# simplew4y/VeritasFi

Hardware: AMD Instinct MI355X
Metric: queries/sec top-100 over 10Mx768 corpus (higher is better)
Workload: dtype f16

## Files before the change

### include/veritasfi_hip.h

```cpp
#ifndef VERITASFI_HIP_H
#define VERITASFI_HIP_H

#include <stdint.h>

#ifdef __cplusplus
extern "C" {
#endif

#define VF_VERSION 100

enum {
    VF_OK = 0,
    VF_EINVAL = -1,
    VF_ENOMEM = -2,
    VF_EHIP = -3,
    VF_EUNSUPPORTED = -4,
    VF_EINTERNAL = -5
};

enum { VF_DTYPE_F32 = 0, VF_DTYPE_F16 = 1, VF_DTYPE_FP8_E4M3 = 2, VF_DTYPE_INT8 = 3 };

typedef struct vf_index vf_index;

typedef struct vf_search_stats {
    int64_t path;
    int64_t n_queries;
    int64_t candidates;
    int64_t max_candidates;
    int64_t uncertified;
    int64_t overflowed;
    int64_t exact_reruns;
    int64_t wide_launches;
    int64_t wide_queries;
    int64_t aux_cus;
    int64_t scans_overlap;
    int64_t scan_kernel;
    int64_t scan_image;
    int64_t reserved[3];
} vf_search_stats;

int vf_version(void);
const char* vf_last_error(void);
int vf_device_count(int32_t* out);

int vf_index_create(vf_index** out, const void* rows, int64_t n, int32_t d, int32_t dtype,
                    int32_t device_id, int64_t id_offset);

int vf_index_create_device(vf_index** out, const void* d_rows, int64_t n, int32_t d, int32_t dtype,
                           int32_t device_id, int64_t id_offset);

int vf_index_create_sharded(vf_index** out, const void* rows, int64_t n, int32_t d, int32_t dtype,
                            const int32_t* device_ids, int32_t n_dev);
int vf_index_create_sharded_from_file(vf_index** out, const char* path, const int32_t* device_ids, int32_t n_dev);
int vf_index_group(vf_index** out, vf_index** shards, int32_t n_shards);
int vf_index_shards(vf_index* idx, int32_t* n_shards, int32_t* device_ids, int32_t cap);
int vf_index_peer_access(vf_index* idx, int32_t* ok, int32_t cap, int32_t* n_missing);

int vf_corpus_file_info(const char* path, int64_t* n, int32_t* d, int32_t* dtype, int32_t* has_ids);
int vf_index_create_from_file(vf_index** out, const char* path, int64_t row_lo, int64_t row_hi, int32_t device_id,
                              int64_t id_offset);

int vf_index_search(vf_index* idx, const float* queries, int32_t nq, int32_t k, int64_t* out_ids,
                    float* out_scores);

int vf_index_search_device(vf_index* idx, const float* d_queries, int32_t nq, int32_t k,
                           int64_t* d_ids, float* d_scores, void* stream);

int vf_index_slots(vf_index* idx, int32_t* out);
int vf_index_search_begin(vf_index* idx, int32_t slot, const float* d_queries, int32_t nq, int32_t k,
                          int64_t* d_ids, float* d_scores, void* stream);
int vf_index_search_end(vf_index* idx, int32_t slot);

int vf_index_info(vf_index* idx, int64_t* n, int32_t* d, int32_t* dtype, int32_t* device_id);
int vf_index_stats(vf_index* idx, vf_search_stats* out);
int vf_index_set_option(vf_index* idx, const char* name, int64_t value);
int vf_index_profile(vf_index* idx, double* scan_ms_total, int64_t* scan_launches, double* pipeline_ms_total,
                     int64_t* scan_bytes_per_launch);
int vf_index_profile_span(vf_index* idx, double* span_ms, int64_t* launches);
int vf_index_debug_read(vf_index* idx, int32_t slot, unsigned long long* out, int64_t n_words);
int vf_index_destroy(vf_index* idx);

int vf_cosine_matrix(const float* x, int32_t n, int32_t d, float* out, int32_t device_id);
int vf_cosine_matrix_rows(vf_index* idx, const int64_t* ids, int32_t n, float* out);
int vf_cosine_matrix_rows_mixed(vf_index* idx, const int64_t* ids, int32_t n, const float* extra, int32_t n_extra, float* out);

int vf_cosine_scores(const float* a, int32_t na, const float* b, int64_t nb, int32_t d, float* out,
                     int32_t device_id);

int vf_merge_topk_device(const int64_t* d_ids_parts, const float* d_score_parts, int32_t nparts,
                         int32_t nq, int32_t k, int64_t* d_ids, float* d_scores, int32_t device_id,
                         void* stream);

int vf_merge_topk_packed_device(const void* d_parts, int32_t nparts, int32_t nq, int32_t k, int64_t* d_ids,
                                float* d_scores, int32_t device_id, void* stream);

int vf_fuse_rank(const float* rerank_scores, const float* time_scores, int32_t n, float* out_scores,
                 int64_t* out_order, int32_t device_id);

typedef struct vf_encoder vf_encoder;
typedef struct vf_encoder_config {
    int32_t vocab, hidden, layers, heads, ffn, max_pos, type_vocab;
    int32_t roberta_pad_idx;
    int32_t pooling;
    int32_t normalize;
    int32_t head;
    float ln_eps;
} vf_encoder_config;

int vf_encoder_weight_sizes(const vf_encoder_config* cfg, int64_t* n_fp16, int64_t* n_fp32);
int vf_encoder_create(vf_encoder** out, const vf_encoder_config* cfg, const void* w_fp16, int64_t n_fp16,
                      const float* w_fp32, int64_t n_fp32, int32_t device_id);
int vf_encoder_forward(vf_encoder* enc, const int32_t* ids, const int32_t* mask, const int32_t* type_ids,
                       int32_t b, int32_t t, int32_t t_valid, float* out);
int vf_encoder_forward_pooled(vf_encoder* enc, const int32_t* ids, const int32_t* mask, const int32_t* type_ids,
                              int32_t b, int32_t t, int32_t t_valid, int32_t pooling, int32_t normalize, float* out);
int vf_encoder_forward_hidden(vf_encoder* enc, const int32_t* ids, const int32_t* mask, const int32_t* type_ids,
                              int32_t b, int32_t t, float* out_hidden);
int vf_encoder_info(vf_encoder* enc, vf_encoder_config* out);
int vf_encoder_destroy(vf_encoder* enc);
typedef struct vf_decoder vf_decoder;
typedef struct vf_decoder_config {
    int32_t vocab, hidden, layers, heads, kv_heads, head_dim, ffn;
    float rope_theta, rms_eps;
    int32_t qk_norm;
    int32_t pooling;
    int32_t normalize;
    int32_t head;
    int32_t act;
    int32_t norm_plus_one;
    float embed_scale;
} vf_decoder_config;
int vf_decoder_weight_sizes(const vf_decoder_config* cfg, int64_t* n_fp16, int64_t* n_fp32);
int vf_decoder_create(vf_decoder** out, const vf_decoder_config* cfg, const void* w_fp16, int64_t n_fp16,
                      const float* w_fp32, int64_t n_fp32, int32_t device_id);
int vf_decoder_forward(vf_decoder* dec, const int32_t* ids, const int32_t* mask, int32_t b, int32_t t, int32_t t_valid,
                       float* out);
int vf_decoder_forward_pooled(vf_decoder* dec, const int32_t* ids, const int32_t* mask, int32_t b, int32_t t, int32_t t_valid,
                              int32_t normalize, float* out);
int vf_decoder_forward_hidden(vf_decoder* dec, const int32_t* ids, const int32_t* mask, int32_t b, int32_t t,
                              float* out_hidden);
int vf_decoder_destroy(vf_decoder* dec);

int vf_reranker_create(vf_encoder** out, const vf_encoder_config* cfg, const void* w_fp16, int64_t n_fp16,
                       const float* w_fp32, int64_t n_fp32, int32_t device_id);
int vf_reranker_score(vf_encoder* rr, const int32_t* ids, const int32_t* mask, const int32_t* type_ids, int32_t b,
                      int32_t t, float* out_scores);
int vf_reranker_destroy(vf_encoder* rr);

typedef struct vf_vit vf_vit;
typedef struct vf_vit_config {
    int32_t image, patch, channels;
    int32_t hidden, layers, heads, ffn;
    int32_t proj_dim;
    int32_t act;
    int32_t normalize;
    float ln_eps;
} vf_vit_config;
int vf_vit_weight_sizes(const vf_vit_config* cfg, int64_t* n_fp16, int64_t* n_fp32);
int vf_vit_create(vf_vit** out, const vf_vit_config* cfg, const void* w_fp16, int64_t n_fp16, const float* w_fp32,
                  int64_t n_fp32, int32_t device_id);
int vf_vit_forward(vf_vit* vit, const float* pixels, int32_t b, float* out);
int vf_vit_forward_u8(vf_vit* vit, const unsigned char* pixels, const float* mean3, const float* std3, int32_t b, float* out);
int vf_vit_destroy(vf_vit* vit);

typedef struct vf_clip_text vf_clip_text;
typedef struct vf_clip_text_config {
    int32_t vocab, max_pos;
    int32_t hidden, layers, heads, ffn;
    int32_t proj_dim;
    int32_t act;
    int32_t eos_token_id;
    int32_t normalize;
    float ln_eps;
} vf_clip_text_config;
int vf_clip_text_weight_sizes(const vf_clip_text_config* cfg, int64_t* n_fp16, int64_t* n_fp32);
int vf_clip_text_create(vf_clip_text** out, const vf_clip_text_config* cfg, const void* w_fp16, int64_t n_fp16, const float* w_fp32,
                        int64_t n_fp32, int32_t device_id);
int vf_clip_text_forward(vf_clip_text* ct, const int32_t* ids, const int32_t* mask, int32_t b, int32_t t, float* out);
int vf_clip_text_destroy(vf_clip_text* ct);

typedef struct vf_bm25 vf_bm25;
int vf_bm25_create(const int64_t* indptr, int64_t vocab, const int32_t* indices, const float* data, int64_t nnz,
                   int64_t n_docs, int32_t device_id, vf_bm25** out, int32_t* slots);
int vf_bm25_search(vf_bm25* h, const int64_t* q_offsets, const int32_t* q_terms, int32_t nq, int32_t k, int64_t* out_ids,
                   float* out_scores);

#ifdef __cplusplus
}
#endif
#endif
```

### veritasfi_amd/_ffi.py

```python
from __future__ import annotations

import ctypes
import os
import threading

_HERE = os.path.dirname(os.path.abspath(__file__))
LIB_PATH = os.environ.get("VF_LIB_PATH") or os.path.join(_HERE, "lib", "libveritasfi_hip.so")

VF_OK = 0
VF_DTYPE_F32, VF_DTYPE_F16, VF_DTYPE_FP8_E4M3, VF_DTYPE_INT8 = 0, 1, 2, 3

c_i32, c_i64, c_f32 = ctypes.c_int32, ctypes.c_int64, ctypes.c_float
p_i32, p_i64, p_f32 = ctypes.POINTER(c_i32), ctypes.POINTER(c_i64), ctypes.POINTER(c_f32)
vp = ctypes.c_void_p


class EncoderConfig(ctypes.Structure):
    _fields_ = [
        ("vocab", c_i32), ("hidden", c_i32), ("layers", c_i32), ("heads", c_i32), ("ffn", c_i32), ("max_pos", c_i32),
        ("type_vocab", c_i32), ("roberta_pad_idx", c_i32), ("pooling", c_i32), ("normalize", c_i32), ("head", c_i32),
        ("ln_eps", c_f32),
    ]


class DecoderConfig(ctypes.Structure):
    _fields_ = [
        ("vocab", c_i32), ("hidden", c_i32), ("layers", c_i32), ("heads", c_i32), ("kv_heads", c_i32), ("head_dim", c_i32),
        ("ffn", c_i32), ("rope_theta", c_f32), ("rms_eps", c_f32), ("qk_norm", c_i32), ("pooling", c_i32),
        ("normalize", c_i32), ("head", c_i32), ("act", c_i32), ("norm_plus_one", c_i32), ("embed_scale", c_f32),
    ]


class VitConfig(ctypes.Structure):
    _fields_ = [
        ("image", c_i32), ("patch", c_i32), ("channels", c_i32), ("hidden", c_i32), ("layers", c_i32), ("heads", c_i32),
        ("ffn", c_i32), ("proj_dim", c_i32), ("act", c_i32), ("normalize", c_i32), ("ln_eps", c_f32),
    ]


class ClipTextConfig(ctypes.Structure):
    _fields_ = [
        ("vocab", c_i32), ("max_pos", c_i32), ("hidden", c_i32), ("layers", c_i32), ("heads", c_i32), ("ffn", c_i32),
        ("proj_dim", c_i32), ("act", c_i32), ("eos_token_id", c_i32), ("normalize", c_i32), ("ln_eps", c_f32),
    ]


class SearchStats(ctypes.Structure):
    _fields_ = [
        ("path", c_i64), ("n_queries", c_i64), ("candidates", c_i64), ("max_candidates", c_i64),
        ("uncertified", c_i64), ("overflowed", c_i64), ("exact_reruns", c_i64), ("wide_launches", c_i64), ("wide_queries", c_i64),
        ("aux_cus", c_i64), ("scans_overlap", c_i64), ("scan_kernel", c_i64), ("scan_image", c_i64), ("reserved", c_i64 * 3),
    ]

    def as_dict(self):
        return {k: int(getattr(self, k)) for k, _ in self._fields_ if k != "reserved"}


SIGNATURES = {
    "vf_version": (ctypes.c_int, []),
    "vf_last_error": (ctypes.c_char_p, []),
    "vf_device_count": (ctypes.c_int, [p_i32]),
    "vf_index_create": (ctypes.c_int, [ctypes.POINTER(vp), vp, c_i64, c_i32, c_i32, c_i32, c_i64]),
    "vf_index_create_device": (ctypes.c_int, [ctypes.POINTER(vp), vp, c_i64, c_i32, c_i32, c_i32, c_i64]),
    "vf_index_create_sharded": (ctypes.c_int, [ctypes.POINTER(vp), vp, c_i64, c_i32, c_i32, p_i32, c_i32]),
    "vf_index_create_sharded_from_file": (ctypes.c_int, [ctypes.POINTER(vp), ctypes.c_char_p, p_i32, c_i32]),
    "vf_index_group": (ctypes.c_int, [ctypes.POINTER(vp), ctypes.POINTER(vp), c_i32]),
    "vf_index_shards": (ctypes.c_int, [vp, p_i32, p_i32, c_i32]),
    "vf_index_peer_access": (ctypes.c_int, [vp, p_i32, c_i32, p_i32]),
    "vf_corpus_file_info": (ctypes.c_int, [ctypes.c_char_p, ctypes.POINTER(c_i64), ctypes.POINTER(c_i32), ctypes.POINTER(c_i32), ctypes.POINTER(c_i32)]),
    "vf_index_create_from_file": (ctypes.c_int, [ctypes.POINTER(vp), ctypes.c_char_p, c_i64, c_i64, c_i32, c_i64]),
    "vf_index_search": (ctypes.c_int, [vp, vp, c_i32, c_i32, vp, vp]),
    "vf_index_search_device": (ctypes.c_int, [vp, vp, c_i32, c_i32, vp, vp, vp]),
    "vf_index_slots": (ctypes.c_int, [vp, p_i32]),
    "vf_index_search_begin": (ctypes.c_int, [vp, c_i32, vp, c_i32, c_i32, vp, vp, vp]),
    "vf_index_search_end": (ctypes.c_int, [vp, c_i32]),
    "vf_index_info": (ctypes.c_int, [vp, p_i64, p_i32, p_i32, p_i32]),
    "vf_index_stats": (ctypes.c_int, [vp, ctypes.POINTER(SearchStats)]),
    "vf_index_set_option": (ctypes.c_int, [vp, ctypes.c_char_p, c_i64]),
    "vf_index_profile": (ctypes.c_int, [vp, ctypes.POINTER(ctypes.c_double), p_i64, ctypes.POINTER(ctypes.c_double), p_i64]),
    "vf_index_profile_span": (ctypes.c_int, [vp, ctypes.POINTER(ctypes.c_double), p_i64]),
    "vf_index_debug_read": (ctypes.c_int, [vp, c_i32, vp, c_i64]),
    "vf_index_destroy": (ctypes.c_int, [vp]),
    "vf_cosine_matrix": (ctypes.c_int, [vp, c_i32, c_i32, vp, c_i32]),
    "vf_cosine_matrix_rows": (ctypes.c_int, [vp, vp, c_i32, vp]),
    "vf_cosine_matrix_rows_mixed": (ctypes.c_int, [vp, vp, c_i32, vp, c_i32, vp]),
    "vf_cosine_scores": (ctypes.c_int, [vp, c_i32, vp, c_i64, c_i32, vp, c_i32]),
    "vf_merge_topk_device": (ctypes.c_int, [vp, vp, c_i32, c_i32, c_i32, vp, vp, c_i32, vp]),
    "vf_merge_topk_packed_device": (ctypes.c_int, [vp, c_i32, c_i32, c_i32, vp, vp, c_i32, vp]),
    "vf_fuse_rank": (ctypes.c_int, [vp, vp, c_i32, vp, vp, c_i32]),
    "vf_encoder_weight_sizes": (ctypes.c_int, [ctypes.POINTER(EncoderConfig), p_i64, p_i64]),
    "vf_encoder_create": (ctypes.c_int, [ctypes.POINTER(vp), ctypes.POINTER(EncoderConfig), vp, c_i64, vp, c_i64, c_i32]),
    "vf_encoder_forward": (ctypes.c_int, [vp, vp, vp, vp, c_i32, c_i32, c_i32, vp]),
    "vf_encoder_forward_pooled": (ctypes.c_int, [vp, vp, vp, vp, c_i32, c_i32, c_i32, c_i32, c_i32, vp]),
    "vf_encoder_forward_hidden": (ctypes.c_int, [vp, vp, vp, vp, c_i32, c_i32, vp]),
    "vf_encoder_info": (ctypes.c_int, [vp, ctypes.POINTER(EncoderConfig)]),
    "vf_encoder_destroy": (ctypes.c_int, [vp]),
    "vf_reranker_create": (ctypes.c_int, [ctypes.POINTER(vp), ctypes.POINTER(EncoderConfig), vp, c_i64, vp, c_i64, c_i32]),
    "vf_reranker_score": (ctypes.c_int, [vp, vp, vp, vp, c_i32, c_i32, vp]),
    "vf_reranker_destroy": (ctypes.c_int, [vp]),
    "vf_decoder_weight_sizes": (ctypes.c_int, [vp, p_i64, p_i64]),
    "vf_decoder_create": (ctypes.c_int, [ctypes.POINTER(vp), vp, vp, c_i64, vp, c_i64, c_i32]),
    "vf_decoder_forward": (ctypes.c_int, [vp, vp, vp, c_i32, c_i32, c_i32, vp]),
    "vf_decoder_forward_pooled": (ctypes.c_int, [vp, vp, vp, c_i32, c_i32, c_i32, c_i32, vp]),
    "vf_decoder_forward_hidden": (ctypes.c_int, [vp, vp, vp, c_i32, c_i32, vp]),
    "vf_decoder_destroy": (ctypes.c_int, [vp]),
    "vf_vit_weight_sizes": (ctypes.c_int, [ctypes.POINTER(VitConfig), p_i64, p_i64]),
    "vf_vit_create": (ctypes.c_int, [ctypes.POINTER(vp), ctypes.POINTER(VitConfig), vp, c_i64, vp, c_i64, c_i32]),
    "vf_vit_forward": (ctypes.c_int, [vp, vp, c_i32, vp]),
    "vf_vit_forward_u8": (ctypes.c_int, [vp, vp, vp, vp, c_i32, vp]),
    "vf_vit_destroy": (ctypes.c_int, [vp]),
    "vf_clip_text_weight_sizes": (ctypes.c_int, [ctypes.POINTER(ClipTextConfig), p_i64, p_i64]),
    "vf_clip_text_create": (ctypes.c_int, [ctypes.POINTER(vp), ctypes.POINTER(ClipTextConfig), vp, c_i64, vp, c_i64, c_i32]),
    "vf_clip_text_forward": (ctypes.c_int, [vp, vp, vp, c_i32, c_i32, vp]),
    "vf_clip_text_destroy": (ctypes.c_int, [vp]),
    "vf_bm25_create": (ctypes.c_int, [p_i64, c_i64, p_i32, p_f32, c_i64, c_i64, c_i32, ctypes.POINTER(vp), p_i32]),
    "vf_bm25_search": (ctypes.c_int, [vp, p_i64, p_i32, c_i32, c_i32, p_i64, p_f32]),
}

_lib = None
_lock = threading.Lock()


def lib():
    global _lib
    if _lib is None:
        with _lock:
            if _lib is None:
                if not os.path.exists(LIB_PATH):
                    raise RuntimeError(
                        f"{LIB_PATH} is missing: build it with `python -m veritasfi_amd.build` "
                        "(hipcc --offload-arch=gfx950). veritasfi_amd has no CPU fallback.")
                try:
                    import torch
                except ImportError:
                    pass
                L = ctypes.CDLL(LIB_PATH)
                for name, (res, args) in SIGNATURES.items():
                    fn = getattr(L, name)
                    fn.restype = res
                    fn.argtypes = args
                _lib = L
    return _lib


def loaded() -> bool:
    return _lib is not None


def last_error() -> str:
    msg = lib().vf_last_error()
    return msg.decode("utf-8", "replace") if msg else ""


def check(rc: int, what: str = "") -> None:
    if rc != VF_OK:
        raise RuntimeError(f"{what or 'veritasfi_hip'} failed (rc={rc}): {last_error()}")
```

### veritasfi_amd/csrc/vf_api.hip

```cpp
#include "../../include/veritasfi_hip.h"
#include "vf_internal.h"

#include <fcntl.h>
#include <float.h>
#include <sys/stat.h>
#include <unistd.h>
#include <math.h>
#include <string.h>

#include <algorithm>
#include <atomic>
#include <mutex>
#include <string>
#include <vector>

using namespace vf;

static thread_local std::string g_err;

static int fail(int code, const std::string& msg) {
    g_err = msg;
    return code;
}
int vf::set_error(int code, const std::string& msg) { return fail(code, msg); }

#define VF_HIP(expr)                                                                                   \
    do {                                                                                               \
        hipError_t _e = (expr);                                                                        \
        if (_e != hipSuccess)                                                                          \
            return fail(VF_EHIP, std::string(#expr) + ": " + hipGetErrorString(_e) + " (" + __FILE__ + \
                                     ":" + std::to_string(__LINE__) + ")");                            \
    } while (0)

#define VF_TRY(expr)             \
    do {                         \
        int _rc = (expr);        \
        if (_rc != VF_OK) return _rc; \
    } while (0)

extern "C" int vf_version(void) { return VF_VERSION; }
extern "C" const char* vf_last_error(void) { return g_err.c_str(); }

extern "C" int vf_device_count(int32_t* out) {
    if (!out) return fail(VF_EINVAL, "vf_device_count: null out");
    int n = 0;
    hipError_t e = hipGetDeviceCount(&n);
    if (e != hipSuccess) { *out = 0; return fail(VF_EHIP, std::string("hipGetDeviceCount: ") + hipGetErrorString(e)); }
    *out = n;
    return VF_OK;
}

namespace {

constexpr int kSlots = 4;

struct DevBuf {
    void* p = nullptr;
    size_t bytes = 0;
    int ensure(size_t need) {
        if (need <= bytes) return VF_OK;
        if (p) { (void)hipFree(p); p = nullptr; bytes = 0; }
        hipError_t e = hipMalloc(&p, need);
        if (e != hipSuccess) return fail(VF_ENOMEM, std::string("hipMalloc(") + std::to_string(need) + "): " + hipGetErrorString(e));
        bytes = need;
        return VF_OK;
    }
    void release() { if (p) (void)hipFree(p); p = nullptr; bytes = 0; }
    template <class T> T* as() const { return (T*)p; }
};

struct HostBuf {
    void* p = nullptr;
    size_t bytes = 0;
    int ensure(size_t need) {
        if (need <= bytes) return VF_OK;
        if (p) { (void)hipHostFree(p); p = nullptr; bytes = 0; }
        hipError_t e = hipHostMalloc(&p, need, hipHostMallocDefault);
        if (e != hipSuccess) return fail(VF_ENOMEM, std::string("hipHostMalloc(") + std::to_string(need) + "): " + hipGetErrorString(e));
        bytes = need;
        return VF_OK;
    }
    void release() { if (p) (void)hipHostFree(p); p = nullptr; bytes = 0; }
};

struct Slot {
    hipStream_t stream = nullptr;
    hipStream_t scan_stream = nullptr;
    hipEvent_t ev_pro = nullptr;
    hipEvent_t ev_in = nullptr, ev_done = nullptr, ev_scan = nullptr;
    hipEvent_t ev_t[4] = {nullptr, nullptr, nullptr, nullptr};
    bool timed = false;
    int wide_launches = 0, wide_queries = 0;
    int scan_kernel = 0;
    int scan_image = 0;
    DevBuf qn, qimg, s0, cnt, tau, hist, hist_coarse, cand, flags, counts;
    DevBuf dbg, wgbase, tilecnt, sib;
    DevBuf qimg8, epsq;
    DevBuf qscale, bandq;
    int image_i8 = 0;
    int64_t wgbase_n = -1; int wgbase_grid = -1;
    DevBuf dense_s, cn_tmp, parts_ids, parts_sc, run_ids, run_sc, qsel;
    int* h_flags = nullptr;
    u32* h_counts = nullptr;
    int* d_flags = nullptr;
    u32* d_counts = nullptr;
    size_t h_cap = 0;
    bool pending = false;
    const float* d_queries = nullptr;
    int nq = 0, k = 0, path = 0;
    int64_t* d_ids = nullptr;
    float* d_scores = nullptr;
    hipStream_t user_stream = nullptr;
};

struct GroupSlot {
    std::vector<hipStream_t> feed;
    std::vector<hipEvent_t> ev;
    std::vector<DevBuf> dq, blob;
    DevBuf all;
    hipEvent_t ev_in = nullptr;
    hipStream_t hq_stream = nullptr;
    hipEvent_t ev_hq = nullptr;
    HostBuf hq;
    std::vector<hipStream_t> hfeed;
    std::vector<hipEvent_t> ev_hb;
    std::vector<hipEvent_t> ev_home;
    std::vector<HostBuf> hb;
    std::vector<char> staged_last;
    bool pending = false;
    int nq = 0, k = 0;
    int64_t* d_ids = nullptr; float* d_scores = nullptr;
    hipStream_t user = nullptr;
};

}

struct vf_index {
    int device = 0;
    int64_t n = 0;
    int d = 0, dp = 0, dtype = 0;
    int64_t id_offset = 0;
    int n_cu = 256;
    int64_t aux_applied = -1;
    bool owns_rows = false;
    void* rows_orig = nullptr;
    void* rows_scan = nullptr;
    bool owns_scan = false;
    float* norm = nullptr;
    float* inv_scan = nullptr;
    float* cn_cache = nullptr;
    unsigned char* rows_img = nullptr;
    bool owns_img = false;
    float* inv_img = nullptr;
    float rho_max = 0.0f;
    float rho_mean = 0.0f;
    std::mutex mu;
    Slot slots[kSlots];
    int64_t force_path = -1, sample_rows = -1, margin = -1, cap_opt = 0, waves_opt = 0, scan_g = 0,
            refresh_every = 128, debug = 0, steal_opt = 0, wide_opt = 1, wide_sync = -1, wide_mfma = -1, wide8_waves = 8, wide8_stage = 0,
            aux_cus = -1, sample_grid = -1, overlap_scans = -1, scan_impl = 2, sample_impl = -1, scan_image = 1, wide_rows = 1, image_mfma = -1;
    vf_search_stats stats{};
    bool profile = false;
    double prof_scan_ms = 0.0, prof_pipe_ms = 0.0;
    int64_t prof_launches = 0, prof_bytes = 0;
    hipEvent_t ev_span = nullptr;
    bool span_started = false;
    bool span_slot[4] = {false, false, false, false};
    DevBuf st_q, st_ids, st_sc;
    std::vector<vf_index*> shards;
    std::vector<int> peer_ok;
    GroupSlot gslots[kSlots];
};

static int ensure_pinned(Slot& s, size_t nq_total) {
    if (nq_total <= s.h_cap) return VF_OK;
    if (s.h_flags) (void)hipHostFree(s.h_flags);
    if (s.h_counts) (void)hipHostFree(s.h_counts);
    s.h_flags = nullptr; s.h_counts = nullptr; s.h_cap = 0;
    size_t cap = std::max<size_t>(nq_total, 256);
    VF_HIP(hipHostMalloc((void**)&s.h_flags, cap * sizeof(int), hipHostMallocMapped));
    VF_HIP(hipHostMalloc((void**)&s.h_counts, cap * sizeof(u32), hipHostMallocMapped));
    VF_HIP(hipHostGetDevicePointer((void**)&s.d_flags, s.h_flags, 0));
    VF_HIP(hipHostGetDevicePointer((void**)&s.d_counts, s.h_counts, 0));
    s.h_cap = cap;
    return VF_OK;
}

static int build_image(vf_index* ix, int64_t mode);

static bool byte_rows(int dtype) { return dtype == VF_DTYPE_FP8_E4M3 || dtype == VF_DTYPE_INT8; }
static bool known_dtype(int64_t dtype) { return dtype >= VF_DTYPE_F32 && dtype <= VF_DTYPE_INT8; }
static size_t dtype_bytes(int dtype) { return dtype == VF_DTYPE_F32 ? 4 : (dtype == VF_DTYPE_F16 ? 2 : 1); }
static int scan_f8(int dtype) { return dtype == VF_DTYPE_INT8 ? 2 : (dtype == VF_DTYPE_FP8_E4M3 ? 1 : 0); }

static int build_common(vf_index* ix) {
    hipDeviceProp_t prop;
    VF_HIP(hipGetDeviceProperties(&prop, ix->device));
    ix->n_cu = prop.multiProcessorCount > 0 ? prop.multiProcessorCount : 256;
    VF_HIP(scan_configure());
    const int dt = ix->dtype;
    const size_t scan_esz = byte_rows(dt) ? 1 : 2;
    ix->dp = (ix->d + 127) / 128 * 128;
    const size_t npad = (size_t)ix->n + 64;
    VF_HIP(hipMalloc((void**)&ix->norm, npad * sizeof(float)));
    VF_HIP(hipMalloc((void**)&ix->inv_scan, npad * sizeof(float)));
    VF_HIP(hipMemset(ix->norm, 0, npad * sizeof(float)));
    VF_HIP(hipMemset(ix->inv_scan, 0, npad * sizeof(float)));
    const bool need_scan = ix->n > kSmallN;
    void* scan_out = nullptr;
    if (need_scan) {
        if (dt != VF_DTYPE_F32 && ix->dp == ix->d && ((uintptr_t)ix->rows_orig % 16) == 0) {
            ix->rows_scan = ix->rows_orig;
            ix->owns_scan = false;
        } else {
            VF_HIP(hipMalloc((void**)&ix->rows_scan, (size_t)ix->n * ix->dp * scan_esz));
            ix->owns_scan = true;
            scan_out = ix->rows_scan;
        }
    }
    VF_HIP(launch_prep_rows(ix->rows_orig, dt, ix->n, ix->d, ix->dp, scan_out, ix->norm, ix->inv_scan, nullptr));
    VF_TRY(build_image(ix, ix->scan_image));
    if (ix->n > 0 && ix->n <= kSmallN) {
        VF_HIP(hipMalloc((void**)&ix->cn_cache, (size_t)ix->n * ix->d * sizeof(float)));
        VF_HIP(launch_normalize_rows(ix->rows_orig, dt, 0, ix->n, ix->d, ix->norm, ix->cn_cache, nullptr));
    }
    VF_HIP(hipDeviceSynchronize());
    return VF_OK;
}

constexpr int64_t kSplitMaxRows = 6'000'000;
constexpr int64_t kScan2rMinRows = 1'100'000;
static bool scan2r_auto_width(int dp, bool f8) { return f8 ? (dp == 768 || dp == 1024) : (dp == 768 || dp == 1024 || dp == 512 || dp == 384); }
static int64_t split_limit(const vf_index* ix) {
    const bool r_rows = !byte_rows(ix->dtype) && ix->scan_impl != 4 && ix->scan_impl != 1 && ix->scan_impl != 3 && !ix->steal_opt &&
                        scan2r_auto_width(ix->dp, false) && scan2r_stage_cap(ix->dp, kMaxBatch, 0) >= 256;
    return r_rows ? INT64_MAX : kSplitMaxRows;
}
static int64_t resolved_aux(const vf_index* ix) {
    if (ix->aux_applied >= 0) return ix->aux_applied;
    int64_t a = ix->aux_cus >= 0 ? ix->aux_cus : (ix->n <= split_limit(ix) ? 32 : 0);
    if (a <= 0 || ix->n_cu < 64 || a * 2 > ix->n_cu) return 0;
    return a;
}
static bool resolved_overlap(const vf_index* ix) {
    return ix->overlap_scans >= 0 ? ix->overlap_scans != 0 : resolved_aux(ix) > 0;
}

constexpr int kImageMaxK = 128;
constexpr int64_t kImageMinRows = 4'000'000;
constexpr double kImageMaxRho = 1.0 / 64;
constexpr size_t kImageHeadroom = (size_t)8 << 30;
constexpr int kImageMfmaAuto = 1;
static bool image_eligible(const vf_index* ix, int64_t mode) {
    if (!ix->shards.empty() || ix->n >= (int64_t)0xFFFFFFFFll || ix->dp != 768 || scan2r_stage_cap(ix->dp, kMaxBatch, 2) < 256) return false;
    if (ix->dtype == VF_DTYPE_INT8) return ix->rows_scan && (mode == 2 ? ix->n > kSmallN : ix->n >= kImageMinRows);
    return (ix->dtype == VF_DTYPE_F16 || ix->dtype == VF_DTYPE_F32) && ix->n >= kImageMinRows;
}
static float* image_offsets(const vf_index* ix) { return ix->inv_img ? ix->inv_img + ix->n + 64 : nullptr; }
static void free_image(vf_index* ix) {
    if (ix->rows_img && ix->owns_img) (void)hipFree(ix->rows_img);
    if (ix->inv_img) (void)hipFree(ix->inv_img);
    ix->rows_img = nullptr; ix->inv_img = nullptr; ix->owns_img = false; ix->rho_max = ix->rho_mean = 0.0f;
}
static int build_image(vf_index* ix, int64_t mode) {
    if (mode == 0 || ix->rows_img || !image_eligible(ix, mode)) return VF_OK;
    const size_t ibytes = 2 * ((size_t)ix->n + 64) * sizeof(float);
    if (ix->dtype == VF_DTYPE_INT8) {
        if (hipMalloc((void**)&ix->inv_img, ibytes) != hipSuccess) {
            (void)hipGetLastError();
            ix->inv_img = nullptr;
            return mode == 2 ? fail(VF_ENOMEM, "scan_image = 2: the row inverses and offsets do not fit in device memory") : VF_OK;
        }
        VF_HIP(hipMemset(ix->inv_img, 0, ibytes));
        VF_HIP(hipMemcpy(ix->inv_img, ix->inv_scan, (size_t)ix->n * sizeof(float), hipMemcpyDeviceToDevice));
        ix->rows_img = (unsigned char*)ix->rows_scan; ix->owns_img = false;
        return VF_OK;
    }
    const size_t bytes = (size_t)ix->n * ix->dp;
    if (mode == 1) {
        size_t free_b = 0, total_b = 0;
        if (hipMemGetInfo(&free_b, &total_b) != hipSuccess) { (void)hipGetLastError(); return VF_OK; }
        if (free_b < bytes + ibytes + kImageHeadroom) return VF_OK;
    }
    ix->owns_img = true;
    if (hipMalloc((void**)&ix->rows_img, bytes) != hipSuccess || hipMalloc((void**)&ix->inv_img, ibytes) != hipSuccess) {
        (void)hipGetLastError();
        free_image(ix);
        return mode == 2 ? fail(VF_ENOMEM, "scan_image = 2: the int8 row image does not fit in device memory") : VF_OK;
    }
    u32* d_rho = nullptr;
    VF_HIP(hipMalloc((void**)&d_rho, 2 * sizeof(u32)));
    VF_HIP(hipMemset(d_rho, 0, 2 * sizeof(u32)));
    VF_HIP(hipMemset(ix->inv_img, 0, ibytes));
    VF_HIP(launch_prep_image(ix->rows_orig, ix->dtype, ix->n, ix->d, ix->dp, ix->norm, ix->rows_img, ix->inv_img, image_offsets(ix), d_rho,
                             (float*)(d_rho + 1), nullptr));
    u32 bits[2] = {0u, 0u};
    VF_HIP(hipMemcpy(bits, d_rho, sizeof(bits), hipMemcpyDeviceToHost));
    (void)hipFree(d_rho);
    float rho, sum;
    memcpy(&rho, &bits[0], sizeof(rho));
    memcpy(&sum, &bits[1], sizeof(sum));
    if (!(rho <= kImageMaxRho)) { free_image(ix); return VF_OK; }
    ix->rho_max = rho;
    ix->rho_mean = sum / (float)ix->n;
    return VF_OK;
}

static int ensure_slot(vf_index* ix, Slot& s) {
    if (s.stream) return VF_OK;
    VF_HIP(hipStreamCreateWithFlags(&s.stream, hipStreamNonBlocking));
    s.scan_stream = s.stream;
    int64_t aux = resolved_aux(ix);
    if (aux) {
        const int words = (ix->n_cu + 31) / 32;
        std::vector<uint32_t> mask(words, 0u);
        for (int b = 0; b < ix->n_cu - (int)aux; ++b) mask[b / 32] |= 1u << (b % 32);
        hipStream_t ms = nullptr;
        if (hipExtStreamCreateWithCUMask(&ms, (uint32_t)words, mask.data()) == hipSuccess && ms) s.scan_stream = ms;
        else { (void)hipGetLastError(); if (ix->aux_applied < 0) aux = 0; }
    }
    if (ix->aux_applied < 0) ix->aux_applied = aux;
    VF_HIP(hipEventCreateWithFlags(&s.ev_in, hipEventDisableTiming));
    VF_HIP(hipEventCreateWithFlags(&s.ev_done, hipEventDisableTiming));
    VF_HIP(hipEventCreateWithFlags(&s.ev_scan, hipEventDisableTiming));
    VF_HIP(hipEventCreateWithFlags(&s.ev_pro, hipEventDisableTiming));
    for (int e = 0; e < 4; ++e) VF_HIP(hipEventCreate(&s.ev_t[e]));
    return VF_OK;
}

static void destroy_index(vf_index* ix) {
    if (!ix) return;
    if (!ix->shards.empty()) {
        for (int i = 0; i < kSlots; ++i) {
            GroupSlot& gs = ix->gslots[i];
            for (size_t g = 0; g < ix->shards.size(); ++g) {
                (void)hipSetDevice(ix->shards[g]->device);
                (void)hipDeviceSynchronize();
                if (g < gs.dq.size()) gs.dq[g].release();
                if (g < gs.blob.size()) gs.blob[g].release();
                if (g < gs.feed.size() && gs.feed[g]) (void)hipStreamDestroy(gs.feed[g]);
                if (g < gs.ev.size() && gs.ev[g]) (void)hipEventDestroy(gs.ev[g]);
                if (g < gs.ev_hb.size() && gs.ev_hb[g]) (void)hipEventDestroy(gs.ev_hb[g]);
                if (g < gs.hb.size()) gs.hb[g].release();
            }
            (void)hipSetDevice(ix->device);
            gs.all.release();
            gs.hq.release();
            for (hipStream_t st : gs.hfeed) if (st) (void)hipStreamDestroy(st);
            for (hipEvent_t ev : gs.ev_home) if (ev) (void)hipEventDestroy(ev);
            if (gs.hq_stream) (void)hipStreamDestroy(gs.hq_stream);
            if (gs.ev_hq) (void)hipEventDestroy(gs.ev_hq);
            if (gs.ev_in) (void)hipEventDestroy(gs.ev_in);
        }
        for (vf_index* sh : ix->shards) destroy_index(sh);
        ix->shards.clear();
    }
    (void)hipSetDevice(ix->device);
    (void)hipDeviceSynchronize();
    ix->st_q.release(); ix->st_ids.release(); ix->st_sc.release();
    for (int i = 0; i < kSlots; ++i) {
        Slot& s = ix->slots[i];
        DevBuf* bufs[] = {&s.qn, &s.qimg, &s.s0, &s.cnt, &s.tau, &s.hist, &s.hist_coarse, &s.cand, &s.flags, &s.counts, &s.dense_s,
                          &s.cn_tmp, &s.parts_ids, &s.parts_sc, &s.run_ids, &s.run_sc, &s.qsel, &s.dbg, &s.wgbase, &s.tilecnt, &s.sib};
        for (DevBuf* b : bufs) b->release();
        if (s.h_flags) (void)hipHostFree(s.h_flags);
        if (s.h_counts) (void)hipHostFree(s.h_counts);
        if (s.scan_stream && s.scan_stream != s.stream) (void)hipStreamDestroy(s.scan_stream);
        if (s.stream) (void)hipStreamDestroy(s.stream);
        if (s.ev_pro) (void)hipEventDestroy(s.ev_pro);
        if (s.ev_in) (void)hipEventDestroy(s.ev_in);
        if (s.ev_done) (void)hipEventDestroy(s.ev_done);
        if (s.ev_scan) (void)hipEventDestroy(s.ev_scan);
        for (int e = 0; e < 4; ++e) if (s.ev_t[e]) (void)hipEventDestroy(s.ev_t[e]);
    }
    if (ix->owns_scan && ix->rows_scan) (void)hipFree(ix->rows_scan);
    if (ix->owns_rows && ix->rows_orig) (void)hipFree(ix->rows_orig);
    if (ix->norm) (void)hipFree(ix->norm);
    if (ix->inv_scan) (void)hipFree(ix->inv_scan);
    if (ix->cn_cache) (void)hipFree(ix->cn_cache);
    if (ix->rows_img && ix->owns_img) (void)hipFree(ix->rows_img);
    if (ix->inv_img) (void)hipFree(ix->inv_img);
    if (ix->ev_span) (void)hipEventDestroy(ix->ev_span);
    delete ix;
}

static int create_impl(vf_index** out, const void* rows, bool rows_on_device, int64_t n, int32_t d, int32_t dtype,
                       int32_t device_id, int64_t id_offset, bool adopt = false) {
    if (!out) return fail(VF_EINVAL, "vf_index_create: null out");
    *out = nullptr;
    if (n < 0 || d <= 0 || (n > 0 && !rows)) return fail(VF_EINVAL, "vf_index_create: bad rows/n/d");
    if (!known_dtype(dtype)) return fail(VF_EINVAL, "vf_index_create: unknown dtype");
    if (n >= (int64_t)0xFFFFFFFFll) return fail(VF_EUNSUPPORTED, "vf_index_create: more than 2^32-1 rows per shard");
    int ndev = 0;
    VF_HIP(hipGetDeviceCount(&ndev));
    if (device_id < 0 || device_id >= ndev) return fail(VF_EINVAL, "vf_index_create: bad device_id");
    VF_HIP(hipSetDevice(device_id));
    vf_index* ix = new (std::nothrow) vf_index();
    if (!ix) return fail(VF_ENOMEM, "vf_index_create: host allocation failed");
    ix->device = device_id; ix->n = n; ix->d = d; ix->id_offset = id_offset;
    ix->dtype = dtype;
    const size_t esz = dtype_bytes(dtype);
    int rc = VF_OK;
    if (rows_on_device && dtype == VF_DTYPE_INT8 && !adopt && n > 0) {
        hipError_t e = hipMalloc(&ix->rows_orig, (size_t)n * d);
        if (e != hipSuccess) rc = fail(VF_ENOMEM, std::string("hipMalloc(corpus): ") + hipGetErrorString(e));
        else {
            ix->owns_rows = true;
            e = launch_rebias_i8(rows, ix->rows_orig, (long long)n * d, nullptr);
            if (e != hipSuccess) rc = fail(VF_EHIP, std::string("re-biasing the int8 rows: ") + hipGetErrorString(e));
        }
    } else if (rows_on_device) {
        ix->rows_orig = const_cast<void*>(rows);
        ix->owns_rows = false;
        if (dtype == VF_DTYPE_INT8 && n > 0) {
            const hipError_t e = launch_rebias_i8(ix->rows_orig, ix->rows_orig, (long long)n * d, nullptr);
            if (e != hipSuccess) rc = fail(VF_EHIP, std::string("re-biasing the int8 rows: ") + hipGetErrorString(e));
        }
    } else if (n > 0) {
        hipError_t e = hipMalloc(&ix->rows_orig, (size_t)n * d * esz);
        if (e != hipSuccess) rc = fail(VF_ENOMEM, std::string("hipMalloc(corpus): ") + hipGetErrorString(e));
        else {
            ix->owns_rows = true;
            e = hipMemcpy(ix->rows_orig, rows, (size_t)n * d * esz, hipMemcpyHostToDevice);
            if (e != hipSuccess) rc = fail(VF_EHIP, std::string("hipMemcpy(corpus): ") + hipGetErrorString(e));
            else if (dtype == VF_DTYPE_INT8) {
                e = launch_rebias_i8(ix->rows_orig, ix->rows_orig, (long long)n * d, nullptr);
                if (e != hipSuccess) rc = fail(VF_EHIP, std::string("re-biasing the int8 rows: ") + hipGetErrorString(e));
            }
        }
    }
    if (rc == VF_OK) rc = build_common(ix);
    if (rc != VF_OK) { std::string keep = g_err; destroy_index(ix); g_err = keep; return rc; }
    *out = ix;
    return VF_OK;
}

extern "C" int vf_index_create(vf_index** out, const void* rows, int64_t n, int32_t d, int32_t dtype,
                               int32_t device_id, int64_t id_offset) {
    DeviceGuard restore_callers_device;
    return create_impl(out, rows, false, n, d, dtype, device_id, id_offset);
}

extern "C" int vf_index_create_device(vf_index** out, const void* d_rows, int64_t n, int32_t d, int32_t dtype,
                                      int32_t device_id, int64_t id_offset) {
    DeviceGuard restore_callers_device;
    return create_impl(out, d_rows, true, n, d, dtype, device_id, id_offset);
}

struct VfcHeader {
    char magic[8];
    uint32_t version, dtype;
    uint64_t n;
    uint32_t d, flags;
    uint8_t reserved[32];
};
static_assert(sizeof(VfcHeader) == 64, "corpus file header is 64 bytes");

static int read_vfc_header(int fd, const char* path, VfcHeader* h, size_t* esz) {
    if (pread(fd, h, sizeof(*h), 0) != (ssize_t)sizeof(*h)) return fail(VF_EINVAL, std::string("corpus file too short: ") + path);
    if (memcmp(h->magic, "VFCORPUS", 8) != 0) return fail(VF_EINVAL, std::string("not a corpus file (bad magic): ") + path);
    if (h->version != 1) return fail(VF_EUNSUPPORTED, std::string("corpus file version not supported: ") + path);
    if (!known_dtype(h->dtype) || h->d == 0) return fail(VF_EINVAL, std::string("corpus file header is corrupt: ") + path);
    *esz = dtype_bytes((int)h->dtype);
    struct stat st;
    if (fstat(fd, &st) != 0) return fail(VF_EINVAL, std::string("cannot stat corpus file: ") + path);
    unsigned long long payload = 0, ids = 0, need = 0;
    if (__builtin_mul_overflow((unsigned long long)h->n, (unsigned long long)h->d * (unsigned long long)*esz, &payload) ||
        __builtin_mul_overflow((unsigned long long)h->n, (h->flags & 1u) ? 8ull : 0ull, &ids) ||
        __builtin_add_overflow(payload, ids, &need) || __builtin_add_overflow(need, 64ull, &need))
        return fail(VF_EINVAL, std::string("corpus file header is corrupt (n x d overflows): ") + path);
    if ((unsigned long long)st.st_size < need) return fail(VF_EINVAL, std::string("corpus file is truncated: ") + path);
    if (h->n >= 0x7fffffffffffffffull / 2) return fail(VF_EINVAL, std::string("corpus file header is corrupt: ") + path);
    return VF_OK;
}

extern "C" int vf_corpus_file_info(const char* path, int64_t* n, int32_t* d, int32_t* dtype, int32_t* has_ids) {
    if (!path) return fail(VF_EINVAL, "vf_corpus_file_info: null path");
    const int fd = open(path, O_RDONLY);
    if (fd < 0) return fail(VF_EINVAL, std::string("cannot open corpus file: ") + path);
    VfcHeader h; size_t esz = 0;
    const int rc = read_vfc_header(fd, path, &h, &esz);
    close(fd);
    if (rc != VF_OK) return rc;
    if (n) *n = (int64_t)h.n;
    if (d) *d = (int32_t)h.d;
    if (dtype) *dtype = (int32_t)h.dtype;
    if (has_ids) *has_ids = (int32_t)(h.flags & 1u);
    return VF_OK;
}

extern "C" int vf_index_create_from_file(vf_index** out, const char* path, int64_t row_lo, int64_t row_hi,
                                         int32_t device_id, int64_t id_offset) {
    DeviceGuard restore_callers_device;
    if (!out || !path) return fail(VF_EINVAL, "vf_index_create_from_file: null argument");
    *out = nullptr;
    const int fd = open(path, O_RDONLY);
    if (fd < 0) return fail(VF_EINVAL, std::string("cannot open corpus file: ") + path);
    VfcHeader h; size_t esz = 0;
    int rc = read_vfc_header(fd, path, &h, &esz);
    if (rc == VF_OK && (row_lo < 0 || row_hi < row_lo || (uint64_t)row_hi > h.n))
        rc = fail(VF_EINVAL, "vf_index_create_from_file: row range outside the file");
    int ndev = 0;
    if (rc == VF_OK && (hipGetDeviceCount(&ndev) != hipSuccess || device_id < 0 || device_id >= ndev))
        rc = fail(VF_EINVAL, "vf_index_create_from_file: bad device_id");
    if (rc != VF_OK) { close(fd); return rc; }
    const int64_t n = row_hi - row_lo;
    const size_t row_bytes = (size_t)h.d * esz, total = (size_t)n * row_bytes;
    void* d_rows = nullptr;
    char* stage[2] = {nullptr, nullptr};
    hipEvent_t ev[2] = {nullptr, nullptr};
    const size_t chunk = 64u << 20;
    hipError_t e = hipSetDevice(device_id);
    if (e == hipSuccess && total) e = hipMalloc(&d_rows, total);
    for (int i = 0; i < 2 && e == hipSuccess && total; ++i) {
        e = hipHostMalloc((void**)&stage[i], chunk, hipHostMallocDefault);
        if (e == hipSuccess) e = hipEventCreateWithFlags(&ev[i], hipEventDisableTiming);
    }
    if (e != hipSuccess) rc = fail(VF_ENOMEM, std::string("vf_index_create_from_file: ") + hipGetErrorString(e));
    size_t done = 0;
    for (int i = 0; rc == VF_OK && done < total; i ^= 1) {
        const size_t len = std::min(chunk, total - done);
        if (hipEventSynchronize(ev[i]) != hipSuccess) { rc = fail(VF_EHIP, "vf_index_create_from_file: event wait failed"); break; }
        size_t got = 0;
        while (got < len) {
            const ssize_t r = pread(fd, stage[i] + got, len - got, (off_t)(64 + (size_t)row_lo * row_bytes + done + got));
            if (r <= 0) { rc = fail(VF_EINVAL, std::string("read error in corpus file: ") + path); break; }
            got += (size_t)r;
        }
        if (rc != VF_OK) break;
        e = hipMemcpyAsync((char*)d_rows + done, stage[i], len, hipMemcpyHostToDevice, nullptr);
        if (e == hipSuccess) e = hipEventRecord(ev[i], nullptr);
        if (e != hipSuccess) { rc = fail(VF_EHIP, std::string("vf_index_create_from_file: ") + hipGetErrorString(e)); break; }
        done += len;
    }
    close(fd);
    if (rc == VF_OK && hipDeviceSynchronize() != hipSuccess) rc = fail(VF_EHIP, "vf_index_create_from_file: copy failed");
    for (int i = 0; i < 2; ++i) {
        if (stage[i]) (void)hipHostFree(stage[i]);
        if (ev[i]) (void)hipEventDestroy(ev[i]);
    }
    if (rc == VF_OK) {
        rc = create_impl(out, d_rows, true, n, (int32_t)h.d, (int32_t)h.dtype, device_id, id_offset, true);
        if (rc == VF_OK) { (*out)->owns_rows = true; d_rows = nullptr; }
    }
    if (d_rows) (void)hipFree(d_rows);
    return rc;
}

extern "C" int vf_index_destroy(vf_index* ix) {
    DeviceGuard restore_callers_device;
    if (!ix) return VF_OK;
    destroy_index(ix);
    return VF_OK;
}

extern "C" int vf_index_info(vf_index* ix, int64_t* n, int32_t* d, int32_t* dtype, int32_t* device_id) {
    if (!ix) return fail(VF_EINVAL, "vf_index_info: null handle");
    if (n) *n = ix->n;
    if (d) *d = ix->d;
    if (dtype) *dtype = ix->dtype;
    if (device_id) *device_id = ix->device;
    return VF_OK;
}

extern "C" int vf_index_stats(vf_index* ix, vf_search_stats* out) {
    if (!ix || !out) return fail(VF_EINVAL, "vf_index_stats: null argument");
    std::lock_guard<std::mutex> g(ix->mu);
    *out = ix->stats;
    return VF_OK;
}

extern "C" int vf_index_profile(vf_index* ix, double* scan_ms_total, int64_t* scan_launches, double* pipeline_ms_total,
                                int64_t* scan_bytes_per_launch) {
    if (!ix) return fail(VF_EINVAL, "vf_index_profile: null handle");
    std::lock_guard<std::mutex> g(ix->mu);
    double sm = ix->prof_scan_ms, pm = ix->prof_pipe_ms;
    int64_t nl = ix->prof_launches, nb = ix->prof_bytes;
    for (vf_index* sh : ix->shards) {
        std::lock_guard<std::mutex> lk(sh->mu);
        sm += sh->prof_scan_ms; pm += sh->prof_pipe_ms; nl += sh->prof_launches;
        if (nb == 0) nb = sh->prof_bytes;
    }
    if (scan_ms_total) *scan_ms_total = sm;
    if (scan_launches) *scan_launches = nl;
    if (pipeline_ms_total) *pipeline_ms_total = pm;
    if (scan_bytes_per_launch) *scan_bytes_per_launch = nb;
    return VF_OK;
}

extern "C" int vf_index_profile_span(vf_index* ix, double* span_ms, int64_t* launches) {
    if (!ix || !span_ms || !launches) return fail(VF_EINVAL, "vf_index_profile_span: null argument");
    DeviceGuard restore_callers_device;
    vf_index* t = ix->shards.empty() ? ix : ix->shards[0];
    std::lock_guard<std::mutex> g(t->mu);
    *span_ms = 0.0; *launches = t->prof_launches;
    if (!t->span_started || !t->ev_span) return VF_OK;
    VF_HIP(hipSetDevice(t->device));
    for (int i = 0; i < kSlots; ++i) {
        if (!t->span_slot[i] || !t->slots[i].ev_t[1] || t->slots[i].pending) continue;
        float ms = 0.f;
        if (hipEventElapsedTime(&ms, t->ev_span, t->slots[i].ev_t[1]) == hipSuccess && ms > *span_ms) *span_ms = ms;
        else (void)hipGetLastError();
    }
    return VF_OK;
}

extern "C" int vf_index_debug_read(vf_index* ix, int32_t slot, unsigned long long* out, int64_t n_words) {
    DeviceGuard restore_callers_device;
    if (!ix || !out || slot < 0 || slot >= kSlots) return fail(VF_EINVAL, "vf_index_debug_read: bad argument");
    if (!ix->shards.empty()) return vf_index_debug_read(ix->shards[0], slot, out, n_words);
    std::lock_guard<std::mutex> g(ix->mu);
    Slot& s = ix->slots[slot];
    const size_t bytes = std::min<size_t>(s.dbg.bytes, (size_t)n_words * 8);
    VF_HIP(hipSetDevice(ix->device));
    VF_HIP(hipDeviceSynchronize());
    if (bytes) VF_HIP(hipMemcpy(out, s.dbg.p, bytes, hipMemcpyDeviceToHost));
    return (int)(bytes / 8);
}

extern "C" int vf_index_slots(vf_index* ix, int32_t* out) {
    if (!ix || !out) return fail(VF_EINVAL, "vf_index_slots: null argument");
    *out = kSlots;
    return VF_OK;
}

extern "C" int vf_index_set_option(vf_index* ix, const char* name, int64_t value) {
    if (!ix || !name) return fail(VF_EINVAL, "vf_index_set_option: null argument");
    for (vf_index* sh : ix->shards) VF_TRY(vf_index_set_option(sh, name, value));
    std::lock_guard<std::mutex> g(ix->mu);
    const std::string s(name);
    auto in_range = [&](int64_t lo, int64_t hi) { return value >= lo && value <= hi; };
    if (s == "force_path") { if (!in_range(-1, 2)) return fail(VF_EINVAL, "force_path must be -1 (auto), 0, 1 or 2"); ix->force_path = value; }
    else if (s == "sample_rows") { if (!in_range(-1, 64) || value == 0) return fail(VF_EINVAL, "sample_rows must be -1 (auto) or in [1, 64]"); ix->sample_rows = value; }
    else if (s == "margin") { if (!in_range(-1, 2048)) return fail(VF_EINVAL, "margin must be -1 (auto) or in [0, 2048]"); ix->margin = value; }
    else if (s == "cap") { if (!in_range(0, 16384)) return fail(VF_EINVAL, "cap must be in [0, 16384]"); ix->cap_opt = value; }
    else if (s == "waves") { if (!in_range(0, 8 * 1024)) return fail(VF_EINVAL, "waves must be in [0, 8192]"); ix->waves_opt = value; }
    else if (s == "scan_g") { if (!in_range(0, 4)) return fail(VF_EINVAL, "scan_g must be in [0, 4]"); ix->scan_g = value; }
    else if (s == "refresh_every") { if (!in_range(1, 256)) return fail(VF_EINVAL, "refresh_every must be in [1, 256]"); ix->refresh_every = value; }
    else if (s == "steal") { if (!in_range(0, 1)) return fail(VF_EINVAL, "steal must be 0 or 1"); ix->steal_opt = value; }
    else if (s == "wide") { if (!in_range(0, 4096)) return fail(VF_EINVAL, "wide must be 0 (off), 1 (auto) or a query count"); ix->wide_opt = value; }
    else if (s == "wide8_stage") { if (value != 0 && !in_range(64, 3584)) return fail(VF_EINVAL, "wide8_stage must be 0 (auto) or 64..3584 candidate-stage entries"); ix->wide8_stage = value; }
    else if (s == "wide8_waves") {
#ifdef VF_EXPERIMENTS
        if (value != 4 && value != 8) return fail(VF_EINVAL, "wide8_waves must be 8 (one 512-thread workgroup per CU, 256-query tiles: the default) or 4 (two 256-thread workgroups, 128-query tiles: measured slower, DESIGN.md 4)");
#else
        if (value != 8) return fail(VF_EINVAL, "wide8_waves must be 8 (the 4-wave form was measured slower and is built with -DVF_EXPERIMENTS only: DESIGN.md 4)");
#endif
        ix->wide8_waves = value;
    }
    else if (s == "wide_mfma") { if (!in_range(-1, 1)) return fail(VF_EINVAL, "wide_mfma must be -1 (auto: the fp8 instruction for e4m3 rows), 0 (fp16 matrix instruction on converted rows) or 1 (the fp8 instruction on the e4m3 row bytes: k_scan_wide8)"); ix->wide_mfma = value; }
    else if (s == "wide_sync") { if (!in_range(-1, 8)) return fail(VF_EINVAL, "wide_sync must be -1 (off) or a slack of 0..8 super-tiles"); ix->wide_sync = value; }
    else if (s == "aux_cus") {
        if (!in_range(-1, 128)) return fail(VF_EINVAL, "aux_cus must be -1 (auto) or in [0, 128]");
        if (ix->aux_applied >= 0 && value != ix->aux_cus)
            return fail(VF_EINVAL, "aux_cus is fixed once the first search has created the scan streams: set it before searching");
        ix->aux_cus = value;
    }
    else if (s == "sample_grid") { if (!in_range(-1, 1024)) return fail(VF_EINVAL, "sample_grid must be -1 (auto), 0 (one workgroup per range) or a workgroup count"); ix->sample_grid = value; }
    else if (s == "scan_impl") { if (!in_range(1, 5)) return fail(VF_EINVAL, "scan_impl must be 1 (k_scan), 2 (auto: k_scan2 for fp16 rows, k_scan2r where it measured faster), 3 (k_scan2 wherever it fits, e4m3 rows converted), 4 (k_scan2 for fp16 rows, never k_scan2r) or 5 (k_scan2r wherever a shape of it exists: fp16 rows of 384 / 512 / 768 / 1024 elements, e4m3 rows of 768 / 1024)"); ix->scan_impl = value; }
    else if (s == "sample_impl") { if (!in_range(-1, 1)) return fail(VF_EINVAL, "sample_impl must be -1 (auto: k_scan2r's operand path for the sample pass where it exists and the CU split is on), 0 (k_scan) or 1 (k_scan2r wherever it fits)"); ix->sample_impl = value; }
    else if (s == "overlap_scans") { if (!in_range(-1, 1)) return fail(VF_EINVAL, "overlap_scans must be -1 (auto), 0 or 1"); ix->overlap_scans = value; }
    else if (s == "scan_image") {
        if (!in_range(0, 2)) return fail(VF_EINVAL, "scan_image must be 0 (off), 1 (auto: when it fits with headroom) or 2 (force)");
        if (!ix->shards.empty()) { ix->scan_image = value; return VF_OK; }
        for (const Slot& sl : ix->slots) if (sl.pending) return fail(VF_EINVAL, "scan_image cannot change while a search is pending");
        DeviceGuard restore_callers_device;
        VF_HIP(hipSetDevice(ix->device));
        VF_HIP(hipDeviceSynchronize());
        if (value == 0) free_image(ix);
        else VF_TRY(build_image(ix, value));
        ix->scan_image = value;
    }
    else if (s == "image_mfma") { if (!in_range(-1, 2)) return fail(VF_EINVAL, "image_mfma must be -1 (auto), 0 (the int8 row image on the fp16 matrix instruction, fp16 queries), 1 (on the int8 matrix instruction, the queries as one int8 plane) or 2 (as two planes, hi + lo: the band of 0)"); ix->image_mfma = value; }
    else if (s == "wide_rows") { if (!in_range(0, 2)) return fail(VF_EINVAL, "wide_rows must be 0 (rows of more than 2432 padded elements never take the fused path), 1 (auto: from 131 072 rows, e4m3 rows from 32 768) or 2 (wherever k_scan_ksplit / k_scan_ksplit8 serve them)"); ix->wide_rows = value; }
    else if (s == "debug") ix->debug = value;
    else if (s == "profile") {
        ix->profile = value != 0; ix->prof_scan_ms = ix->prof_pipe_ms = 0.0; ix->prof_launches = 0;
        ix->span_started = false;
        for (bool& b : ix->span_slot) b = false;
    }
    else return fail(VF_EINVAL, "vf_index_set_option: unknown option " + s);
    return VF_OK;
}

static int exact_search(vf_index* ix, Slot& s, const float* qn_dev, int nq, int k, int64_t* out_ids,
                        float* out_scores, hipStream_t st) {
    const int dt = ix->dtype;
    const int64_t chunk = kSmallN;
    const int64_t nchunks = ix->n == 0 ? 1 : (ix->n + chunk - 1) / chunk;
    if (nchunks > 1) {
        int64_t P = 1;
        while (P < 2 * (int64_t)k) P <<= 1;
        if (P * 8 > 160 * 1024) return fail(VF_EUNSUPPORTED, "exact chunked search supports k <= 8192 when n > 16384");
    }
    VF_TRY(s.dense_s.ensure((size_t)nq * chunk * sizeof(float)));
    if (nchunks == 1) {
        const float* cn = ix->cn_cache;
        if (!cn && ix->n > 0) {
            VF_TRY(s.cn_tmp.ensure((size_t)chunk * ix->d * sizeof(float)));
            VF_HIP(launch_normalize_rows(ix->rows_orig, dt, 0, ix->n, ix->d, ix->norm, s.cn_tmp.as<float>(), st));
            cn = s.cn_tmp.as<float>();
        }
        VF_HIP(launch_dense_dot16(qn_dev, nq, cn, ix->n, ix->d, s.dense_s.as<float>(), chunk, st));
        VF_HIP(launch_sort_rows(s.dense_s.as<float>(), chunk, nq, (int)ix->n, k, ix->id_offset, (long long*)out_ids,
                                out_scores, k, st));
        return VF_OK;
    }
    VF_TRY(s.cn_tmp.ensure((size_t)chunk * ix->d * sizeof(float)));
    const size_t part = (size_t)nq * k;
    VF_TRY(s.parts_ids.ensure(2 * part * sizeof(long long)));
    VF_TRY(s.parts_sc.ensure(2 * part * sizeof(float)));
    VF_TRY(s.run_ids.ensure(part * sizeof(long long)));
    VF_TRY(s.run_sc.ensure(part * sizeof(float)));
    long long* pid = s.parts_ids.as<long long>();
    float* psc = s.parts_sc.as<float>();
    VF_HIP(hipMemsetAsync(pid, 0xFF, part * sizeof(long long), st));
    VF_HIP(hipMemsetAsync(psc, 0, part * sizeof(float), st));
    for (int64_t c = 0; c < nchunks; ++c) {
        const int64_t r0 = c * chunk, nr = std::min(chunk, ix->n - r0);
        VF_HIP(launch_normalize_rows(ix->rows_orig, dt, r0, nr, ix->d, ix->norm, s.cn_tmp.as<float>(), st));
        VF_HIP(launch_dense_dot16(qn_dev, nq, s.cn_tmp.as<float>(), nr, ix->d, s.dense_s.as<float>(), chunk, st));
        VF_HIP(launch_sort_rows(s.dense_s.as<float>(), chunk, nq, (int)nr, k, ix->id_offset + r0, pid + part, psc + part,
                                k, st));
        VF_HIP(launch_merge_topk(pid, psc, 2, nq, k, s.run_ids.as<long long>(), s.run_sc.as<float>(), st));
        VF_HIP(hipMemcpyAsync(pid, s.run_ids.p, part * sizeof(long long), hipMemcpyDeviceToDevice, st));
        VF_HIP(hipMemcpyAsync(psc, s.run_sc.p, part * sizeof(float), hipMemcpyDeviceToDevice, st));
    }
    VF_HIP(hipMemcpyAsync(out_ids, s.run_ids.p, part * sizeof(long long), hipMemcpyDeviceToDevice, st));
    VF_HIP(hipMemcpyAsync(out_scores, s.run_sc.p, part * sizeof(float), hipMemcpyDeviceToDevice, st));
    return VF_OK;
}

struct FusedPlan {
    int kprime, cap, total_waves, grid, samp;
    float eps;
    bool image;
    int tau_band, fine_band;
};

static int qn_tile_for(int nq_batch) { return nq_batch <= kQueryTile ? kQueryTile : kMaxBatch; }

constexpr int64_t kWideRowsMinRows = 131072;
static bool ksplit_width(const vf_index* ix) { return scan_lds_bytes(ix->dp, kQueryTile) > 160 * 1024; }
constexpr int64_t kWideRowsMinRows8 = 32768;
static bool rows_e4m3(const vf_index* ix) { return ix->dtype == VF_DTYPE_FP8_E4M3; }
static int ksplit_stage_cap(const vf_index* ix) { return rows_e4m3(ix) ? scan_ksplit8_stage_cap(ix->dp) : scan_ksplit_stage_cap(ix->dp); }
static bool ksplit_serves(const vf_index* ix, bool forced) {
    if (ix->dtype == VF_DTYPE_INT8) return false;
    if (ix->wide_rows == 0 || ksplit_stage_cap(ix) < 256) return false;
    return forced || ix->wide_rows == 2 || ix->n >= (rows_e4m3(ix) ? kWideRowsMinRows8 : kWideRowsMinRows);
}

static bool fused_possible(const vf_index* ix, int k, bool forced = false) {
    if (ix->n <= 1024 || k > kMaxKFused || k <= 0) return false;
    if (!ix->rows_scan || !ix->inv_scan) return false;
    if (ksplit_width(ix)) return ix->n > kSmallN && ksplit_serves(ix, forced);
    return true;
}

static int batch_limit(const vf_index* ix) {
    return scan_lds_bytes(ix->dp, kMaxBatch) <= 160 * 1024 ? kMaxBatch : kQueryTile;
}

static void image_bound(int d, int dtype, float rho_mean, float* eps, int* tau_band, int* fine_band) {
    const double u16 = 1.0 / 2048.0;
    const double base = u16 * (dtype == VF_DTYPE_F32 ? 2.0 : 1.0) + sqrt((double)d) * ldexp(1.0, -24) + 2.0 * d * ldexp(1.0, -24) + 1e-6;
    const float e = (float)(base + 1e-7);
    const double band = (double)e + 1.5 * rho_mean * (1.0 + u16) * (1.0 + ldexp(1.0, -20)) + ldexp(1.0, -9);
    *eps = e;
    *tau_band = (int)ceil(band * (kHistBins / 2)) + 1;
    *fine_band = (int)ceil(band * (kHistBins / 2) * 16) + 1;
}

extern "C" int vf_debug_image_bound(int32_t d, int32_t dtype, float rho_mean, float* eps, int32_t* tau_band, int32_t* fine_band) {
    if (!eps || !tau_band || !fine_band || d <= 0) return fail(VF_EINVAL, "vf_debug_image_bound: bad argument");
    int tb = 0, fb = 0;
    image_bound(d, dtype, rho_mean, eps, &tb, &fb);
    *tau_band = tb; *fine_band = fb;
    return VF_OK;
}

extern "C" int vf_debug_image_q8_bound(float rho_q, float eps_img, int32_t tau_band, int32_t fine_band, float* eps_q, int32_t* tau_band_q,
                                       int32_t* fine_band_q) {
    if (!eps_q || !tau_band_q || !fine_band_q) return fail(VF_EINVAL, "vf_debug_image_q8_bound: bad argument");
    const Q8Bound b = image_q8_bound(rho_q);
    *eps_q = image_q8_eps(eps_img, b.eps_add);
    *tau_band_q = tau_band + b.tau_bins; *fine_band_q = fine_band + b.fine_bins;
    return VF_OK;
}

static int image_planes(const vf_index* ix, int qt) {
    const int m = ix->image_mfma < 0 ? kImageMfmaAuto : (int)ix->image_mfma;
    return (m >= 1 && scan2r_stage_cap(ix->dp, qt, 2 + m) >= 256) ? m : 0;
}

static bool image_serves(const vf_index* ix, int k, int qt) {
    return ix->rows_img && k <= kImageMaxK && (ix->scan_impl == 2 || ix->scan_impl == 5) && !ix->steal_opt && ix->sample_impl != 0 &&
           scan2r_stage_cap(ix->dp, qt, 2) >= 256;
}

static FusedPlan make_plan(const vf_index* ix, int k, bool image = false) {
    FusedPlan p;
    p.image = image; p.tau_band = 0; p.fine_band = 0;
    int margin = ix->margin >= 0 ? (int)ix->margin : std::max(24, k / 4);
    const double u16 = 1.0 / 2048.0;
    const float eps_plan = (float)(u16 * (ix->dtype == VF_DTYPE_F32 ? 2.0 : 1.0) + sqrt((double)ix->d) * ldexp(1.0, -24) +
                                   2.0 * ix->d * ldexp(1.0, -24) + 1e-6);
    if (ix->margin < 0 && ksplit_width(ix)) {
        const double z = sqrt(2.0 * log(std::max(3.0, (double)ix->n / k)));
        margin = std::max(margin, (int)ceil(2.5 * eps_plan * k * z * sqrt((double)ix->d)));
    }
    p.kprime = ix->margin >= 0 ? k + margin : (k + margin + 31) / 32 * 32;
    p.kprime = std::min(p.kprime, 4096);
    int cap = kMaxCap;
    while (cap < 4 * p.kprime && cap < 16384) cap <<= 1;
    if (ix->cap_opt > 0) { cap = 1; while (cap < ix->cap_opt) cap <<= 1; cap = std::min(cap, 16384); }
    while (cap < 2 * p.kprime) cap <<= 1;
    p.cap = cap;
    const int64_t scan_cus = ix->n_cu - resolved_aux(ix);
    int64_t wgs = std::min<int64_t>(scan_cus, std::max<int64_t>(1, ix->n / 512));
    if (ix->waves_opt > 0) wgs = std::max<int64_t>(1, ix->waves_opt / (kScanThreads / 64));
    p.grid = (int)wgs;
    p.total_waves = p.grid * (kScanThreads / 64);
    p.samp = ix->sample_rows > 0 ? (int)ix->sample_rows : ((ix->n <= 1500000 && 8ll * p.total_waves >= 16ll * p.kprime) ? 8 : 16);
    if (ix->cap_opt <= 0) {
        const double sample_rows = (double)p.total_waves * p.samp;
        const double expect = p.kprime * (1.0 + log(std::max(1.0, (double)ix->n / std::max(1.0, sample_rows))));
        while (p.cap < (int)(1.6 * expect) && p.cap < 32768) p.cap <<= 1;
    }
    p.eps = eps_plan;
    if (image) {
        image_bound(ix->d, ix->dtype, ix->rho_mean, &p.eps, &p.tau_band, &p.fine_band);
        p.kprime = k;
        p.cap = 32768;
    }
    return p;
}

static int select_path(const vf_index* ix, int k) {
    if (ix->force_path >= 0) {
        if (ix->force_path == 1 && !fused_possible(ix, k, true)) return -1;
        return (int)ix->force_path;
    }
    if (ix->n <= kSmallN) return 0;
    return fused_possible(ix, k) ? 1 : 2;
}

constexpr int kWideMinQueries = 129;
constexpr int kWideMinQueries16 = 65;
constexpr int kWideMinQueriesKsplit = 33;
constexpr int kWideMinQueriesKsplit8 = 65;
constexpr int kWideMaxQueries = 1024;
constexpr int kWideTile = 256;

static bool wide_possible(const vf_index* ix, int nq) {
    const bool ks = ksplit_width(ix);
    if (ix->wide_opt == 0 || nq < (ix->wide_opt > 1 ? (int)ix->wide_opt : ks ? (rows_e4m3(ix) ? kWideMinQueriesKsplit8 : kWideMinQueriesKsplit) : (byte_rows(ix->dtype) ? kWideMinQueries : kWideMinQueries16))) return false;
    return ix->dp % (byte_rows(ix->dtype) ? 256 : 128) == 0;
}

static int wide_pass(vf_index* ix, Slot& s, const FusedPlan& p0, const float* d_queries, int nb, int k, int64_t* d_ids,
                     float* d_scores, int flag_off, float* qn_b, bool timed, hipStream_t st, int slot_id) {
    const int qtot = (nb + kWideTile - 1) / kWideTile * kWideTile;
    const int J = qtot / kWideTile;
    const int RG = std::max(1, ix->n_cu / J);
    FusedPlan p = p0;
    if (p.kprime > 256) p.cap = std::max(p.cap, 16384);
    const bool w8 = (ix->wide_mfma > 0 || (ix->wide_mfma < 0 && !ksplit_width(ix))) && ix->dtype == VF_DTYPE_FP8_E4M3 && ix->dp % 64 == 0 &&
                    (ix->n / RG + 2 * 256) * (int64_t)ix->dp < (int64_t)0xFFFFFFFFll;
    if (w8) {
        if (p.kprime > 256) p.cap = std::max(p.cap, 32768);
    }
    const int samp = J >= 2 ? 64 : 32;
    const size_t slen = (size_t)RG * samp * 8;
    VF_TRY(s.qimg.ensure((size_t)ix->dp * qtot * 2));
    VF_TRY(s.s0.ensure((size_t)qtot * slen * sizeof(float)));
    VF_TRY(s.cnt.ensure((size_t)qtot * kCntStride * sizeof(u32)));
    VF_TRY(s.tau.ensure((size_t)qtot * sizeof(int)));
    VF_TRY(s.hist.ensure((size_t)qtot * kHistBins * sizeof(u32)));
    VF_TRY(s.hist_coarse.ensure((size_t)qtot * 64 * sizeof(u32)));
    VF_TRY(s.cand.ensure((size_t)qtot * p.cap * sizeof(u64)));
    if (s.wgbase_n != ix->n || s.wgbase_grid != -RG) {
        std::vector<long long> base(RG);
        for (int w = 0; w < RG; ++w) base[w] = ix->n * (long long)w / RG;
        VF_TRY(s.wgbase.ensure((size_t)RG * sizeof(long long)));
        VF_HIP(hipMemcpyAsync(s.wgbase.p, base.data(), (size_t)RG * sizeof(long long), hipMemcpyHostToDevice, st));
        VF_HIP(hipStreamSynchronize(st));
        s.wgbase_n = ix->n; s.wgbase_grid = -RG;
    }
    VF_HIP(launch_prep_queries(d_queries, nb, ix->d, ix->dp, qtot, qn_b, s.qimg.as<_Float16>(), st));
    if (w8) {
        VF_TRY(s.qimg8.ensure((size_t)ix->dp * qtot * 2));
        VF_TRY(s.epsq.ensure((size_t)qtot * sizeof(float)));
        VF_HIP(launch_prep_wide8(qn_b, nb, ix->d, ix->dp, qtot, (unsigned char*)s.qimg8.p, s.epsq.as<float>(), st));
    }
    const int f8 = scan_f8(ix->dtype);
    ScanArgs a{};
    a.rows = (const char*)ix->rows_scan; a.inv_scan = ix->inv_scan; a.qimg = s.qimg.as<_Float16>();
    a.n = ix->n; a.dp = ix->dp; a.row_bytes = (long long)ix->dp * (f8 ? 1 : 2);
    a.total_waves = RG * 8; a.samp = samp;
    a.s0 = s.s0.as<float>(); a.wg_base = s.wgbase.as<long long>(); a.cnt = s.cnt.as<u32>(); a.tau_bin = s.tau.as<int>();
    a.hist = s.hist.as<u32>(); a.hist_coarse = s.hist_coarse.as<u32>(); a.cand = s.cand.as<u64>(); a.cap = p.cap; a.kprime = p.kprime;
    a.stage_cap = 3584; a.dbg = nullptr; a.debug = (int)ix->debug;
    a.refresh_every = 1;
    while (a.refresh_every * 2 <= (int)std::min<int64_t>(256, std::max<int64_t>(1, ix->refresh_every))) a.refresh_every *= 2;
    a.nq = nb; a.qn_total = qtot; a.jtiles = J; a.rgroups = RG;
    if (ix->n / RG < (int64_t)samp * 8)
        VF_HIP(hipMemsetAsync(a.s0, 0xFF, (size_t)qtot * slen * sizeof(float), st));
    VF_HIP(launch_scan_wide(a, kModeSample, f8, st));
    VF_HIP(launch_sel0(a, qtot, st));
    for (int o = 0; o < kSlots; ++o)
        if (o != slot_id && ix->slots[o].ev_scan) VF_HIP(hipStreamWaitEvent(st, ix->slots[o].ev_scan, 0));
    const int w8_waves = ix->wide8_waves == 4 ? 4 : 8;
    const int J8 = w8 && w8_waves == 4 ? (nb + 127) / 128 : J;
    if (J8 > 1 && ix->wide_sync >= 0) {
        VF_TRY(s.sib.ensure((size_t)RG * 8 * sizeof(u32)));
        VF_HIP(hipMemsetAsync(s.sib.p, 0, (size_t)RG * 8 * sizeof(u32), st));
        a.sib = s.sib.as<u32>(); a.sib_slack = (int)ix->wide_sync;
    }
    if (timed) VF_HIP(hipEventRecord(s.ev_t[0], st));
    if (w8) {
        ScanArgs a8 = a;
        a8.qimg = (const _Float16*)s.qimg8.p;
        a8.jtiles = J8;
        a8.stage_cap = ix->wide8_stage > 0 ? (int)std::min<int64_t>(ix->wide8_stage, scan_wide8_stage_cap(w8_waves)) : scan_wide8_stage_cap(w8_waves);
        if (ix->debug & 128) {
            VF_TRY(s.dbg.ensure((size_t)8 * J8 * ((RG + 7) / 8) * w8_waves * 16 * sizeof(u64)));
            VF_HIP(hipMemsetAsync(s.dbg.p, 0, s.dbg.bytes, st));
            a8.dbg = s.dbg.as<u64>();
        }
        VF_HIP(launch_scan_wide8(a8, w8_waves, st));
    } else
        VF_HIP(launch_scan_wide(a, kModeMain, f8, st));
    VF_HIP(hipEventRecord(s.ev_scan, st));
    if (timed) {
        VF_HIP(hipEventRecord(s.ev_t[1], st));
        const int64_t sampled = std::min<int64_t>(ix->n, (int64_t)RG * std::min<int64_t>((int64_t)samp * 8, ix->n / RG));
        ix->prof_bytes = (ix->n - sampled) * ((int64_t)ix->d * (f8 ? 1 : 2) + 4);
    }
    FinalArgs f{};
    f.cnt = a.cnt; f.cand = a.cand; f.cap = p.cap; f.tau_bin = a.tau_bin; f.rows_orig = ix->rows_orig;
    f.orig_dtype = ix->dtype; f.orig_row_elems = ix->d; f.norm = ix->norm; f.qn = qn_b;
    f.d = ix->d; f.k = k; f.kprime = p.kprime; f.eps = p.eps; f.n_rows = ix->n; f.id_offset = ix->id_offset;
    f.eps_q = w8 ? s.epsq.as<float>() : nullptr;
    f.out_ids = (long long*)d_ids; f.out_scores = d_scores;
    f.flags = s.d_flags + flag_off; f.cand_count_out = s.d_counts + flag_off;
    f.dbg = nullptr;
    if (ix->debug & 256) { VF_TRY(s.dbg.ensure((size_t)qtot * 8 * sizeof(u64))); f.dbg = s.dbg.as<u64>(); }
    VF_HIP(launch_final(f, nb, st));
    s.scan_kernel = w8 ? 4 : 3;
    return VF_OK;
}

static int begin_impl(vf_index* ix, int slot_id, const float* d_queries, int nq, int k, int64_t* d_ids,
                      float* d_scores, hipStream_t user) {
    Slot& s = ix->slots[slot_id];
    if (s.pending) return fail(VF_EINVAL, "vf_index_search_begin: slot already has a pending search");
    const int path = select_path(ix, k);
    if (path < 0) return fail(VF_EUNSUPPORTED, "forced fused path is not possible for this n / k / d");
    if (path != 1 && ix->n > kSmallN && k > 8192)
        return fail(VF_EUNSUPPORTED, "exact chunked search supports k <= 8192 when n > 16384");
    VF_TRY(ensure_slot(ix, s));
    VF_HIP(hipEventRecord(s.ev_in, user));
    VF_HIP(hipStreamWaitEvent(s.stream, s.ev_in, 0));
    hipStream_t st = s.stream;
    const int bl = batch_limit(ix);
    VF_TRY(s.qn.ensure((size_t)std::max(nq, 1) * ix->d * sizeof(float)));
    VF_TRY(s.qimg.ensure(scan_lds_bytes(ix->dp, kMaxBatch)));
    VF_TRY(ensure_pinned(s, (size_t)nq));
    s.pending = true; s.d_queries = d_queries; s.nq = nq; s.k = k; s.d_ids = d_ids; s.d_scores = d_scores;
    s.path = path; s.user_stream = user; s.wide_launches = 0; s.wide_queries = 0; s.scan_kernel = 0;
    if (nq == 0 || k == 0) { VF_HIP(hipEventRecord(s.ev_done, st)); return VF_OK; }

    if (path != 1) {
        for (int b0 = 0; b0 < nq; b0 += bl) {
            const int nb = std::min(bl, nq - b0);
            VF_HIP(launch_prep_queries(d_queries + (size_t)b0 * ix->d, nb, ix->d, ix->dp, qn_tile_for(nb),
                                       s.qn.as<float>() + (size_t)b0 * ix->d, s.qimg.as<_Float16>(), st));
            VF_TRY(exact_search(ix, s, s.qn.as<float>() + (size_t)b0 * ix->d, nb, k, d_ids + (size_t)b0 * k,
                                d_scores + (size_t)b0 * k, st));
        }
        VF_HIP(hipEventRecord(s.ev_done, st));
        return VF_OK;
    }

    const bool ks = ksplit_width(ix);
    const bool img = !ks && !wide_possible(ix, nq) && image_serves(ix, k, qn_tile_for(std::min(bl, nq)));
    FusedPlan p = make_plan(ix, k, img);
    s.scan_image = img ? 1 : 0;
    s.image_i8 = img ? image_planes(ix, qn_tile_for(std::min(bl, nq))) : 0;
    const int img_f8 = 2 + s.image_i8;
    if (wide_possible(ix, nq)) {
        s.timed = ix->profile;
        if (s.timed) VF_HIP(hipEventRecord(s.ev_t[2], st));
        for (int b0 = 0; b0 < nq; b0 += kWideMaxQueries) {
            const int nb = std::min(kWideMaxQueries, nq - b0);
            VF_TRY(wide_pass(ix, s, p, d_queries + (size_t)b0 * ix->d, nb, k, d_ids + (size_t)b0 * k, d_scores + (size_t)b0 * k,
                             b0, s.qn.as<float>() + (size_t)b0 * ix->d, s.timed && b0 == 0, st, slot_id));
            ++s.wide_launches; s.wide_queries += nb;
        }
        if (s.timed) VF_HIP(hipEventRecord(s.ev_t[3], st));
        VF_HIP(hipEventRecord(s.ev_done, st));
        return VF_OK;
    }
    VF_TRY(s.s0.ensure((size_t)kMaxBatch * p.total_waves * p.samp * sizeof(float)));
    VF_TRY(s.cnt.ensure((size_t)kMaxBatch * kCntStride * sizeof(u32)));
    VF_TRY(s.tau.ensure(kMaxBatch * sizeof(int)));
    VF_TRY(s.hist.ensure((size_t)kMaxBatch * kHistBins * sizeof(u32)));
    VF_TRY(s.hist_coarse.ensure((size_t)kMaxBatch * 64 * sizeof(u32)));
    VF_TRY(s.cand.ensure((size_t)kMaxBatch * p.cap * sizeof(u64)));
    VF_TRY(s.tilecnt.ensure((size_t)p.grid * sizeof(u32)));
    s.timed = ix->profile;
    if (s.timed) VF_HIP(hipEventRecord(s.ev_t[2], st));
    if (s.wgbase_n != ix->n || s.wgbase_grid != p.grid) {
        std::vector<long long> base(p.grid);
        for (int w = 0; w < p.grid; ++w) base[w] = ix->n * (long long)w / p.grid;
        VF_TRY(s.wgbase.ensure((size_t)p.grid * sizeof(long long)));
        VF_HIP(hipMemcpy(s.wgbase.p, base.data(), (size_t)p.grid * sizeof(long long), hipMemcpyHostToDevice));
        s.wgbase_n = ix->n; s.wgbase_grid = p.grid;
    }
    for (int b0 = 0; b0 < nq; b0 += bl) {
        const int nb = std::min(bl, nq - b0);
        const int qt = qn_tile_for(nb);
        float* qn_b = s.qn.as<float>() + (size_t)b0 * ix->d;
        VF_HIP(launch_prep_queries(d_queries + (size_t)b0 * ix->d, nb, ix->d, ix->dp, qt, qn_b, s.image_i8 ? nullptr : s.qimg.as<_Float16>(), st));
        ScanArgs a{};
        a.rows = (const char*)ix->rows_scan; a.inv_scan = ix->inv_scan; a.qimg = s.qimg.as<_Float16>();
        if (s.image_i8) {
            VF_TRY(s.qimg8.ensure((size_t)ix->dp * kMaxBatch * 2));
            VF_TRY(s.epsq.ensure(kMaxBatch * sizeof(float)));
            VF_TRY(s.qscale.ensure(kMaxBatch * sizeof(float)));
            VF_TRY(s.bandq.ensure(2 * kMaxBatch * sizeof(int)));
            VF_HIP(launch_prep_q8(qn_b, nb, ix->d, ix->dp, qt, s.image_i8, (signed char*)s.qimg8.p, s.qscale.as<float>(), s.epsq.as<float>(), s.bandq.as<int>(),
                                  p.eps, p.tau_band, p.fine_band, st));
            a.qimg = (const _Float16*)s.qimg8.p; a.q_scale = s.qscale.as<float>(); a.band_q = s.bandq.as<int>();
        }
        a.n = ix->n; a.dp = ix->dp; a.row_bytes = (long long)ix->dp * (byte_rows(ix->dtype) ? 1 : 2); a.total_waves = p.total_waves; a.samp = p.samp;
        if (p.image) { a.rows = (const char*)ix->rows_img; a.inv_scan = ix->inv_img; a.off_scan = image_offsets(ix); a.row_bytes = ix->dp; }
        a.s0 = s.s0.as<float>(); a.wg_base = s.wgbase.as<long long>(); a.cnt = s.cnt.as<u32>(); a.tau_bin = s.tau.as<int>(); a.hist = s.hist.as<u32>();
        a.cand = s.cand.as<u64>(); a.cap = p.cap; a.kprime = p.kprime; a.tau_band = p.tau_band;
        a.hist_coarse = s.hist_coarse.as<u32>(); a.stage_cap = ks ? ksplit_stage_cap(ix) : scan_stage_cap(ix->dp, qt);
        a.tile_cnt = ix->steal_opt ? s.tilecnt.as<u32>() : nullptr; a.scan_grid = p.grid;
        a.dbg = nullptr;
        if (ix->debug & 128) { VF_TRY(s.dbg.ensure((size_t)p.total_waves * ((ix->debug & 512) ? 72 : 4) * sizeof(u64))); a.dbg = s.dbg.as<u64>(); if (ix->debug & 512) VF_HIP(hipMemsetAsync(s.dbg.p, 0, s.dbg.bytes, st)); }
        a.refresh_every = (int)std::min<int64_t>(256, std::max<int64_t>(4, std::max<int64_t>(1, ix->refresh_every) * nb / kMaxBatch));
        while (a.refresh_every & (a.refresh_every - 1)) a.refresh_every &= a.refresh_every - 1;
        a.nq = nb; a.debug = (int)ix->debug;
        if (ix->n / p.total_waves < p.samp)
            VF_HIP(hipMemsetAsync(a.s0, 0xFF, (size_t)qt * p.total_waves * p.samp * sizeof(float), st));
        const bool f8rows = ix->dtype == VF_DTYPE_FP8_E4M3 || p.image;
        const bool i8conv = ix->dtype == VF_DTYPE_INT8 && !p.image;
        const bool r_f8_auto = f8rows && ix->scan_impl == 2 && ix->n > kScan2rMinRows && !ix->steal_opt && scan2r_auto_width(ix->dp, true);
        const bool sample_r = p.image || (!i8conv && ix->sample_impl != 0 && ix->scan_impl != 1 && scan2r_stage_cap(ix->dp, qt, f8rows) >= 256 &&
                              (ix->sample_impl == 1 || (!f8rows && s.scan_stream != s.stream && scan2r_auto_width(ix->dp, false)) || r_f8_auto));
        if (ks) {
            VF_HIP(rows_e4m3(ix) ? launch_scan_ksplit8(a, kModeSample, p.grid, st) : launch_scan_ksplit(a, kModeSample, p.grid, st));
        } else if (sample_r) {
            const int64_t sg_r = ix->sample_grid > 0 ? ix->sample_grid : (s.scan_stream != s.stream ? resolved_aux(ix) : p.grid);
            ScanArgs as = a;
            as.stage_cap = 0;
            VF_HIP(launch_scan2r_sample(as, qt, (int)std::min<int64_t>(std::max<int64_t>(sg_r, 1), p.grid), p.image ? img_f8 : (int)f8rows, st));
        } else {
        const int64_t sg_opt = ix->sample_grid >= 0 ? ix->sample_grid : (s.scan_stream != s.stream ? 4 * resolved_aux(ix) : 0);
        const int sgrid = sg_opt > 0 ? (int)std::min<int64_t>(sg_opt, p.grid) : p.grid;
        VF_HIP(launch_scan(a, kModeSample, qt, sgrid, (int)ix->scan_g, scan_f8(ix->dtype), st));
        }
        VF_HIP(launch_sel0(a, qt, st));
        hipStream_t sst = s.scan_stream;
        if (sst != st) {
            VF_HIP(hipEventRecord(s.ev_pro, st));
            VF_HIP(hipStreamWaitEvent(sst, s.ev_pro, 0));
        }
        if (!resolved_overlap(ix))
            for (int o = 0; o < kSlots; ++o)
                if (o != slot_id && ix->slots[o].ev_scan) VF_HIP(hipStreamWaitEvent(sst, ix->slots[o].ev_scan, 0));
        if (s.timed && b0 == 0) {
            if (!ix->span_started) {
                if (!ix->ev_span) VF_HIP(hipEventCreate(&ix->ev_span));
                VF_HIP(hipEventRecord(ix->ev_span, sst));
                ix->span_started = true;
            }
            ix->span_slot[slot_id] = true;
            VF_HIP(hipEventRecord(s.ev_t[0], sst));
        }
        const int f8 = ix->dtype == VF_DTYPE_FP8_E4M3 ? 1 : 0;
        const int cap2 = i8conv ? 0 : (((ix->scan_impl == 3 || ((ix->scan_impl == 2 || ix->scan_impl == 4 || ix->scan_impl == 5) && !f8)) && !ix->steal_opt) ? scan2_stage_cap(ix->dp, qt, f8) : 0);
        const bool r_auto = ix->scan_impl == 2 && ix->n > kScan2rMinRows && scan2r_auto_width(ix->dp, f8 != 0) && (f8 || (s.scan_stream != s.stream && resolved_overlap(ix)));
#ifdef VF_EXPERIMENTS
        const bool dbg_r = f8 || !(ix->debug & (32 | 64));
#else
        const bool dbg_r = true;
#endif
        const int capr = ((ix->scan_impl == 5 || r_auto) && !ix->steal_opt && dbg_r && !i8conv) ? scan2r_stage_cap(ix->dp, qt, f8) : 0;
        if (ks && f8) {
            VF_HIP(launch_scan_ksplit8(a, kModeMain, p.grid, sst));
            s.scan_kernel = 7;
        } else if (ks) {
            VF_HIP(launch_scan_ksplit(a, kModeMain, p.grid, sst));
            s.scan_kernel = 6;
        } else if (p.image) {
            ScanArgs a2 = a;
            a2.stage_cap = scan2r_stage_cap(ix->dp, qt, img_f8);
            VF_HIP(launch_scan2r(a2, qt, p.grid, img_f8, sst));
            s.scan_kernel = 5;
        } else if (capr >= 256) {
            ScanArgs a2 = a;
            a2.stage_cap = capr;
            VF_HIP(launch_scan2r(a2, qt, p.grid, f8, sst));
            s.scan_kernel = 5;
        } else if (cap2 >= 256) {
            ScanArgs a2 = a;
            a2.stage_cap = cap2;
#ifdef VF_EXPERIMENTS
            if (ix->debug & 32) {
                const bool fresh = s.sib.bytes < 4096;
                VF_TRY(s.sib.ensure(4096));
                if (fresh) VF_HIP(hipMemsetAsync(s.sib.p, 0xFF, 4096, st));
                a2.sib = s.sib.as<u32>();
            }
#endif
            VF_HIP(launch_scan2(a2, qt, p.grid, f8, sst));
            s.scan_kernel = 2;
        } else {
            VF_HIP(launch_scan(a, kModeMain, qt, p.grid, (int)ix->scan_g, scan_f8(ix->dtype), sst));
            s.scan_kernel = 1;
        }
        VF_HIP(hipEventRecord(s.ev_scan, sst));
        if (s.timed && b0 == 0) {
            VF_HIP(hipEventRecord(s.ev_t[1], sst));
            const int64_t per_wave = ix->n / p.total_waves;
            const int64_t sampled = std::min<int64_t>(ix->n, (int64_t)p.total_waves * std::min<int64_t>(p.samp, per_wave));
            ix->prof_bytes = (ix->n - sampled) * (p.image ? (int64_t)ix->dp + 8 : (int64_t)ix->d * (byte_rows(ix->dtype) ? 1 : 2) + 4);
        }
        if (sst != st) VF_HIP(hipStreamWaitEvent(st, s.ev_scan, 0));
        FinalArgs f{};
        f.cnt = a.cnt; f.cand = a.cand; f.cap = p.cap; f.tau_bin = a.tau_bin; f.rows_orig = ix->rows_orig;
        f.orig_dtype = ix->dtype; f.orig_row_elems = ix->d; f.norm = ix->norm; f.qn = qn_b;
        f.d = ix->d; f.k = k; f.kprime = p.kprime; f.eps = p.eps; f.n_rows = ix->n; f.id_offset = ix->id_offset;
        f.band = p.fine_band;
        if (s.image_i8) { f.eps_q = s.epsq.as<float>(); f.band_q = s.bandq.as<int>() + qt; }
        f.out_ids = (long long*)(d_ids + (size_t)b0 * k); f.out_scores = d_scores + (size_t)b0 * k;
        f.flags = s.d_flags + b0; f.cand_count_out = s.d_counts + b0;
        f.dbg = nullptr;
        if (ix->debug & 256) { VF_TRY(s.dbg.ensure((size_t)std::max(p.total_waves * 4, 64 * 8) * sizeof(u64))); f.dbg = s.dbg.as<u64>(); }
        VF_HIP(launch_final(f, nb, st));
    }
    if (s.timed) VF_HIP(hipEventRecord(s.ev_t[3], st));
    VF_HIP(hipEventRecord(s.ev_done, st));
    return VF_OK;
}

static int end_impl(vf_index* ix, int slot_id) {
    Slot& s = ix->slots[slot_id];
    if (!s.pending) return fail(VF_EINVAL, "vf_index_search_end: slot has no pending search");
    s.pending = false;
    VF_HIP(hipEventSynchronize(s.ev_done));
    vf_search_stats stt{};
    stt.path = s.path; stt.n_queries = s.nq; stt.wide_launches = s.wide_launches; stt.wide_queries = s.wide_queries;
    stt.aux_cus = (s.path == 1 && s.scan_stream && s.scan_stream != s.stream) ? resolved_aux(ix) : 0;
    stt.scans_overlap = (s.path == 1 && resolved_overlap(ix)) ? 1 : 0;
    stt.scan_kernel = s.scan_kernel;
    stt.scan_image = (s.path == 1) ? s.scan_image : 0;
    if (s.path == 1 && s.nq > 0 && s.k > 0) {
        if (s.timed) {
            float ms = 0.f;
            if (hipEventElapsedTime(&ms, s.ev_t[0], s.ev_t[1]) == hipSuccess) { ix->prof_scan_ms += ms; ++ix->prof_launches; }
            if (hipEventElapsedTime(&ms, s.ev_t[2], s.ev_t[3]) == hipSuccess) ix->prof_pipe_ms += ms;
            s.timed = false;
        }
        std::vector<int> redo;
        for (int q = 0; q < s.nq; ++q) {
            stt.candidates += s.h_counts[q];
            stt.max_candidates = std::max<int64_t>(stt.max_candidates, s.h_counts[q]);
            if (s.h_flags[q] == 1) ++stt.uncertified;
            if (s.h_flags[q] == 2) ++stt.overflowed;
            if (s.h_flags[q] != 0) redo.push_back(q);
        }
        if (!redo.empty()) {
            const int m = (int)redo.size();
            hipStream_t st = s.stream;
            VF_TRY(s.qsel.ensure((size_t)m * ix->d * sizeof(float) + (size_t)m * s.k * (sizeof(long long) + sizeof(float))));
            float* qsel = s.qsel.as<float>();
            long long* rid = (long long*)(qsel + (size_t)m * ix->d);
            float* rsc = (float*)(rid + (size_t)m * s.k);
            for (int i = 0; i < m; ++i)
                VF_HIP(hipMemcpyAsync(qsel + (size_t)i * ix->d, s.qn.as<float>() + (size_t)redo[i] * ix->d,
                                      (size_t)ix->d * sizeof(float), hipMemcpyDeviceToDevice, st));
            for (int i0 = 0; i0 < m; i0 += kMaxBatch) {
                const int nb = std::min(kMaxBatch, m - i0);
                VF_TRY(exact_search(ix, s, qsel + (size_t)i0 * ix->d, nb, s.k, (int64_t*)(rid + (size_t)i0 * s.k),
                                    rsc + (size_t)i0 * s.k, st));
            }
            for (int i = 0; i < m; ++i) {
                VF_HIP(hipMemcpyAsync(s.d_ids + (size_t)redo[i] * s.k, rid + (size_t)i * s.k, (size_t)s.k * sizeof(long long),
                                      hipMemcpyDeviceToDevice, st));
                VF_HIP(hipMemcpyAsync(s.d_scores + (size_t)redo[i] * s.k, rsc + (size_t)i * s.k, (size_t)s.k * sizeof(float),
                                      hipMemcpyDeviceToDevice, st));
            }
            VF_HIP(hipEventRecord(s.ev_done, st));
            VF_HIP(hipEventSynchronize(s.ev_done));
            stt.exact_reruns = m;
        }
    }
    VF_HIP(hipStreamWaitEvent(s.user_stream, s.ev_done, 0));
    ix->stats = stt;
    return VF_OK;
}

static int check_search_args(vf_index* ix, const void* q, int nq, int k, const void* ids, const void* sc) {
    if (!ix) return fail(VF_EINVAL, "search: null handle");
    if (nq < 0 || k < 0) return fail(VF_EINVAL, "search: negative nq / k");
    if (nq > 0 && k > 0 && (!q || !ids || !sc)) return fail(VF_EINVAL, "search: null buffer");
    return VF_OK;
}

static int group_ensure_slot(vf_index* ix, GroupSlot& gs) {
    const size_t G = ix->shards.size();
    if (gs.feed.size() == G) return VF_OK;
    gs.feed.assign(G, nullptr); gs.ev.assign(G, nullptr);
    gs.dq.resize(G); gs.blob.resize(G);
    for (size_t g = 0; g < G; ++g) {
        VF_HIP(hipSetDevice(ix->shards[g]->device));
        VF_HIP(hipStreamCreateWithFlags(&gs.feed[g], hipStreamNonBlocking));
        VF_HIP(hipEventCreateWithFlags(&gs.ev[g], hipEventDisableTiming));
    }
    VF_HIP(hipSetDevice(ix->device));
    VF_HIP(hipEventCreateWithFlags(&gs.ev_in, hipEventDisableTiming));
    gs.hfeed.assign(G, nullptr); gs.ev_hb.assign(G, nullptr); gs.ev_home.assign(G, nullptr); gs.hb.resize(G); gs.staged_last.assign(G, 0);
    return VF_OK;
}

static bool shard_is_staged(const vf_index* ix, size_t g) { return g < ix->peer_ok.size() && !ix->peer_ok[g]; }

static int group_ensure_staged(vf_index* ix, GroupSlot& gs, size_t g) {
    if (!gs.hq_stream) {
        VF_HIP(hipSetDevice(ix->device));
        VF_HIP(hipStreamCreateWithFlags(&gs.hq_stream, hipStreamNonBlocking));
        VF_HIP(hipEventCreateWithFlags(&gs.ev_hq, hipEventDisableTiming));
    }
    if (!gs.hfeed[g]) {
        VF_HIP(hipSetDevice(ix->device));
        VF_HIP(hipStreamCreateWithFlags(&gs.hfeed[g], hipStreamNonBlocking));
        VF_HIP(hipEventCreateWithFlags(&gs.ev_home[g], hipEventDisableTiming));
        VF_HIP(hipSetDevice(ix->shards[g]->device));
        VF_HIP(hipEventCreateWithFlags(&gs.ev_hb[g], hipEventDisableTiming));
    }
    return VF_OK;
}

static int group_begin(vf_index* ix, int slot_id, const float* d_queries, int nq, int k, int64_t* d_ids, float* d_scores,
                       hipStream_t user) {
    GroupSlot& gs = ix->gslots[slot_id];
    if (gs.pending) return fail(VF_EINVAL, "vf_index_search_begin: slot already has a pending search");
    const size_t G = ix->shards.size();
    if ((size_t)G * k > 16384) return fail(VF_EUNSUPPORTED, "sharded search: shards * k > 16384");
    VF_TRY(group_ensure_slot(ix, gs));
    gs.nq = nq; gs.k = k; gs.d_ids = d_ids; gs.d_scores = d_scores; gs.user = user;
    if (nq == 0 || k == 0) { gs.pending = true; return VF_OK; }
    const size_t qbytes = (size_t)nq * ix->d * sizeof(float);
    const size_t part = (size_t)packed_part_bytes(nq, k);
    VF_HIP(hipSetDevice(ix->device));
    VF_TRY(gs.all.ensure(G * part));
    VF_HIP(hipEventRecord(gs.ev_in, user));
    size_t started = 0;
    int rc = VF_OK;
    bool host_copy_issued = false;
    for (size_t g = 0; g < G && rc == VF_OK; ++g) {
        vf_index* sh = ix->shards[g];
        const bool staged = shard_is_staged(ix, g);
        hipError_t e = hipSuccess;
        if (staged) {
            if ((rc = group_ensure_staged(ix, gs, g)) != VF_OK) break;
            if (!host_copy_issued) {
                if ((rc = gs.hq.ensure(qbytes)) != VF_OK) break;
                e = hipSetDevice(ix->device);
                if (e == hipSuccess) e = hipStreamWaitEvent(gs.hq_stream, gs.ev_in, 0);
                if (e == hipSuccess) e = hipMemcpyAsync(gs.hq.p, d_queries, qbytes, hipMemcpyDeviceToHost, gs.hq_stream);
                if (e == hipSuccess) e = hipEventRecord(gs.ev_hq, gs.hq_stream);
                if (e != hipSuccess) { rc = fail(VF_EHIP, std::string("sharded search: staged query copy (home -> host): ") + hipGetErrorString(e)); break; }
                host_copy_issued = true;
            }
        }
        e = hipSetDevice(sh->device);
        if (e == hipSuccess) e = hipStreamWaitEvent(gs.feed[g], staged ? gs.ev_hq : gs.ev_in, 0);
        if (e != hipSuccess) { rc = fail(VF_EHIP, std::string("sharded search: ") + hipGetErrorString(e)); break; }
        if ((rc = gs.dq[g].ensure(qbytes)) != VF_OK || (rc = gs.blob[g].ensure(part)) != VF_OK) break;
        if (staged) e = hipMemcpyAsync(gs.dq[g].p, gs.hq.p, qbytes, hipMemcpyHostToDevice, gs.feed[g]);
        else e = hipMemcpyPeerAsync(gs.dq[g].p, sh->device, d_queries, ix->device, qbytes, gs.feed[g]);
        if (e != hipSuccess) { rc = fail(VF_EHIP, std::string("sharded search: query ") + (staged ? "staged" : "peer") + " copy: " + hipGetErrorString(e)); break; }
        std::lock_guard<std::mutex> lk(sh->mu);
        rc = begin_impl(sh, slot_id, gs.dq[g].as<float>(), nq, k, (int64_t*)gs.blob[g].p,
                        (float*)((char*)gs.blob[g].p + (size_t)nq * k * 8), gs.feed[g]);
        if (rc == VF_OK) ++started; else sh->slots[slot_id].pending = false;
    }
    if (rc != VF_OK) {
        const std::string keep = g_err;
        for (size_t g = 0; g < started; ++g) {
            (void)hipSetDevice(ix->shards[g]->device);
            std::lock_guard<std::mutex> lk(ix->shards[g]->mu);
            (void)end_impl(ix->shards[g], slot_id);
        }
        g_err = keep;
        return rc;
    }
    gs.pending = true;
    return VF_OK;
}

static int group_end(vf_index* ix, int slot_id) {
    GroupSlot& gs = ix->gslots[slot_id];
    if (!gs.pending) return fail(VF_EINVAL, "vf_index_search_end: slot has no pending search");
    gs.pending = false;
    vf_search_stats tot{};
    tot.n_queries = gs.nq;
    if (gs.nq == 0 || gs.k == 0) { ix->stats = tot; return VF_OK; }
    const size_t G = ix->shards.size();
    const size_t part = (size_t)packed_part_bytes(gs.nq, gs.k);
    int rc = VF_OK;
    for (size_t g = 0; g < G; ++g) {
        vf_index* sh = ix->shards[g];
        (void)hipSetDevice(sh->device);
        int r;
// ... 562 lines not shown
```

### veritasfi_amd/csrc/vf_internal.h

```cpp
#pragma once
#include <hip/hip_runtime.h>
#include <math.h>
#include <stdint.h>

#include "../../include/veritasfi_hip.h"

#include <string>

#include "vf_ksplit_geom.h"

namespace vf {

int set_error(int code, const std::string& msg);

typedef unsigned long long u64;
typedef unsigned int u32;

struct DeviceGuard {
    int prev = -1;
    DeviceGuard() { if (hipGetDevice(&prev) != hipSuccess) prev = -1; }
    ~DeviceGuard() { if (prev >= 0) (void)hipSetDevice(prev); }
    DeviceGuard(const DeviceGuard&) = delete;
    DeviceGuard& operator=(const DeviceGuard&) = delete;
};

__device__ __forceinline__ u32 orderkey(float f) {
    f = f + 0.0f;
    const u32 b = __float_as_uint(f);
    return b ^ ((b >> 31) ? 0xFFFFFFFFu : 0x80000000u);
}
__device__ __forceinline__ float unorderkey(u32 k) {
    return __uint_as_float((k & 0x80000000u) ? (k ^ 0x80000000u) : ~k);
}

__device__ __forceinline__ void bitonic_sort_desc(u64* s, int n, int tid, int nthreads) {
    for (int k = 2; k <= n; k <<= 1) {
        for (int j = k >> 1; j > 0; j >>= 1) {
            for (int i = tid; i < (n >> 1); i += nthreads) {
                const int lo = ((i & ~(j - 1)) << 1) | (i & (j - 1));
                const int hi = lo | j;
                const bool desc = (lo & k) == 0;
                const u64 a = s[lo], b = s[hi];
                if ((a < b) == desc) { s[lo] = b; s[hi] = a; }
            }
            __syncthreads();
        }
    }
}

constexpr int kQueryTile = 32;
constexpr int kMaxBatch = 64;
constexpr int kRowTile = 32;
constexpr int kScanThreads = 512;
constexpr int kHistBins = 2048;
constexpr int kSmallN = 16384;
constexpr int kMaxCap = 8192;
constexpr int kCntStride = 32;
constexpr int kMaxKFused = 2048;

enum ScanMode { kModeSample = 0, kModeMain = 1 };

struct Q8Bound { float eps_add; int tau_bins, fine_bins; };
__host__ __device__ inline Q8Bound image_q8_bound(float rho_q) {
    Q8Bound b;
    if (!(rho_q < 1.0f)) { b.eps_add = INFINITY; b.tau_bins = kHistBins; b.fine_bins = 16 * kHistBins; return b; }
    const double c = (double)rho_q * (65.0 / 64.0);
    b.eps_add = (float)c;
    if ((double)b.eps_add < c) b.eps_add = nextafterf(b.eps_add, INFINITY);
    b.tau_bins = (int)ceil(c * (kHistBins / 2));
    b.fine_bins = (int)ceil(c * (kHistBins / 2) * 16);
    return b;
}
__host__ __device__ inline float image_q8_eps(float eps_img, float eps_add) {
    const float e = nextafterf(eps_img + eps_add, INFINITY) + 0x1p-20f;
    return nextafterf(e, INFINITY);
}

struct ScanArgs {
    const char* rows;
    const float* inv_scan;
    const float* off_scan;
    const float* q_scale;
    const _Float16* qimg;
    long long n;
    int dp;
    long long row_bytes;
    int total_waves;
    int samp;
    float* s0;
    const long long* wg_base;
    u32* cnt;
    int* tau_bin;
    u32* hist;
    u32* hist_coarse;
    int stage_cap;
    u64* cand;
    int cap;
    int kprime;
    int tau_band;
    const int* band_q;
    int refresh_every;
    int nq;
    u32* tile_cnt;
    int scan_grid;
    int qn_total, jtiles, rgroups;
    u32* sib;
    int sib_slack;
    unsigned long long* dbg;
    int debug;
};

struct FinalArgs {
    const u32* cnt; const u64* cand; int cap;
    int top_cap, sel_cap;
    const int* tau_bin;
    const void* rows_orig; int orig_dtype; long long orig_row_elems;
    const float* norm;
    const float* qn;
    int d; int k; int kprime; float eps;
    const float* eps_q;
    int band;
    const int* band_q;
    long long n_rows;
    long long id_offset;
    long long* out_ids; float* out_scores;
    int* flags;
    u32* cand_count_out;
    unsigned long long* dbg;
};

hipError_t launch_prep_rows(const void* rows, int dt , long long n, int d, int dp,
                            void* scan ,
                            float* norm, float* inv_scan, hipStream_t s);
hipError_t launch_prep_image(const void* rows, int dt, long long n, int d, int dp, const float* norm, unsigned char* img,
                             float* inv_img, float* off_img, u32* rho_max_bits, float* rho_sum, hipStream_t s);
hipError_t launch_prep_queries(const float* q, int nq, int d, int dp, int qn_tile ,
                               float* qn, _Float16* qimg, hipStream_t s);
hipError_t launch_normalize_rows(const void* rows, int dt , long long row0, long long nrows, int d,
                                 const float* norm, float* out, hipStream_t s);
hipError_t launch_normalize_rows_gather(const void* rows, int dt, const long long* sel , int nsel, int d,
                                        const float* norm, float* out, hipStream_t s);
hipError_t launch_dense_dot16(const float* qn, int nq, const float* cn, long long nrows, int d,
                              float* out, long long out_stride, hipStream_t s);
hipError_t launch_sort_rows(const float* scores, long long score_stride, int nq, int n, int k,
                            long long id_base, long long* out_ids, float* out_scores, int out_stride,
                            hipStream_t s);
hipError_t launch_scan(const ScanArgs& a, int mode, int qn_tile, int grid, int want_g ,
                       int f8 , hipStream_t s);
hipError_t launch_rebias_i8(const void* in, void* out, long long bytes, hipStream_t s);
hipError_t launch_debug_cvt_e4m3(const unsigned char* in, float* out, int count, hipStream_t s);
hipError_t launch_debug_mfma_i8(const signed char* A, const signed char* B, int* C, hipStream_t s);
hipError_t launch_scan2(const ScanArgs& a, int qn_tile, int grid, int rows_are_fp8, hipStream_t s);
size_t scan2_lds_bytes(int dp, int qn_tile, int stage_cap);
int scan2_stage_cap(int dp, int qn_tile, int rows_are_fp8);
size_t scan2r_lds_bytes(int dp, int qn_tile, int stage_cap, int f8);
int scan2r_stage_cap(int dp, int qn_tile, int f8);
hipError_t launch_scan2r(const ScanArgs& a, int qn_tile, int grid, int f8, hipStream_t s);
hipError_t launch_scan2r_sample(const ScanArgs& a, int qn_tile, int grid, int f8, hipStream_t s);
hipError_t launch_scan_ksplit(const ScanArgs& a, int mode, int grid, hipStream_t s);
size_t scan_ksplit_lds_bytes(int dp, int stage_cap);
int scan_ksplit_stage_cap(int dp);
hipError_t launch_scan_ksplit8(const ScanArgs& a, int mode, int grid, hipStream_t s);
size_t scan_ksplit8_lds_bytes(int dp, int stage_cap);
int scan_ksplit8_stage_cap(int dp);
hipError_t launch_scan_wide(const ScanArgs& a, int mode, int f8 , hipStream_t s);
size_t scan_wide_lds_bytes(int stage_cap);
hipError_t launch_prep_wide8(const float* qn, int nq, int d, int dp, int qtot, unsigned char* img8, float* eps_q, hipStream_t s);
hipError_t launch_scan_wide8(const ScanArgs& a, int waves , hipStream_t s);
int scan_wide8_stage_cap(int waves);
int scan_wide8_occupancy(int waves, int stage_cap);
hipError_t launch_prep_q8(const float* qn, int nq, int d, int dp, int qn_tile, int planes , signed char* img8, float* q_scale, float* eps_q, int* band_q,
                          float eps_img, int tau_band, int fine_band, hipStream_t s);
hipError_t launch_sel0(const ScanArgs& a, int qn_tile, hipStream_t s);
hipError_t launch_final(FinalArgs a, int nq, hipStream_t s);
hipError_t launch_merge_topk(const long long* ids_parts, const float* score_parts, int nparts, int nq,
                             int k, long long* ids, float* scores, hipStream_t s);
hipError_t launch_merge_topk_packed(const void* parts, int nparts, int nq, int k, long long* ids, float* scores,
                                    hipStream_t s);
hipError_t launch_fuse_rank(const float* a, const float* b, int n, float* out, long long* order,
                            hipStream_t s);
inline long long packed_part_bytes(int nq, int k) { return ((long long)nq * k * 12 + 15) / 16 * 16; }
size_t scan_lds_bytes(int dp, int qn_tile);
int scan_stage_cap(int dp, int qn_tile);
hipError_t scan_configure();

}
```

### veritasfi_amd/csrc/vf_kernels.hip

```cpp
#include "vf_internal.h"

#include <float.h>
#include <algorithm>
#include <type_traits>

#include <mutex>

namespace vf {

typedef _Float16 h8 __attribute__((ext_vector_type(8)));
typedef _Float16 h4 __attribute__((ext_vector_type(4)));
typedef float f16v __attribute__((ext_vector_type(16)));
typedef int i4v __attribute__((ext_vector_type(4)));
typedef int i16v __attribute__((ext_vector_type(16)));
typedef int i8v __attribute__((ext_vector_type(8)));

__device__ __forceinline__ float group16_tree(float acc) {
    acc = acc + __shfl_down(acc, 8, 16);
    acc = acc + __shfl_down(acc, 4, 16);
    acc = acc + __shfl_down(acc, 2, 16);
    acc = acc + __shfl_down(acc, 1, 16);
    return acc;
}

// ... 579 lines not shown
#if VF_SCAN_NT
    return __builtin_nontemporal_load(p);
#else
    return *p;
#endif
}

template <int G>
__device__ __forceinline__ void issue_loads(h8 (&buf)[4 * G], const char* rows, long long row_bytes, long long myrow,
                                            int ss , int h) {
    const char* p = rows + myrow * row_bytes + (long long)(ss * G) * 128 + h * 64;
#pragma unroll
    for (int g = 0; g < G; ++g)
#pragma unroll
        for (int i = 0; i < 4; ++i) buf[g * 4 + i] = stream_load((const h8*)(p + g * 128 + i * 16));
}

template <int NT, int G>
__device__ __forceinline__ void compute_superstep(f16v (&acc)[NT], const h8 (&buf)[4 * G], const char* lds_lane,
                                                  int ss) {
    constexpr int QN = NT * kQueryTile;
    const char* base = lds_lane + (long long)(ss * G) * (8 * QN * 16);
#pragma unroll
    for (int g = 0; g < G; ++g)
#pragma unroll
        for (int i = 0; i < 4; ++i)
#pragma unroll
            for (int nt = 0; nt < NT; ++nt) {
                const h8 b = *(const h8*)(base + (g * 8 + i) * (QN * 16) + nt * (kQueryTile * 16));
                acc[nt] = __builtin_amdgcn_mfma_f32_32x32x16_f16(buf[g * 4 + i], b, acc[nt], 0, 0, 0);
            }
}

typedef _Float16 h2v __attribute__((ext_vector_type(2)));

__device__ __forceinline__ h8 cvt8_e4m3(u32 w0, u32 w1) {
    const h2v a = __builtin_amdgcn_cvt_scalef32_pk_f16_fp8(w0, 1.0f, false);
    const h2v b = __builtin_amdgcn_cvt_scalef32_pk_f16_fp8(w0, 1.0f, true);
    const h2v c = __builtin_amdgcn_cvt_scalef32_pk_f16_fp8(w1, 1.0f, false);
    const h2v d = __builtin_amdgcn_cvt_scalef32_pk_f16_fp8(w1, 1.0f, true);
    h8 r;
    r[0] = a[0]; r[1] = a[1]; r[2] = b[0]; r[3] = b[1]; r[4] = c[0]; r[5] = c[1]; r[6] = d[0]; r[7] = d[1];
    return r;
}

__device__ __forceinline__ h8 cvt8_i8b(u32 w0, u32 w1) {
    const h2v off = {(_Float16)-1152.0f, (_Float16)-1152.0f};
    const h2v a = __builtin_bit_cast(h2v, __builtin_amdgcn_perm(0x64646464u, w0, 0x04010400u)) + off;
    const h2v b = __builtin_bit_cast(h2v, __builtin_amdgcn_perm(0x64646464u, w0, 0x04030402u)) + off;
    const h2v c = __builtin_bit_cast(h2v, __builtin_amdgcn_perm(0x64646464u, w1, 0x04010400u)) + off;
    const h2v d = __builtin_bit_cast(h2v, __builtin_amdgcn_perm(0x64646464u, w1, 0x04030402u)) + off;
    h8 r;
    r[0] = a[0]; r[1] = a[1]; r[2] = b[0]; r[3] = b[1]; r[4] = c[0]; r[5] = c[1]; r[6] = d[0]; r[7] = d[1];
    return r;
}

template <int G>
__device__ __forceinline__ void issue_loads_f8(uint4 (&buf)[2 * G], const char* rows, long long row_bytes, long long myrow,
                                               int ss, int h) {
    const char* p = rows + myrow * row_bytes + (long long)(ss * G) * 64 + h * 32;
#pragma unroll
    for (int g = 0; g < G; ++g)
#pragma unroll
        for (int i = 0; i < 2; ++i) {
            typedef unsigned int u4v __attribute__((ext_vector_type(4)));
            const u4v w = stream_load((const u4v*)(p + g * 64 + i * 16));
            buf[g * 2 + i] = make_uint4(w[0], w[1], w[2], w[3]);
        }
}

template <int NT, int G, int F8 = 1>
__device__ __forceinline__ void compute_superstep_f8(f16v (&acc)[NT], const uint4 (&buf)[2 * G], const char* lds_lane,
                                                     int ss) {
    constexpr int QN = NT * kQueryTile;
    const char* base = lds_lane + (long long)(ss * G) * (8 * QN * 16);
#pragma unroll
    for (int g = 0; g < G; ++g)
#pragma unroll
        for (int i = 0; i < 4; ++i) {
            const uint4 w = buf[g * 2 + (i >> 1)];
            h8 afrag;
            if constexpr (F8 == 2) afrag = (i & 1) ? cvt8_i8b(w.z, w.w) : cvt8_i8b(w.x, w.y);
            else afrag = (i & 1) ? cvt8_e4m3(w.z, w.w) : cvt8_e4m3(w.x, w.y);
#pragma unroll
            for (int nt = 0; nt < NT; ++nt) {
                const h8 b = *(const h8*)(base + (g * 8 + i) * (QN * 16) + nt * (kQueryTile * 16));
                acc[nt] = __builtin_amdgcn_mfma_f32_32x32x16_f16(afrag, b, acc[nt], 0, 0, 0);
            }
        }
}

__global__ void k_debug_cvt_e4m3(const unsigned char* in, float* out, int count) {
    const int i = blockIdx.x * blockDim.x + threadIdx.x;
    if (i * 8 >= count) return;
    u32 w0 = 0, w1 = 0;
    for (int j = 0; j < 4; ++j) {
        w0 |= (u32)(i * 8 + j < count ? in[i * 8 + j] : 0) << (8 * j);
        w1 |= (u32)(i * 8 + 4 + j < count ? in[i * 8 + 4 + j] : 0) << (8 * j);
    }
    const h8 r = cvt8_e4m3(w0, w1);
    for (int j = 0; j < 8; ++j) if (i * 8 + j < count) out[i * 8 + j] = (float)r[j];
}

hipError_t launch_debug_cvt_e4m3(const unsigned char* in, float* out, int count, hipStream_t s) {
    if (count <= 0) return hipSuccess;
    const int groups = (count + 7) / 8;
    hipLaunchKernelGGL(k_debug_cvt_e4m3, dim3((groups + 63) / 64), dim3(64), 0, s, in, out, count);
    return hipGetLastError();
}

__global__ __launch_bounds__(64) void k_debug_mfma_i8(const signed char* A, const signed char* B, int* C) {
    const int lane = threadIdx.x, r = lane & 31, h = lane >> 5;
    const i4v a = *(const i4v*)(A + r * 32 + 16 * h), b = *(const i4v*)(B + r * 32 + 16 * h);
    i16v acc;
#pragma unroll
    for (int e = 0; e < 16; ++e) acc[e] = 0;
    acc = __builtin_amdgcn_mfma_i32_32x32x32_i8(a, b, acc, 0, 0, 0);
#pragma unroll
    for (int e = 0; e < 16; ++e) C[((e & 3) + 8 * (e >> 2) + 4 * h) * 32 + r] = acc[e];
}

hipError_t launch_debug_mfma_i8(const signed char* A, const signed char* B, int* C, hipStream_t s) {
    hipLaunchKernelGGL(k_debug_mfma_i8, dim3(1), dim3(64), 0, s, A, B, C);
    return hipGetLastError();
}

__device__ __forceinline__ int wave_tau_two_level(const u32* coarse_q, const u32* fine_q, int kprime,
                                                            int lane) {
    const u32 c = __hip_atomic_load(coarse_q + lane, __ATOMIC_RELAXED, __HIP_MEMORY_SCOPE_AGENT);
    u32 suf = c;
#pragma unroll
    for (int off = 1; off < 64; off <<= 1) {
        const u32 v = __shfl_down(suf, off);
        if (lane + off < 64) suf += v;
    }
    const u32 above = suf - c;
    const unsigned long long cross = __ballot(above < (u32)kprime && suf >= (u32)kprime);
    if (cross == 0ull) return -1;
    const int L = __ffsll((long long)cross) - 1;
    const u32 aboveL = (u32)__shfl((int)above, L);
    const u32 f = lane < 32 ? __hip_atomic_load(fine_q + L * 32 + lane, __ATOMIC_RELAXED, __HIP_MEMORY_SCOPE_AGENT) : 0u;
    u32 sf = f;
#pragma unroll
    for (int off = 1; off < 32; off <<= 1) {
        const u32 v = __shfl_down(sf, off);
        if (lane + off < 32) sf += v;
    }
    const unsigned long long ok = __ballot(lane < 32 && aboveL + sf >= (u32)kprime);
    if (ok == 0ull) return -1;
    return L * 32 + (63 - __clzll((long long)ok));
}

constexpr int kCtlBytes = 272;

template <int NT>
__device__ __forceinline__ constexpr int QN_of() { return NT * kQueryTile; }

template <int NT>
struct EpiRegs {
    float inv_lane;
    int tau_g[NT];
    bool sync_tau;
    const char* inv_lds = nullptr;
    float off_lane = 0.0f;
};

#define VF_DPP_ROR(v, n) (u32) __builtin_amdgcn_update_dpp(0, (int)(v), 0x120 + (n), 0xF, 0xF, false)
__device__ __forceinline__ u32 wave_or_u32(u32 v) {
    v |= VF_DPP_ROR(v, 1);
    v |= VF_DPP_ROR(v, 2);
    v |= VF_DPP_ROR(v, 4);
    v |= VF_DPP_ROR(v, 8);
    return (u32)(__builtin_amdgcn_readlane((int)v, 0) | __builtin_amdgcn_readlane((int)v, 16) |
                 __builtin_amdgcn_readlane((int)v, 32) | __builtin_amdgcn_readlane((int)v, 48));
}
__device__ __forceinline__ u32 wave_sum_u32(u32 v) {
    v += VF_DPP_ROR(v, 1);
    v += VF_DPP_ROR(v, 2);
    v += VF_DPP_ROR(v, 4);
    v += VF_DPP_ROR(v, 8);
    return (u32)(__builtin_amdgcn_readlane((int)v, 0) + __builtin_amdgcn_readlane((int)v, 16) +
                 __builtin_amdgcn_readlane((int)v, 32) + __builtin_amdgcn_readlane((int)v, 48));
}

template <int NT, int MODE>
__device__ __forceinline__ void epi_prefetch(EpiRegs<NT>& e, const ScanArgs& a, long long t0, int lane, bool sync_tau) {
    e.inv_lane = a.inv_scan[t0 + (lane & 31)];
    e.sync_tau = sync_tau;
    if (MODE == kModeMain && sync_tau) {
#pragma unroll
        for (int nt = 0; nt < NT; ++nt)
            e.tau_g[nt] = __hip_atomic_load(a.tau_bin + nt * kQueryTile + (lane & 31), __ATOMIC_RELAXED,
                                            __HIP_MEMORY_SCOPE_AGENT);
    }
}

template <int NT, int MODE, bool PUBLISH = true, bool INV_LDS = false, bool OFF = false>
__device__ __forceinline__ void tile_epilogue(const ScanArgs& a, const f16v (&acc)[NT], const EpiRegs<NT>& e,
                                              long long t0, long long hi, long long s0_slot, int lane, char* ctl) {
    const int r31 = lane & 31, h = lane >> 5;
    auto inv_of = [&](int reg) {
        const int r0 = (reg & 3) + 8 * (reg >> 2);
        const float lo_half = __builtin_bit_cast(float, __builtin_amdgcn_readlane(__builtin_bit_cast(int, e.inv_lane), r0));
        const float hi_half = __builtin_bit_cast(float, __builtin_amdgcn_readlane(__builtin_bit_cast(int, e.inv_lane), r0 + 4));
        return h ? hi_half : lo_half;
    };
    auto off_of = [&](int reg) {
        const int r0 = (reg & 3) + 8 * (reg >> 2);
        const float lo_half = __builtin_bit_cast(float, __builtin_amdgcn_readlane(__builtin_bit_cast(int, e.off_lane), r0));
        const float hi_half = __builtin_bit_cast(float, __builtin_amdgcn_readlane(__builtin_bit_cast(int, e.off_lane), r0 + 4));
        return h ? hi_half : lo_half;
    };
    if (MODE == kModeSample) {
        const long long s0_stride = (long long)a.total_waves * a.samp;
#pragma unroll
        for (int nt = 0; nt < NT; ++nt) {
            const int q = nt * kQueryTile + r31;
#pragma unroll
            for (int reg = 0; reg < 16; ++reg) {
                const int rr = (reg & 3) + 8 * (reg >> 2) + 4 * h;
                if constexpr (OFF) {
                    if (t0 + rr < hi) a.s0[(long long)q * s0_stride + s0_slot + rr] = acc[nt][reg] * inv_of(reg) + off_of(reg);
                } else {
                    if (t0 + rr < hi) a.s0[(long long)q * s0_stride + s0_slot + rr] = acc[nt][reg] * inv_of(reg);
                }
            }
        }
        return;
    }
    int* tau_lds = (int*)(ctl + 16);
    if (e.sync_tau && lane < 32) {
#pragma unroll
        for (int nt = 0; nt < NT; ++nt) atomicMax(tau_lds + nt * kQueryTile + lane, e.tau_g[nt]);
    }
    float inv16[16];
    if constexpr (INV_LDS) {
#pragma unroll
        for (int g = 0; g < 4; ++g) {
            const float4 v = *(const float4*)(e.inv_lds + (8 * g + 4 * h) * 4);
            inv16[4 * g] = v.x; inv16[4 * g + 1] = v.y; inv16[4 * g + 2] = v.z; inv16[4 * g + 3] = v.w;
        }
    } else {
#pragma unroll
        for (int reg = 0; reg < 16; ++reg) inv16[reg] = inv_of(reg);
    }
    float off16[16];
    if constexpr (OFF) {
        static_assert(INV_LDS, "the offsets ride in the scratch half the inverse norms' DMA fills");
#pragma unroll
        for (int g = 0; g < 4; ++g) {
            const float4 v = *(const float4*)(e.inv_lds + 128 + (8 * g + 4 * h) * 4);
            off16[4 * g] = v.x; off16[4 * g + 1] = v.y; off16[4 * g + 2] = v.z; off16[4 * g + 3] = v.w;
        }
    }
    const long long left = hi - t0;
    const int lf = __builtin_amdgcn_readfirstlane((int)(left < kRowTile ? left : kRowTile));
    if (lf < kRowTile) {
#pragma unroll
        for (int reg = 0; reg < 16; ++reg) inv16[reg] = ((reg & 3) + 8 * (reg >> 2) + 4 * h) < lf ? inv16[reg] : __builtin_nanf("");
    }
    typedef float mvec __attribute__((ext_vector_type(NT * 16)));
    mvec m;
    float tb[NT];
    bool any = false;
#pragma unroll
    for (int nt = 0; nt < NT; ++nt) {
        const int q = nt * kQueryTile + r31;
        const int t = tau_lds[q];
        tb[nt] = q < a.nq ? (t <= 0 ? -INFINITY : (float)t) : INFINITY;
        float top = -INFINITY;
#pragma unroll
        for (int reg = 0; reg < 16; ++reg) {
            if constexpr (OFF) m[nt * 16 + reg] = acc[nt][reg] * inv16[reg] + off16[reg];
            else m[nt * 16 + reg] = acc[nt][reg] * inv16[reg];
            top = fmaxf(top, m[nt * 16 + reg]);
        }
        any |= bin_x(top) >= tb[nt];
    }
    if (__ballot(any) == 0ull) return;
    u32 mask = 0;
#pragma unroll
    for (int nt = 0; nt < NT; ++nt)
#pragma unroll
        for (int reg = 0; reg < 16; ++reg) mask |= (bin_x(m[nt * 16 + reg]) >= tb[nt]) ? (1u << (nt * 16 + reg)) : 0u;
    const unsigned long long hot = __ballot(mask != 0u);
    if (hot == 0ull) return;
    if (a.debug & 4) return;
    u32 umask = 0u, total = 0u;
    if (__popcll(hot) <= 8) {
        for (unsigned long long hb = hot; hb != 0ull; hb &= hb - 1ull) {
            const u32 m = (u32)__builtin_amdgcn_readlane((int)mask, __builtin_ctzll(hb));
            umask |= m;
            total += (u32)__popc(m);
        }
    } else {
        umask = wave_or_u32(mask);
        total = wave_sum_u32((u32)__popc(mask));
    }
    u32* stage_cnt = (u32*)ctl;
    uint4* stage_ent = (uint4*)(ctl + kCtlBytes);
    const u32 rs = 31u - (u32)__builtin_clz((u32)a.refresh_every | 1u);
    const u32 R = 1u << rs;
    u32 base = 0;
    if (lane == 0) base = atomicAdd(stage_cnt, total);
    base = (u32)__builtin_amdgcn_readfirstlane((int)base);
    const bool need = (base >> rs) != ((base + total) >> rs);
    if (a.debug & 8) return;
    u32 run = base;
    const u32 edge = (((base + total) >> rs) << rs) - 1u;
    int qq = 0;
    for (u32 um = umask; um != 0u; um &= um - 1u) {
        const int pair = __builtin_ctz(um);
        const int nt = pair >> 4, reg = pair & 15;
        const int q = nt * kQueryTile + r31;
        const bool mine = ((mask >> pair) & 1u) != 0u;
        const unsigned long long bal = __ballot(mine);
        if (mine) {
            const u32 slot = run + __builtin_amdgcn_mbcnt_hi((u32)(bal >> 32), __builtin_amdgcn_mbcnt_lo((u32)bal, 0u));
            const int rr = (reg & 3) + 8 * (reg >> 2) + 4 * h;
            const float sc = m[pair];
            const u32 bin = (u32)bin_of_x(bin_x(sc));
            const u32 key = orderkey(sc), row = (u32)(t0 + rr);
            if (slot < (u32)a.stage_cap) {
                stage_ent[slot] = make_uint4(row, key, (u32)q | (bin << 8), 1u);
            } else {
                const u32 gs = atomicAdd(a.cnt + q * kCntStride, 1u);
                if (gs < (u32)a.cap) a.cand[(long long)q * a.cap + gs] = ((u64)key << 32) | (u64)row;
                atomicAdd(a.hist + (long long)q * kHistBins + bin, 1u);
                atomicAdd(a.hist_coarse + q * 64 + (bin >> 5), 1u);
            }
        }
        const u32 nxt = run + (u32)__popcll(bal);
        if (run <= edge && edge < nxt) qq = nt * kQueryTile + ((__ffsll((long long)bal) - 1) & 31);
        run = nxt;
    }
    if (a.debug & 2) return;
    if constexpr (!PUBLISH) return;
    if (need) {
        const int nb = wave_tau_two_level(a.hist_coarse + qq * 64, a.hist + (long long)qq * kHistBins, a.kprime, lane) - (a.band_q ? a.band_q[qq] : a.tau_band);
        if (lane == 0 && nb > 0) {
            atomicMax(a.tau_bin + qq, nb);
            atomicMax(tau_lds + qq, nb);
        }
        for (u32 blk = base >> rs; blk < (base + total) >> rs; ++blk)
        for (u32 j = (u32)lane; j < R; j += 64u) {
            const u32 idx = (blk << rs) + j;
            if (idx >= (u32)a.stage_cap) break;
            const uint4 en = stage_ent[idx];
            if (en.w == 1u) {
                const u32 q = en.z & 0xFFu, bin = en.z >> 8;
                if (q < (u32)QN_of<NT>() && bin < (u32)kHistBins) {
                    atomicAdd(a.hist + (long long)q * kHistBins + bin, 1u);
                    atomicAdd(a.hist_coarse + q * 64 + (bin >> 5), 1u);
                }
            }
        }
    }
}

#define VF_ISSUE(BUF, ...)                                                        \
    do {                                                                          \
        if constexpr (F8 != 0) issue_loads_f8<G>(BUF, __VA_ARGS__);               \
        else issue_loads<G>(BUF, __VA_ARGS__);                                    \
    } while (0)
#define VF_COMPUTE(ACC, BUF, ...)                                                 \
    do {                                                                          \
        if constexpr (F8 != 0) compute_superstep_f8<NT, G, F8>(ACC, BUF, __VA_ARGS__); \
        else compute_superstep<NT, G>(ACC, BUF, __VA_ARGS__);                      \
    } while (0)

template <int NT, int G, int MODE, int F8>
__global__ __launch_bounds__(kScanThreads) void k_scan(ScanArgs a) {
    extern __shared__ __attribute__((aligned(16))) char smem[];
    constexpr int QN = NT * kQueryTile;
    constexpr int WAVES = kScanThreads / 64;
    const int tid = threadIdx.x;
    const int lane = tid & 63, wid = tid >> 6;
    const int r31 = lane & 31, h = lane >> 5;
    const long long grid = (MODE == kModeSample && a.scan_grid > 0) ? a.scan_grid : gridDim.x;
    const long long swg = (long long)a.samp * WAVES;
    long long lo, hi;
    int ntiles;
    auto part_of = [&](long long v, long long& plo, long long& phi) {
        const long long Ra = a.n * v / grid, Rb = a.n * (v + 1) / grid;
        const long long Rs = (Ra + swg < Rb) ? Ra + swg : Rb;
        plo = MODE == kModeSample ? Ra : Rs;
        phi = MODE == kModeSample ? Rs : Rb;
    };
    part_of(blockIdx.x, lo, hi);
    ntiles = (int)((hi - lo + kRowTile - 1) / kRowTile);
    const int tps = (int)((swg + kRowTile - 1) / kRowTile);
    if (MODE == kModeSample) {
        const long long mine = ((long long)grid - blockIdx.x + gridDim.x - 1) / gridDim.x;
        ntiles = (int)(mine > 0 ? mine : 0) * tps;
    }
    auto sample_tile = [&](int tile, long long& t0, long long& thi, long long& sbase) {
        const int m = tile / tps, j = tile - m * tps;
        const long long v = blockIdx.x + (long long)m * gridDim.x;
        long long plo, phi;
        part_of(v < grid ? v : grid - 1, plo, phi);
        t0 = plo + (long long)j * kRowTile;
        thi = phi;
        sbase = v * swg + (long long)j * kRowTile;
    };
    constexpr int kPoolDiv = 12;
    const bool pooled = MODE == kModeMain && a.tile_cnt != nullptr;
    auto pool_of = [&](long long v, long long& plo, long long& phi) {
        part_of(v, plo, phi);
        const int nt_v = (int)((phi - plo + kRowTile - 1) / kRowTile);
        plo += (long long)(nt_v - nt_v / kPoolDiv) * kRowTile;
        if (plo > phi) plo = phi;
    };
    if (pooled) {
        const int nloc = ntiles - ntiles / kPoolDiv;
        hi = lo + (long long)nloc * kRowTile < hi ? lo + (long long)nloc * kRowTile : hi;
        ntiles = nloc;
    }
    const int SS = (a.dp >> 6) / G;
    char* ctl = smem + (size_t)a.dp * QN * 2;
    u32* next_tile = (u32*)(ctl + 4);
    u32* const own_cnt = next_tile;

    typedef typename std::conditional<F8 != 0, uint4, h8>::type stage_t;
    stage_t A0[F8 ? 2 * G : 4 * G], A1[F8 ? 2 * G : 4 * G];
    EpiRegs<NT> epi;
    int cur_tile = wid, claimed = 0x7fffffff, tiles_done = 0;
    bool active = cur_tile < ntiles;
    u32 lo32 = (u32)lo + (u32)r31, hi32m1 = (u32)(hi - 1);
    auto rowof = [&](int tile) {
        if (MODE == kModeSample) {
            long long t0s, this_, sb;
            sample_tile(tile < ntiles ? tile : (ntiles > 0 ? ntiles - 1 : 0), t0s, this_, sb);
            const long long r = t0s + r31;
            return r < this_ - 1 ? r : this_ - 1;
        }
        const u32 r = lo32 + (u32)tile * kRowTile;
        return (long long)(r < hi32m1 ? r : hi32m1);
    };
    if (active) VF_ISSUE(A0, a.rows, a.row_bytes, rowof(cur_tile), 0, h);
    {
        const uint4* src = (const uint4*)a.qimg;
        uint4* dst = (uint4*)smem;
        const int nvec = (a.dp >> 3) * QN;
#pragma unroll 4
        for (int i = tid; i < nvec; i += kScanThreads) dst[i] = src[i];
        uint4* z = (uint4*)ctl;
        const int nz = (MODE == kModeMain) ? (kCtlBytes / 16 + a.stage_cap) : 1;
        for (int i = tid; i < nz; i += kScanThreads) z[i] = make_uint4(0u, (i == 0) ? (u32)WAVES : 0u, 0u, 0u);
    }
    __syncthreads();
    if (MODE == kModeMain && tid < QN) ((int*)(ctl + 16))[tid] = a.tau_bin[tid];
    __syncthreads();
    const char* lds_lane = smem + ((4 * h) * QN + r31) * 16;
    unsigned long long* dbg = (MODE == kModeMain && (a.debug & 128) && a.dbg && lane == 0)
                                  ? a.dbg + ((long long)blockIdx.x * WAVES + wid) * 4 : nullptr;
    if (dbg) dbg[0] = wall_clock64();

    u32* seg_cnt = own_cnt;
    long long s0_base = (long long)blockIdx.x * swg;
    for (;;) {
    if (active) {
        f16v acc[NT];
#pragma unroll
        for (int nt = 0; nt < NT; ++nt)
#pragma unroll
            for (int e = 0; e < 16; ++e) acc[nt][e] = 0.0f;
        const int pairs = SS >> 1;
        while (true) {
            long long t0 = lo + (long long)cur_tile * kRowTile, t_hi = hi, t_s0 = s0_base + (t0 - lo);
            if (MODE == kModeSample) sample_tile(cur_tile, t0, t_hi, t_s0);
            {
                int v_ = 0;
                if (lane == 0) v_ = (int)atomicAdd(seg_cnt, 1u);
                claimed = __builtin_amdgcn_readfirstlane(v_);
            }
            const long long myrow = rowof(cur_tile);
            for (int p = 0; p + 1 < pairs; ++p) {
                VF_ISSUE(A1, a.rows, a.row_bytes, myrow, 2 * p + 1, h);
                __builtin_amdgcn_sched_barrier(0);
                VF_COMPUTE(acc, A0, lds_lane, 2 * p);
// ... 550 lines not shown
    constexpr int passes = 1;
#endif
    int tiles_done = 0;
    for (int pass = 0; pass < passes; ++pass) {
    if (pass > 0) {
        asm volatile("s_waitcnt vmcnt(0)" ::: "memory");
        __syncthreads();
        if (tid == 0) *next_tile = (u32)kScan2Waves;
        __syncthreads();
        cur_tile = wid;
        if (active) {
            src_cur = src_of(cur_tile);
            issue_epi(lo + (long long)cur_tile * kRowTile, !kScan2Service, tiles_done & 1);
#pragma unroll
            for (int sg = 0; sg < kRing; ++sg) issue_seg(src_cur, sg, sg);
        }
    }
    if (active) {
        f16v acc[NT];
#pragma unroll
        for (int nt = 0; nt < NT; ++nt)
#pragma unroll
            for (int e = 0; e < 16; ++e) acc[nt][e] = 0.0f;
        int buf = 0;
        while (true) {
            const long long t0 = lo + (long long)cur_tile * kRowTile;
            int claimed;
            {
                int v_ = 0;
                if (lane == 0) v_ = (int)atomicAdd(next_tile, 1u);
                claimed = __builtin_amdgcn_readfirstlane(v_);
            }
            const bool more = claimed < ntiles;
            const int nxt = more ? claimed : cur_tile;
            src_nxt = src_of(nxt);
            const bool sync_now = !kScan2Service && (tiles_done & (kScan2Waves - 1)) == wid;
            const bool sync_next = !kScan2Service && ((tiles_done + 1) & (kScan2Waves - 1)) == wid;
            if (dbg && dbg_rec > 4 && tiles_done < 64) dbg[4 + tiles_done] = wall_clock64();
            for (int sg = 0; sg < S; ++sg) {
                asm volatile("s_waitcnt vmcnt(8)" ::: "memory");
                const char* ab = a_lane + buf * kSegBytes;
                if constexpr (F8 == 0) {
                    const char* bb = lds_lane + (long long)sg * (8 * QN * 16);
#pragma unroll
                    for (int i = 0; i < 4; ++i) {
                        const h8 af = *(const h8*)(ab + (((4 * h + i) ^ asw) << 4));
#pragma unroll
                        for (int nt = 0; nt < NT; ++nt) {
                            const h8 bf = *(const h8*)(bb + i * (QN * 16) + nt * (kQueryTile * 16));
                            acc[nt] = __builtin_amdgcn_mfma_f32_32x32x16_f16(af, bf, acc[nt], 0, 0, 0);
                        }
                    }
                } else {
#pragma unroll
                    for (int c = 0; c < 2; ++c) {
                        const uint4 w0 = *(const uint4*)(ab + (((4 * c + 2 * h) ^ asw) << 4));
                        const uint4 w1 = *(const uint4*)(ab + (((4 * c + 2 * h + 1) ^ asw) << 4));
                        const char* bb = lds_lane + (long long)(sg * 16 + c * 8) * (QN * 16);
#pragma unroll
                        for (int i = 0; i < 4; ++i) {
                            const uint4 w = i < 2 ? w0 : w1;
                            const h8 af = (i & 1) ? cvt8_e4m3(w.z, w.w) : cvt8_e4m3(w.x, w.y);
#pragma unroll
                            for (int nt = 0; nt < NT; ++nt) {
                                const h8 bf = *(const h8*)(bb + i * (QN * 16) + nt * (kQueryTile * 16));
                                acc[nt] = __builtin_amdgcn_mfma_f32_32x32x16_f16(af, bf, acc[nt], 0, 0, 0);
                            }
                        }
                    }
                }
                asm volatile("s_waitcnt lgkmcnt(0)" ::: "memory");
                const int s3 = sg + kRing;
                if (s3 < S) issue_seg(src_cur, s3, buf);
                else {
                    if (s3 == S) issue_epi(lo + (long long)nxt * kRowTile, sync_next, (tiles_done + 1) & 1);
                    issue_seg(src_nxt, s3 - S, buf);
                }
                buf = buf + 1 == kRing ? 0 : buf + 1;
            }
            const char* sc = scratch + (tiles_done & 1) * 512;
            EpiRegs<NT> epi;
            epi.inv_lane = *(const float*)(sc + 256 + r31 * 4);
            epi.inv_lds = sc + 256;
            epi.sync_tau = sync_now;
            if (sync_now) {
#pragma unroll
                for (int nt = 0; nt < NT; ++nt) epi.tau_g[nt] = *(const int*)(sc + (nt * kQueryTile + r31) * 4);
            }
            tile_epilogue<NT, MODE, !kScan2Service, true>(a, acc, epi, t0, hi, 0, lane, ctl);
#pragma unroll
            for (int nt = 0; nt < NT; ++nt)
#pragma unroll
                for (int e = 0; e < 16; ++e) acc[nt][e] = 0.0f;
            ++tiles_done;
            if (!more) break;
            cur_tile = nxt;
            src_cur = src_nxt;
        }
    }
    }
    if (dbg && dbg_rec > 4) dbg[69] = (unsigned long long)tiles_done;
    asm volatile("s_waitcnt vmcnt(0)" ::: "memory");
    if (!service && lane == 0) atomicAdd((u32*)(ctl + 8), 1u);
    if (dbg) dbg[1] = wall_clock64();
    __syncthreads();
    if (dbg) dbg[2] = wall_clock64();
    {
        const u32 staged = *(const u32*)ctl;
        const u32 nst = staged < (u32)a.stage_cap ? staged : (u32)a.stage_cap;
        uint4* ent = (uint4*)(ctl + kCtlBytes);
        u32* qcnt = (u32*)img;
        u32* qbase = qcnt + QN;
        if (tid < QN) qcnt[tid] = 0u;
        __syncthreads();
        for (u32 i = tid; i < nst; i += kScan2Threads) {
            const uint4 e = ent[i];
            const u32 q = e.z & 0xFFu;
            if (e.w != 1u || q >= (u32)QN) continue;
            ent[i].w = 2u + atomicAdd(qcnt + q, 1u);
        }
        __syncthreads();
        if (tid < QN) {
            const u32 c = qcnt[tid];
            qbase[tid] = c ? atomicAdd(a.cnt + tid * kCntStride, c) : 0u;
        }
        __syncthreads();
        for (u32 i = tid; i < nst; i += kScan2Threads) {
            const uint4 e = ent[i];
            if (e.w < 2u) continue;
            const u32 q = e.z & 0xFFu;
            const u32 gs = qbase[q] + (e.w - 2u);
            if (gs < (u32)a.cap) a.cand[(long long)q * a.cap + gs] = ((u64)e.y << 32) | (u64)e.x;
        }
    }
    if (dbg) dbg[3] = wall_clock64();
}

struct Scan2rShape { int S, RB, RING; };
static Scan2rShape scan2r_shape(int dp, int f8) {
    if (!f8 && dp == 768) return {12, 6, 6};
    if (!f8 && dp == 1024) return {16, 6, 4};
    if (!f8 && dp == 512) return {8, 4, 6};
    if (!f8 && dp == 384) return {6, 3, 6};
    if (f8 == 3) return dp == 768 ? Scan2rShape{6, 6, 6} : Scan2rShape{0, 0, 0};
    if (f8 == 4) return dp == 768 ? Scan2rShape{6, 3, 6} : Scan2rShape{0, 0, 0};
    if (f8 && dp == 768) return {6, 3, 6};
    if (f8 && dp == 1024) return {8, 3, 4};
    return {0, 0, 0};
}

size_t scan2r_lds_bytes(int dp, int qn_tile, int stage_cap, int f8) {
    const Scan2rShape sh = scan2r_shape(dp, f8);
    const size_t seg_img = (size_t)(f8 ? 128 : 64) * qn_tile * 2;
    return (size_t)(sh.S - sh.RB) * seg_img + (size_t)kScan2Waves * (sh.RING * kSegBytes + kScratchBytes) + kCtlBytes + (size_t)stage_cap * 16;
}
int scan2r_stage_cap(int dp, int qn_tile, int f8) {
    if (scan2r_shape(dp, f8).S == 0) return 0;
    const size_t fixed = scan2r_lds_bytes(dp, qn_tile, 0, f8);
    if (fixed + 256 * 16 > 160 * 1024) return 0;
    const size_t area = std::min<size_t>(160 * 1024 - fixed, 32 * 1024);
    return (int)(area / 16);
}

template <int NT, int MODE, int F8 = 0, int S = 12, int RB = 6, int RING = 6, int AR = 1>
__global__ __launch_bounds__(kScan2Waves * 64) void k_scan2r(ScanArgs a) {
    const unsigned long long t_entry = (a.debug & 512) ? wall_clock64() : 0ull;
    const unsigned long long c_entry = (a.debug & 512) ? __builtin_amdgcn_s_memtime() : 0ull;
    extern __shared__ __attribute__((aligned(1024))) char smem[];
    constexpr int QN = NT * kQueryTile, THREADS = kScan2Waves * 64;
    constexpr bool I8 = F8 >= 3;
    constexpr int PLANES = F8 == 4 ? 2 : 1;
    constexpr int J = I8 ? 4 * PLANES : F8 ? 8 : 4;
    constexpr int SEGIMG = J * 2 * QN * 16;
    auto frag_off = [](int j) { return I8 ? (2 * (j & 3) * PLANES + (j >> 2)) * (QN * 16) : F8 ? ((j >> 2) * 8 + (j & 3)) * (QN * 16) : j * (QN * 16); };
    static_assert(F8 != 3 || RB == S, "the single int8 plane lives in registers whole: no LDS part");
    static_assert(S >= RING && RB <= S && RB <= 6, "ring fill and the spelled-out register segments");
    const int tid = threadIdx.x, lane = tid & 63, wid = tid >> 6;
    const int r31 = lane & 31, h = lane >> 5;
    const long long grid = (MODE == kModeSample && a.scan_grid > 0) ? a.scan_grid : gridDim.x;
    const long long swg = (long long)a.samp * (kScanThreads / 64);
    const int tps = (int)((swg + kRowTile - 1) / kRowTile);
    long long lo = 0, hi = 0;
    int ntiles;
    if (MODE == kModeSample) {
        const long long mine = (grid - (long long)blockIdx.x + gridDim.x - 1) / gridDim.x;
        ntiles = (int)(mine > 0 ? mine : 0) * tps;
    } else {
        const long long Ra = a.n * blockIdx.x / grid, Rb = a.n * (blockIdx.x + 1) / grid;
        lo = (Ra + swg < Rb) ? Ra + swg : Rb; hi = Rb;
        ntiles = (int)((hi - lo + kRowTile - 1) / kRowTile);
    }
    auto tile_rows = [&](int tile, long long& t0, long long& thi, long long& sbase) {
        if (MODE == kModeSample) {
            const int m = tile / tps, j = tile - m * tps;
            long long v = (long long)blockIdx.x + (long long)m * gridDim.x;
            v = v < grid ? v : grid - 1;
            const long long Ra = a.n * v / grid, Rb = a.n * (v + 1) / grid;
            thi = (Ra + swg < Rb) ? Ra + swg : Rb;
            t0 = Ra + (long long)j * kRowTile;
            sbase = v * swg + (long long)j * kRowTile;
        } else {
            t0 = lo + (long long)tile * kRowTile; thi = hi; sbase = 0;
        }
    };
    h8 breg[RB][J][NT];
    {
        const char* qb = (const char*)a.qimg + ((long long)((I8 ? PLANES : 4) * h) * QN + r31) * 16;
#pragma unroll
        for (int sg = 0; sg < RB; ++sg)
#pragma unroll
            for (int j = 0; j < J; ++j)
#pragma unroll
                for (int nt = 0; nt < NT; ++nt)
                    breg[sg][j][nt] = *(const h8*)(qb + (long long)sg * SEGIMG + frag_off(j) + nt * (kQueryTile * 16));
    }
    float sq[NT];
#pragma unroll
    for (int nt = 0; nt < NT; ++nt) sq[nt] = I8 ? a.q_scale[nt * kQueryTile + r31] : 1.0f;
    char* ring = smem + (size_t)wid * (RING * kSegBytes);
    char* img = smem + kScan2Waves * RING * kSegBytes;
    constexpr size_t kImgBytes = (size_t)(S - RB) * SEGIMG;
    char* scratch = img + kImgBytes + (size_t)wid * kScratchBytes;
    char* ctl = img + kImgBytes + kScan2Waves * kScratchBytes;
    u32* next_tile = (u32*)(ctl + 4);
    const unsigned ring_l = (unsigned)__builtin_amdgcn_readfirstlane((int)lds_addr(ring)), scratch_l = (unsigned)__builtin_amdgcn_readfirstlane((int)lds_addr(scratch));
    const int drow = lane >> 3;
    struct TileSrc { unsigned long long ua; unsigned v[4]; };
    auto src_of = [&](int tile) -> TileSrc {
        long long t0_, thi_, sb_;
        tile_rows(tile, t0_, thi_, sb_);
        TileSrc ts;
        const long long last_row = thi_ - 1 > 0 ? thi_ - 1 : 0;
        long long base_row = t0_ > 0 ? t0_ : 0;
        base_row = base_row < last_row ? base_row : last_row;
        ts.ua = (unsigned long long)(a.rows + base_row * a.row_bytes);
        ts.ua = ((unsigned long long)(unsigned)__builtin_amdgcn_readfirstlane((int)(ts.ua >> 32)) << 32) | (unsigned)__builtin_amdgcn_readfirstlane((int)ts.ua);
#pragma unroll
        for (int m = 0; m < 4; ++m) {
            const int row = 8 * m + drow;
            long long r = t0_ + row;
            r = r < last_row ? r : last_row;
            r = r > base_row ? r : base_row;
            ts.v[m] = (unsigned)((r - base_row) * a.row_bytes) + ((((lane & 7) ^ ((row >> 1) & 7))) << 4);
        }
        return ts;
    };
    auto first_row = [&](int tile) {
        long long t0_, thi_, sb_;
        tile_rows(tile, t0_, thi_, sb_);
        const long long last_row = thi_ - 1 > 0 ? thi_ - 1 : 0;
        return t0_ < last_row ? t0_ : last_row;
    };
    auto issue_seg = [&](const TileSrc& src, int seg, int buf) {
        dma16x4(src.ua + (unsigned long long)seg * 128ull, src.v[0], src.v[1], src.v[2], src.v[3], ring_l + buf * kSegBytes);
    };
    auto issue_epi = [&](long long t0, bool sync_tau, int par) {
        par = __builtin_amdgcn_readfirstlane(par);
        dma4((F8 >= 2 && h) ? a.off_scan + t0 + r31 : a.inv_scan + t0 + r31, scratch_l + par * 512 + 256);
        if (sync_tau) dma4(a.tau_bin + (lane < QN ? lane : QN - 1), scratch_l + par * 512);
    };
    int cur_tile = __builtin_amdgcn_readfirstlane(wid);
    const bool active = cur_tile < ntiles;
    TileSrc src_cur{}, src_nxt{};
    if (active) {
        src_cur = src_of(cur_tile);
        issue_epi(first_row(cur_tile), MODE == kModeMain, 0);
#pragma unroll
        for (int sg = 0; sg < RING; ++sg) issue_seg(src_cur, sg, sg);
    }
    typedef unsigned int u4r __attribute__((ext_vector_type(4)));
    {
        const char* srcq = (const char*)a.qimg + (long long)RB * SEGIMG;
        constexpr int nkb = (int)(kImgBytes >> 10);
        const unsigned img_l = (unsigned)__builtin_amdgcn_readfirstlane((int)lds_addr(img));
        const int wu = __builtin_amdgcn_readfirstlane(wid);
        for (int c = wu; c < nkb; c += kScan2Waves) dma16(srcq + ((long long)c << 10) + (lane << 4), img_l + ((unsigned)c << 10));
        __builtin_amdgcn_s_waitcnt(0x0F70);
        if constexpr (AR) {
#pragma unroll
            for (int sg = 0; sg < RB; ++sg)
#pragma unroll
                for (int j = 0; j < J; ++j)
#pragma unroll
                    for (int nt = 0; nt < NT; ++nt) asm volatile("" : "+a"(breg[sg][j][nt]));
        }
        uint4* z = (uint4*)ctl;
        const int nz = kCtlBytes / 16 + (MODE == kModeMain ? a.stage_cap : 0);
        for (int i = tid; i < nz; i += THREADS) z[i] = make_uint4(0u, (i == 0) ? (u32)kScan2Waves : 0u, 0u, 0u);
    }
    __syncthreads();
    if (MODE == kModeMain) {
        if (tid < QN) ((int*)(ctl + 16))[tid] = a.tau_bin[tid];
        __syncthreads();
    }

    const char* lds_lane = img + (((I8 ? PLANES : 4) * h) * QN + r31) * 16;
    const int asw = (r31 >> 1) & 7;
    const char* a_lane = ring + r31 * 128;
    const int dbg_rec = (a.debug & 512) ? 72 : 4;
    unsigned long long* dbg = (MODE == kModeMain && (a.debug & 128) && a.dbg && lane == 0) ? a.dbg + ((long long)blockIdx.x * kScan2Waves + wid) * dbg_rec : nullptr;
    if (dbg) dbg[0] = wall_clock64();
    if (dbg && dbg_rec > 4) {
        dbg[68] = t_entry;
        unsigned hw_id, xcc_id;
        asm volatile("s_getreg_b32 %0, hwreg(HW_REG_HW_ID)\n\ts_getreg_b32 %1, hwreg(HW_REG_XCC_ID)" : "=s"(hw_id), "=s"(xcc_id));
        dbg[70] = ((unsigned long long)xcc_id << 32) | hw_id;
    }
#ifdef VF_EXPERIMENTS
    const bool prof = (a.debug & 4096) != 0;
    unsigned long long pc_wait = 0, pc_use = 0, pc_fill = 0, pc_head = 0, pc_epi = 0, pc_n = 0, pt0 = 0, pt1 = 0;
    auto cyc = [&]() { unsigned long long t; asm volatile("s_memtime %0\n\ts_waitcnt lgkmcnt(0)" : "=s"(t) :: "memory"); return t; };
#define VF_PC(stmt) if (prof) { stmt; }
#else
#define VF_PC(stmt)
#endif
    int tiles_done = 0;
    if (active) {
        f16v acc[NT];
        i16v acci[PLANES][NT];
#pragma unroll
        for (int nt = 0; nt < NT; ++nt)
#pragma unroll
            for (int e = 0; e < 16; ++e) {
                acc[nt][e] = 0.0f;
#pragma unroll
                for (int pl = 0; pl < PLANES; ++pl) acci[pl][nt][e] = 0;
            }
        int buf = 0;
        while (true) {
            VF_PC(pt0 = cyc())
            long long t0, t_hi, t_s0;
            tile_rows(cur_tile, t0, t_hi, t_s0);
            int claimed;
            {
                int v_ = 0;
                if (lane == 0) v_ = (int)atomicAdd(next_tile, 1u);
                claimed = __builtin_amdgcn_readfirstlane(v_);
            }
            const bool more = claimed < ntiles;
            const int nxt = more ? claimed : cur_tile;
            src_nxt = src_of(nxt);
            const bool sync_now = MODE == kModeMain && (tiles_done & (kScan2Waves - 1)) == wid;
            const bool sync_next = MODE == kModeMain && ((tiles_done + 1) & (kScan2Waves - 1)) == wid;
            if (dbg && dbg_rec > 4 && tiles_done < 64) dbg[4 + tiles_done] = wall_clock64();
            VF_PC(pt1 = cyc(); pc_head += pt1 - pt0)
            auto consume = [&](auto sg_c, const char* bb) {
                constexpr int sgc = decltype(sg_c)::value;
                VF_PC(pt0 = cyc())
                if constexpr (RING == 6) asm volatile("s_waitcnt vmcnt(20)" ::: "memory");
                else if constexpr (RING == 5) asm volatile("s_waitcnt vmcnt(16)" ::: "memory");
                else asm volatile("s_waitcnt vmcnt(12)" ::: "memory");
                static_assert(RING >= 4 && RING <= 6, "the counted waits above");
                VF_PC(pt1 = cyc(); pc_wait += pt1 - pt0; ++pc_n)
                const char* ab = a_lane + buf * kSegBytes;
                auto bfrag = [&](int j, int nt) -> h8 {
                    if constexpr (sgc >= 0) {
                        return breg[sgc < 0 ? 0 : sgc][j][nt];
                    } else {
                        return *(const h8*)(bb + frag_off(j) + nt * (kQueryTile * 16));
                    }
                };
                if constexpr (I8) {
                    i4v af[4];
                    h8 bl[J][NT];
#pragma unroll
                    for (int i = 0; i < 4; ++i) af[i] = *(const i4v*)(ab + (((2 * i + h) ^ asw) << 4));
                    if constexpr (sgc < 0) {
#pragma unroll
                        for (int j = 0; j < J; ++j)
#pragma unroll
                            for (int nt = 0; nt < NT; ++nt) bl[j][nt] = bfrag(j, nt);
                    }
                    __builtin_amdgcn_sched_barrier(0);
#pragma unroll
                    for (int i = 0; i < 4; ++i) {
                        const i4v ax = af[i] ^ (int)0x80808080;
#pragma unroll
                        for (int pl = 0; pl < PLANES; ++pl)
#pragma unroll
                            for (int nt = 0; nt < NT; ++nt)
                                acci[pl][nt] = __builtin_amdgcn_mfma_i32_32x32x32_i8(ax, __builtin_bit_cast(i4v, sgc < 0 ? bl[4 * pl + i][nt] : bfrag(4 * pl + i, nt)),
                                                                                     acci[pl][nt], 0, 0, 0);
                    }
                } else if constexpr (F8 == 0) {
                    if constexpr (AR) {
                        h8 af[4], bl[4][NT];
#pragma unroll
                        for (int i = 0; i < 4; ++i) af[i] = *(const h8*)(ab + (((4 * h + i) ^ asw) << 4));
                        if constexpr (sgc < 0) {
#pragma unroll
                            for (int i = 0; i < 4; ++i)
#pragma unroll
                                for (int nt = 0; nt < NT; ++nt) bl[i][nt] = bfrag(i, nt);
                        }
                        __builtin_amdgcn_sched_barrier(0);
#pragma unroll
                        for (int i = 0; i < 4; ++i)
#pragma unroll
                            for (int nt = 0; nt < NT; ++nt)
                                acc[nt] = __builtin_amdgcn_mfma_f32_32x32x16_f16(af[i], sgc < 0 ? bl[i][nt] : bfrag(i, nt), acc[nt], 0, 0, 0);
                    } else {
#pragma unroll
                        for (int i = 0; i < 4; ++i) {
                            const h8 af = *(const h8*)(ab + (((4 * h + i) ^ asw) << 4));
#pragma unroll
                            for (int nt = 0; nt < NT; ++nt) acc[nt] = __builtin_amdgcn_mfma_f32_32x32x16_f16(af, bfrag(i, nt), acc[nt], 0, 0, 0);
                        }
                    }
                } else {
                    uint4 wv[4];
                    h8 bl[8][NT];
#pragma unroll
                    for (int c = 0; c < 2; ++c) {
                        wv[2 * c] = *(const uint4*)(ab + (((4 * c + 2 * h) ^ asw) << 4));
                        wv[2 * c + 1] = *(const uint4*)(ab + (((4 * c + 2 * h + 1) ^ asw) << 4));
                    }
                    if constexpr (sgc < 0) {
#pragma unroll
                        for (int j = 0; j < 8; ++j)
#pragma unroll
                            for (int nt = 0; nt < NT; ++nt) bl[j][nt] = bfrag(j, nt);
                    }
                    __builtin_amdgcn_sched_barrier(0);
#pragma unroll
                    for (int c = 0; c < 2; ++c) {
#ifdef VF_EXPERIMENTS
                        if (c == 1 && (a.debug & 32)) break;
#endif
                        const uint4 w0 = wv[2 * c], w1 = wv[2 * c + 1];
#pragma unroll
                        for (int i = 0; i < 4; ++i) {
                            const uint4 w = i < 2 ? w0 : w1;
                            h8 af;
#ifdef VF_EXPERIMENTS
                            if (a.debug & 64) {
                                const u4r raw = {(i & 1) ? w.z : w.x, (i & 1) ? w.w : w.y, (i & 1) ? w.z : w.x, (i & 1) ? w.w : w.y};
                                af = __builtin_bit_cast(h8, raw);
                            } else
#endif
                            if constexpr (F8 == 2) af = (i & 1) ? cvt8_i8b(w.z, w.w) : cvt8_i8b(w.x, w.y);
                            else af = (i & 1) ? cvt8_e4m3(w.z, w.w) : cvt8_e4m3(w.x, w.y);
#pragma unroll
                            for (int nt = 0; nt < NT; ++nt)
                                acc[nt] = __builtin_amdgcn_mfma_f32_32x32x16_f16(af, sgc < 0 ? bl[4 * c + i][nt] : bfrag(4 * c + i, nt), acc[nt], 0, 0, 0);
                        }
                    }
                }
                asm volatile("s_waitcnt lgkmcnt(0)" ::: "memory");
                VF_PC(pt0 = cyc(); pc_use += pt0 - pt1)
            };
            auto refill = [&](int sg) {
                const int s3 = sg + RING;
                if (s3 < S) issue_seg(src_cur, s3, buf);
                else {
                    if (s3 == S) issue_epi(first_row(nxt), sync_next, (tiles_done + 1) & 1);
                    issue_seg(src_nxt, s3 - S, buf);
                }
                buf = buf + 1 == RING ? 0 : buf + 1;
                VF_PC(pt1 = cyc(); pc_fill += pt1 - pt0)
            };
#define VF_R_SEG(N) if constexpr (RB > N) { consume(std::integral_constant<int, N>{}, nullptr); refill(N); }
            VF_R_SEG(0) VF_R_SEG(1) VF_R_SEG(2) VF_R_SEG(3) VF_R_SEG(4) VF_R_SEG(5)
#undef VF_R_SEG
            for (int sg = RB; sg < S; ++sg) {
                consume(std::integral_constant<int, -1>{}, lds_lane + (long long)(sg - RB) * SEGIMG);
                refill(sg);
            }
            VF_PC(pt0 = cyc())
            const char* sc = scratch + (tiles_done & 1) * 512;
            EpiRegs<NT> epi;
            epi.inv_lane = *(const float*)(sc + 256 + r31 * 4);
            epi.inv_lds = sc + 256;
            if constexpr (F8 >= 2) epi.off_lane = *(const float*)(sc + 384 + r31 * 4);
            if constexpr (I8) {
#pragma unroll
                for (int nt = 0; nt < NT; ++nt)
#pragma unroll
                    for (int e = 0; e < 16; ++e) {
                        float v = (float)acci[0][nt][e];
                        if constexpr (PLANES == 2) { v = v * 254.0f + (float)acci[1][nt][e]; acci[1][nt][e] = 0; }
                        acc[nt][e] = v * sq[nt];
                        acci[0][nt][e] = 0;
                    }
            }
            epi.sync_tau = sync_now;
            if (sync_now) {
#pragma unroll
                for (int nt = 0; nt < NT; ++nt) epi.tau_g[nt] = *(const int*)(sc + (nt * kQueryTile + r31) * 4);
            }
            tile_epilogue<NT, MODE, true, true, F8 >= 2>(a, acc, epi, t0, t_hi, t_s0, lane, ctl);
#pragma unroll
            for (int nt = 0; nt < NT; ++nt)
#pragma unroll
                for (int e = 0; e < 16; ++e) acc[nt][e] = 0.0f;
            VF_PC(pt1 = cyc(); pc_epi += pt1 - pt0)
            ++tiles_done;
            if (!more) break;
            cur_tile = nxt;
            src_cur = src_nxt;
        }
    }
    if (dbg && dbg_rec > 4) dbg[69] = (unsigned long long)tiles_done;
    asm volatile("s_waitcnt vmcnt(0)" ::: "memory");
    if (MODE == kModeSample) return;
    if (lane == 0) atomicAdd((u32*)(ctl + 8), 1u);
    if (dbg) dbg[1] = wall_clock64();
    __syncthreads();
    if (dbg) dbg[2] = wall_clock64();
    {
        const u32 staged = *(const u32*)ctl;
        const u32 nst = staged < (u32)a.stage_cap ? staged : (u32)a.stage_cap;
        uint4* ent = (uint4*)(ctl + kCtlBytes);
        u32* qcnt = (u32*)(kImgBytes ? img : smem);
        u32* qbase = qcnt + QN;
        if (tid < QN) qcnt[tid] = 0u;
        __syncthreads();
        for (u32 i = tid; i < nst; i += THREADS) {
            const uint4 e = ent[i];
            const u32 q = e.z & 0xFFu;
            if (e.w != 1u || q >= (u32)QN) continue;
            ent[i].w = 2u + atomicAdd(qcnt + q, 1u);
        }
        __syncthreads();
        if (tid < QN) {
            const u32 c = qcnt[tid];
            qbase[tid] = c ? atomicAdd(a.cnt + tid * kCntStride, c) : 0u;
        }
        __syncthreads();
        for (u32 i = tid; i < nst; i += THREADS) {
            const uint4 e = ent[i];
            if (e.w < 2u) continue;
            const u32 q = e.z & 0xFFu;
            const u32 gs = qbase[q] + (e.w - 2u);
            if (gs < (u32)a.cap) a.cand[(long long)q * a.cap + gs] = ((u64)e.y << 32) | (u64)e.x;
        }
    }
    if (dbg && dbg_rec > 4) dbg[71] = __builtin_amdgcn_s_memtime() - c_entry;
#ifdef VF_EXPERIMENTS
    if (dbg && dbg_rec > 4 && prof) { dbg[4] = pc_wait; dbg[5] = pc_use; dbg[6] = pc_fill; dbg[7] = pc_head; dbg[8] = pc_epi; dbg[9] = pc_n; }
#endif
#undef VF_PC
    if (dbg) dbg[3] = wall_clock64();
}

constexpr int kWideQ = 256, kWideNT = kWideQ / kQueryTile, kWideKC = 64, kWideRows = 256;
#ifndef VF_WIDE_THREADS
#define VF_WIDE_THREADS 512
#endif
constexpr int kWideThreads = VF_WIDE_THREADS, kWideWaves = kWideThreads / 64, kWideM = kWideRows / kWideWaves / kRowTile;
constexpr int kWideBuf = (kWideKC / 8) * kWideQ * 16;
constexpr int kWideCtl = 16 + 3 * kWideQ * 4;
constexpr int kSampWaves = kScanThreads / 64;

template <int F8> struct WideStage { uint4 w[kWideM][4]; };
template <int F8> __device__ __forceinline__ constexpr int wide_dc() { return F8 ? 2 : 1; }

template <int F8>
__device__ __forceinline__ void wide_issue_a(WideStage<F8>& st, const char* rows, long long row_bytes, const long long (&row)[kWideM],
                                             int unit, int h) {
#pragma unroll
    for (int m = 0; m < kWideM; ++m) {
        if constexpr (F8 != 0) {
            const char* p = rows + row[m] * row_bytes + (long long)unit * 128 + h * 32;
            st.w[m][0] = *(const uint4*)p;
            st.w[m][1] = *(const uint4*)(p + 16);
            st.w[m][2] = *(const uint4*)(p + 64);
            st.w[m][3] = *(const uint4*)(p + 80);
        } else {
            const char* p = rows + row[m] * row_bytes + (long long)unit * 128 + h * 64;
#pragma unroll
            for (int i = 0; i < 4; ++i) st.w[m][i] = *(const uint4*)(p + i * 16);
        }
    }
}

template <int F8, int CC>
__device__ __forceinline__ void wide_compute(f16v (&acc)[kWideM][kWideNT], const WideStage<F8>& st, const char* lds_lane,
                                             const char* next_lane, h8 (&bq)[4]) {
    auto frag_at = [&](int sn) {
        const char* base = sn < 4 * kWideNT ? lds_lane : next_lane;
        const int s2 = sn < 4 * kWideNT ? sn : sn - 4 * kWideNT;
        return *(const h8*)(base + (s2 / kWideNT) * (kWideQ * 16) + (s2 % kWideNT) * (kQueryTile * 16));
    };
#pragma unroll
    for (int i = 0; i < 4; ++i) {
        h8 afrag[kWideM];
#pragma unroll
        for (int m = 0; m < kWideM; ++m) {
            if constexpr (F8 != 0) {
                const uint4 w = st.w[m][2 * CC + (i >> 1)];
                if constexpr (F8 == 2) afrag[m] = (i & 1) ? cvt8_i8b(w.z, w.w) : cvt8_i8b(w.x, w.y);
                else afrag[m] = (i & 1) ? cvt8_e4m3(w.z, w.w) : cvt8_e4m3(w.x, w.y);
            } else {
                afrag[m] = __builtin_bit_cast(h8, st.w[m][i]);
            }
        }
#pragma unroll
        for (int nt = 0; nt < kWideNT; ++nt) {
            const int sidx = i * kWideNT + nt;
#pragma unroll
            for (int m = 0; m < kWideM; ++m) acc[m][nt] = __builtin_amdgcn_mfma_f32_32x32x16_f16(afrag[m], bq[sidx % 4], acc[m][nt], 0, 0, 0);
            __builtin_amdgcn_sched_group_barrier(0x008, kWideM, 0);
            bq[(sidx + 3) % 4] = frag_at(sidx + 3);
            __builtin_amdgcn_sched_group_barrier(0x100, 1, 0);
        }
    }
}

template <int Q = kWideQ, int THREADS = kWideThreads>
__device__ __forceinline__ void wide_flush(const ScanArgs& a, char* ctl, int jt, int tid) {
    constexpr int kWideQ = Q, kWideThreads = THREADS, kWideCtl = 16 + 3 * Q * 4;
    u32* stage_cnt = (u32*)ctl;
    u32* qcnt = (u32*)(ctl + 16 + kWideQ * 4);
    u32* qbase = qcnt + kWideQ;
    uint4* ent = (uint4*)(ctl + kWideCtl);
    __syncthreads();
    const u32 staged = *stage_cnt;
    const u32 nst = staged < (u32)a.stage_cap ? staged : (u32)a.stage_cap;
    if (tid < kWideQ) qcnt[tid] = 0u;
    __syncthreads();
    const u32 published = staged & ~((u32)a.refresh_every - 1u);
    for (u32 i = tid; i < nst; i += kWideThreads) {
        const uint4 e = ent[i];
        const u32 q = e.z & 0xFFu;
        if (e.w != 1u) continue;
        ent[i].w = 2u + atomicAdd(qcnt + q, 1u);
        if (i >= published) {
            const u32 bin = e.z >> 8, gq = (u32)jt * kWideQ + q;
            if (bin < (u32)kHistBins) {
                atomicAdd(a.hist + (long long)gq * kHistBins + bin, 1u);
                atomicAdd(a.hist_coarse + gq * 64 + (bin >> 5), 1u);
            }
        }
    }
    __syncthreads();
    if (tid < kWideQ) {
        const u32 c = qcnt[tid];
        qbase[tid] = c ? atomicAdd(a.cnt + ((long long)jt * kWideQ + tid) * kCntStride, c) : 0u;
    }
    __syncthreads();
    for (u32 i = tid; i < nst; i += kWideThreads) {
        const uint4 e = ent[i];
        if (e.w >= 2u) {
            const u32 q = e.z & 0xFFu;
            const u32 gs = qbase[q] + (e.w - 2u);
            if (gs < (u32)a.cap) a.cand[((long long)jt * kWideQ + q) * a.cap + gs] = ((u64)e.y << 32) | (u64)e.x;
        }
        ent[i] = make_uint4(0u, 0u, 0u, 0u);
    }
    if (tid == 0) *stage_cnt = 0u;
    __syncthreads();
}


template <int MODE, int NT = kWideNT, int Q = kWideQ>
__device__ __forceinline__ void wide_epilogue(const ScanArgs& a, const f16v (&acc)[NT], float inv_lane, long long t0,
                                              long long hi, long long s0_slot, int jt, int lane, char* ctl, bool sync_tau,
                                              int q0 = 0 ,
                                              unsigned long long* ph = nullptr ) {
    constexpr int kWideQ = Q, kWideCtl = 16 + 3 * Q * 4;
    const int r31 = lane & 31, h = lane >> 5;
    unsigned long long pc0 = ph ? wall_clock64() : 0ull;
    auto ph_mark = [&](int i) { if (ph) { const unsigned long long n_ = wall_clock64(); ph[i] += n_ - pc0; pc0 = n_; } };
    auto inv_of = [&](int reg) {
        const int r0 = (reg & 3) + 8 * (reg >> 2);
        const float lo_half = __builtin_bit_cast(float, __builtin_amdgcn_readlane(__builtin_bit_cast(int, inv_lane), r0));
        const float hi_half = __builtin_bit_cast(float, __builtin_amdgcn_readlane(__builtin_bit_cast(int, inv_lane), r0 + 4));
        return h ? hi_half : lo_half;
    };
    const int qg0 = jt * kWideQ;
    if (MODE == kModeSample) {
        const long long s0_stride = (long long)a.rgroups * a.samp * kSampWaves;
#pragma unroll
        for (int nt = 0; nt < NT; ++nt) {
            const int q = qg0 + q0 + nt * kQueryTile + r31;
#pragma unroll
            for (int reg = 0; reg < 16; ++reg) {
                const int rr = (reg & 3) + 8 * (reg >> 2) + 4 * h;
                if (t0 + rr < hi) a.s0[(long long)q * s0_stride + s0_slot + rr] = acc[nt][reg] * inv_of(reg);
            }
        }
        return;
    }
    int* tau_lds = (int*)(ctl + 16);
    if (sync_tau) {
#pragma unroll
        for (int nt = 0; nt < NT; ++nt) {
// ... 962 lines not shown
#define VF_SCAN2R_SHAPES(X, NT, MODE) VF_SCAN2R_PRODUCT(X, NT, MODE)
#endif
#define VF_SCAN2R_ALL(X) VF_SCAN2R_SHAPES(X, 1, kModeMain) VF_SCAN2R_SHAPES(X, 2, kModeMain) VF_SCAN2R_SHAPES(X, 1, kModeSample) VF_SCAN2R_SHAPES(X, 2, kModeSample)
static hipError_t launch_scan2r_any(const ScanArgs& a, int qn_tile, int mode, int grid, int f8, size_t lds, hipStream_t s) {
    Scan2rShape sh = scan2r_shape(a.dp, f8);
#ifdef VF_EXPERIMENTS
    if (f8 == 1 && a.dp == 768 && (a.debug & 2048)) sh.RING = 4;
#endif
    const int nt = qn_tile / kQueryTile;
    bool done = false;
    const int ar = (!f8 && a.dp == 768 && (a.debug & 1024)) ? 0 : 1;
#define VF_X(NT, MODE, F8, S_, RB_, RING_, AR_) \
    if (!done && nt == NT && mode == MODE && f8 == F8 && sh.S == S_ && sh.RB == RB_ && sh.RING == RING_ && ar == AR_) { \
        hipLaunchKernelGGL((k_scan2r<NT, MODE, F8, S_, RB_, RING_, AR_>), dim3(grid), dim3(kScan2Waves * 64), lds, s, a); done = true; }
    VF_SCAN2R_ALL(VF_X)
#undef VF_X
    return done ? hipGetLastError() : hipErrorInvalidValue;
}
hipError_t launch_scan2r(const ScanArgs& a, int qn_tile, int grid, int f8, hipStream_t s) {
    return launch_scan2r_any(a, qn_tile, kModeMain, grid, f8, scan2r_lds_bytes(a.dp, qn_tile, a.stage_cap, f8), s);
}
hipError_t launch_scan2r_sample(const ScanArgs& a, int qn_tile, int grid, int f8, hipStream_t s) {
    return launch_scan2r_any(a, qn_tile, kModeSample, grid, f8, scan2r_lds_bytes(a.dp, qn_tile, 0, f8), s);
}

template <int NT, int G, int MODE>
static hipError_t configure_one() {
    hipError_t e = hipFuncSetAttribute((const void*)k_scan<NT, G, MODE, 0>, hipFuncAttributeMaxDynamicSharedMemorySize,
                                       160 * 1024);
    if (e != hipSuccess) return e;
    e = hipFuncSetAttribute((const void*)k_scan<NT, G, MODE, 2>, hipFuncAttributeMaxDynamicSharedMemorySize, 160 * 1024);
    if (e != hipSuccess) return e;
    return hipFuncSetAttribute((const void*)k_scan<NT, G, MODE, 1>, hipFuncAttributeMaxDynamicSharedMemorySize, 160 * 1024);
}

__device__ __forceinline__ int wave_tau_from_lds(const u32* lh, int kprime, int lane) {
    u32 hv[32];
    u32 sum = 0;
#pragma unroll
    for (int i = 0; i < 32; ++i) { hv[i] = lh[lane * 32 + i]; sum += hv[i]; }
    u32 suf = sum;
#pragma unroll
    for (int off = 1; off < 64; off <<= 1) {
        const u32 v = __shfl_down(suf, off);
        if (lane + off < 64) suf += v;
    }
    const u32 above = suf - sum;
    int best = -1;
    if (above < (u32)kprime && suf >= (u32)kprime) {
        u32 run = above;
        bool found = false;
#pragma unroll
        for (int i = 31; i >= 0; --i) {
            run += hv[i];
            if (!found && run >= (u32)kprime) { best = lane * 32 + i; found = true; }
        }
    }
#pragma unroll
    for (int off = 32; off; off >>= 1) best = max(best, __shfl_xor(best, off));
    return best;
}

__global__ __launch_bounds__(1024) void k_sel0(ScanArgs a) {
    __shared__ u32 lh[kHistBins];
    __shared__ u32 lcnt;
    __shared__ int sbin;
    const int q = blockIdx.x, tid = threadIdx.x;
    for (int b = tid; b < kHistBins; b += 1024) lh[b] = 0;
    if (tid == 0) { lcnt = 0; sbin = 0; }
    __syncthreads();
    const long long len = (long long)a.total_waves * a.samp;
    const float* s = a.s0 + (long long)q * len;
    const long long swg = (long long)a.samp * (kScanThreads / 64);
    constexpr int kKeep = 32;
    float v[kKeep];
    const bool in_regs = len <= (long long)kKeep * 1024;
    __shared__ float wave_thr[16];
    float pre = -INFINITY;
    if (q < a.nq) {
        if (in_regs) {
            float mx = -INFINITY;
#pragma unroll
            for (int u = 0; u < kKeep; ++u) {
                const long long i = tid + (long long)u * 1024;
                const float x = s[i < len ? i : len - 1];
                v[u] = i < len ? x : -INFINITY;
                mx = fmaxf(mx, v[u]);
            }
            if (a.kprime <= 1024) {
                const int rounds = (a.kprime + 15) / 16;
                const int lane = tid & 63;
                float cur = mx, thr = -INFINITY;
                for (int i = 0; i < rounds; ++i) {
                    float wm = cur;
#pragma unroll
                    for (int o = 32; o; o >>= 1) wm = fmaxf(wm, __shfl_xor(wm, o));
                    thr = wm;
                    const unsigned long long bal = __ballot(cur == wm);
                    if (bal && lane == __ffsll((long long)bal) - 1) cur = -INFINITY;
                }
                if (lane == 0) wave_thr[tid >> 6] = thr;
                __syncthreads();
                pre = wave_thr[0];
#pragma unroll
                for (int w = 1; w < 16; ++w) pre = fminf(pre, wave_thr[w]);
            }
#pragma unroll
            for (int u = 0; u < kKeep; ++u)
                if (v[u] > -INFINITY && v[u] >= pre) atomicAdd(&lh[bin_of_x(bin_x(v[u]))], 1u);
        } else {
            for (long long i = tid; i < len; i += 1024) {
                const float x = s[i];
                if (x > -INFINITY) atomicAdd(&lh[bin_of_x(bin_x(x))], 1u);
            }
        }
    }
    __syncthreads();
    if (tid < 64) {
        const int nb = wave_tau_from_lds(lh, a.kprime, tid);
        const int band = (a.band_q && q < a.nq) ? a.band_q[q] : a.tau_band;
        if (tid == 0) sbin = nb - band > 0 ? nb - band : 0;
    }
    __syncthreads();
    const int tb = sbin;
    auto emit = [&](float x, long long i) {
        if (x > -INFINITY && bin_of_x(bin_x(x)) >= tb) {
            const u32 slot = atomicAdd(&lcnt, 1u);
            const u32 wg = (u32)i / (u32)swg;
            const long long row = a.wg_base[wg] + (long long)((u32)i - wg * (u32)swg);
            if (slot < (u32)a.cap) a.cand[(long long)q * a.cap + slot] = ((u64)orderkey(x) << 32) | (u64)(u32)row;
        }
    };
    if (q < a.nq) {
        if (in_regs) {
#pragma unroll
            for (int u = 0; u < kKeep; ++u) emit(v[u], tid + (long long)u * 1024);
        } else {
            for (long long i = tid; i < len; i += 1024) emit(s[i], i);
        }
    }
    __syncthreads();
    for (int b = tid; b < kHistBins; b += 1024) a.hist[(long long)q * kHistBins + b] = (q < a.nq && b >= tb) ? lh[b] : 0u;
    if (tid < 64) {
        u32 c = 0;
#pragma unroll
        for (int i = 0; i < 32; ++i) {
            const int b = tid * 32 + i;
            c += (q < a.nq && b >= tb) ? lh[b] : 0u;
        }
        a.hist_coarse[q * 64 + tid] = c;
    }
    if (tid == 0) {
        a.cnt[q * kCntStride] = lcnt;
        a.tau_bin[q] = (q < a.nq && !(a.debug & 1)) ? tb : kHistBins;
    }
    if (q == 0 && a.tile_cnt)
        for (int i = tid; i < a.scan_grid; i += 1024) a.tile_cnt[i] = 0u;
}

hipError_t launch_sel0(const ScanArgs& a, int qn_tile, hipStream_t s) {
    hipLaunchKernelGGL(k_sel0, dim3(qn_tile), dim3(1024), 0, s, a);
    return hipGetLastError();
}

constexpr int kFinalThreads = 256;

__device__ __forceinline__ void rank_select_desc(const u64* keys, int n, u64* out, int limit, int tid) {
    for (int i0 = tid; i0 < n; i0 += 4 * kFinalThreads) {
        u64 mine[4];
        int rank[4];
#pragma unroll
        for (int u = 0; u < 4; ++u) {
            const int i = i0 + u * kFinalThreads;
            mine[u] = i < n ? keys[i] : 0ull;
            rank[u] = 0;
        }
        int j = 0;
        for (; j + 16 <= n; j += 16) {
            u64 kj[16];
#pragma unroll
            for (int t = 0; t < 16; ++t) kj[t] = keys[j + t];
#pragma unroll
            for (int t = 0; t < 16; ++t)
#pragma unroll
                for (int u = 0; u < 4; ++u) rank[u] += kj[t] > mine[u] ? 1 : 0;
        }
        for (; j < n; ++j) {
            const u64 kj = keys[j];
#pragma unroll
            for (int u = 0; u < 4; ++u) rank[u] += kj > mine[u] ? 1 : 0;
        }
#pragma unroll
        for (int u = 0; u < 4; ++u)
            if (i0 + u * kFinalThreads < n && rank[u] < limit) out[rank[u]] = mine[u];
    }
}

template <int DT> struct RowVec;
template <> struct RowVec<VF_DTYPE_F16> { typedef uint4 type; };
template <> struct RowVec<VF_DTYPE_FP8_E4M3> { typedef uint2 type; };
template <> struct RowVec<VF_DTYPE_INT8> { typedef uint2 type; };
template <> struct RowVec<VF_DTYPE_F32> { struct type { uint4 a, b; }; };

template <int DT>
__device__ __forceinline__ void decode8(const typename RowVec<DT>::type& v, float (&x)[8]) {
    if constexpr (DT == VF_DTYPE_F16) {
        const h8 hv = __builtin_bit_cast(h8, v);
#pragma unroll
        for (int e = 0; e < 8; ++e) x[e] = (float)hv[e];
    } else if constexpr (DT == VF_DTYPE_FP8_E4M3) {
        const h8 hv = cvt8_e4m3(v.x, v.y);
#pragma unroll
        for (int e = 0; e < 8; ++e) x[e] = (float)hv[e];
    } else if constexpr (DT == VF_DTYPE_INT8) {
        const h8 hv = cvt8_i8b(v.x, v.y);
#pragma unroll
        for (int e = 0; e < 8; ++e) x[e] = (float)hv[e];
    } else {
        x[0] = __uint_as_float(v.a.x); x[1] = __uint_as_float(v.a.y); x[2] = __uint_as_float(v.a.z); x[3] = __uint_as_float(v.a.w);
        x[4] = __uint_as_float(v.b.x); x[5] = __uint_as_float(v.b.y); x[6] = __uint_as_float(v.b.z); x[7] = __uint_as_float(v.b.w);
    }
}

template <int DT>
__device__ __forceinline__ float rescore_pair(const void* rows, long long row, int d, const float* qs, float nm, int h) {
    constexpr int ESZ = DT == VF_DTYPE_F32 ? 4 : (DT == VF_DTYPE_F16 ? 2 : 1);
    constexpr int kBlk = DT == VF_DTYPE_F32 ? 8 : 16;
    typedef typename RowVec<DT>::type vec_t;
    const float inv = canon_inv(nm);
    float acc[8];
#pragma unroll
    for (int e = 0; e < 8; ++e) acc[e] = 0.0f;
    const char* base = (const char*)rows + row * (long long)d * ESZ;
    const int nblk = d >> 4;
    if constexpr (DT == VF_DTYPE_FP8_E4M3 || DT == VF_DTYPE_INT8) {
        if ((d & 15) == 0) {
            constexpr int kPair = 16;
            const int npair = (nblk + 1) >> 1;
            for (int p0 = 0; p0 < npair; p0 += kPair) {
                uint4 v[kPair];
#pragma unroll
                for (int u = 0; u < kPair; ++u) {
                    int b = 2 * (p0 + u) + h;
                    b = b < nblk ? b : nblk - 1;
                    v[u] = *(const uint4*)(base + (long long)b * 16);
                }
#pragma unroll
                for (int u = 0; u < kPair; ++u) {
                    const u32 sx = h ? v[u].x : v[u].z, sy = h ? v[u].y : v[u].w;
                    const u32 rx = (u32)__shfl_xor((int)sx, 1), ry = (u32)__shfl_xor((int)sy, 1);
                    const uint2 blk0 = h ? make_uint2(rx, ry) : make_uint2(v[u].x, v[u].y);
                    const uint2 blk1 = h ? make_uint2(v[u].z, v[u].w) : make_uint2(rx, ry);
#pragma unroll
                    for (int t = 0; t < 2; ++t) {
                        const int bb = 2 * (p0 + u) + t;
                        const bool live = bb < nblk;
                        const int b = live ? bb : nblk - 1;
                        float x[8];
                        decode8<DT>(t ? blk1 : blk0, x);
                        const float4 q0 = *(const float4*)(qs + b * 16 + 8 * h), q1 = *(const float4*)(qs + b * 16 + 8 * h + 4);
                        const float qq[8] = {q0.x, q0.y, q0.z, q0.w, q1.x, q1.y, q1.z, q1.w};
#pragma unroll
                        for (int e = 0; e < 8; ++e) {
                            const float tt = __builtin_fmaf(qq[e], x[e] * inv, acc[e]);
                            acc[e] = live ? tt : acc[e];
                        }
                    }
                }
            }
            goto tail;
        }
    }
    if ((((long long)d * ESZ) & 15) == 0) {
        for (int b0 = 0; b0 < nblk; b0 += kBlk) {
            vec_t v[kBlk];
#pragma unroll
            for (int u = 0; u < kBlk; ++u) {
                const int b = b0 + u < nblk ? b0 + u : nblk - 1;
                v[u] = *(const vec_t*)(base + ((long long)b * 16 + 8 * h) * ESZ);
            }
#pragma unroll
            for (int u = 0; u < kBlk; ++u) {
                const bool live = b0 + u < nblk;
                const int b = live ? b0 + u : nblk - 1;
                float x[8];
                decode8<DT>(v[u], x);
                const float4 q0 = *(const float4*)(qs + b * 16 + 8 * h), q1 = *(const float4*)(qs + b * 16 + 8 * h + 4);
                const float qq[8] = {q0.x, q0.y, q0.z, q0.w, q1.x, q1.y, q1.z, q1.w};
#pragma unroll
                for (int e = 0; e < 8; ++e) {
                    const float t = __builtin_fmaf(qq[e], x[e] * inv, acc[e]);
                    acc[e] = live ? t : acc[e];
                }
            }
        }
    } else {
        for (int b = 0; b < nblk; ++b)
#pragma unroll
            for (int e = 0; e < 8; ++e) {
                const int j = b * 16 + 8 * h + e;
                acc[e] = __builtin_fmaf(qs[j], load_elem(rows, DT, row * (long long)d + j) * inv, acc[e]);
            }
    }
tail:
#pragma unroll
    for (int e = 0; e < 8; ++e) {
        const int j = nblk * 16 + 8 * h + e;
        if (j < d) acc[e] = __builtin_fmaf(qs[j], load_elem(rows, DT, row * (long long)d + j) * inv, acc[e]);
    }
    float s8[8];
#pragma unroll
    for (int e = 0; e < 8; ++e) s8[e] = acc[e] + __shfl_xor(acc[e], 1);
    const float s4[4] = {s8[0] + s8[4], s8[1] + s8[5], s8[2] + s8[6], s8[3] + s8[7]};
    return (s4[0] + s4[2]) + (s4[1] + s4[3]);
}

__global__ __launch_bounds__(kFinalThreads) void k_final(FinalArgs a) {
    extern __shared__ __attribute__((aligned(16))) char smem_raw[];
    u64* top = (u64*)smem_raw;
    u64* sel = top + a.top_cap;
    u64* rk = sel;
    float* qs = (float*)(sel + a.sel_cap);
    u32* lh = (u32*)(qs + ((a.d + 3) & ~3));
    u32& s_nsel = lh[kHistBins];
    int& s_bin = *(int*)(lh + kHistBins + 1);
    u32& s_minkey = lh[kHistBins + 2];
    const int q = blockIdx.x, tid = threadIdx.x;
    unsigned long long* dbg = (a.dbg && tid == 0) ? a.dbg + (long long)q * 8 : nullptr;
    if (dbg) dbg[0] = wall_clock64();
    const u32 n_raw = a.cnt[q * kCntStride];
    const int n = n_raw < (u32)a.cap ? (int)n_raw : a.cap;
    const int mwant = n < a.kprime ? n : a.kprime;
    const u64* cq = a.cand + (long long)q * a.cap;
    const int tbin = a.tau_bin[q];
    const int band = a.band_q ? a.band_q[q] : a.band;
    if (n_raw > (u32)a.cap) {
        for (int i = tid; i < a.k; i += kFinalThreads) { a.out_ids[(long long)q * a.k + i] = -1; a.out_scores[(long long)q * a.k + i] = -FLT_MAX; }
        if (tid == 0) { a.flags[q] = 2; a.cand_count_out[q] = n_raw; }
        return;
    }
    for (int j = tid; j < a.d; j += kFinalThreads) qs[j] = a.qn[(long long)q * a.d + j];
    for (int b = tid; b < kHistBins; b += kFinalThreads) lh[b] = 0u;
    if (tid == 0) { s_nsel = 0u; s_bin = 0; s_minkey = 0xFFFFFFFFu; }
    __syncthreads();
    const float fscale = tbin > 0 ? 16.0f : 1.0f, forig = tbin > 0 ? (float)tbin : 0.0f;
    auto fine_bin = [&](u64 kv) {
        const float x = (bin_x(unorderkey((u32)(kv >> 32))) - forig) * fscale;
        const int fb = (int)floorf(x) + 1;
        return fb < 0 ? 0 : (fb > kHistBins - 1 ? kHistBins - 1 : fb);
    };
    for (int i = tid; i < n; i += kFinalThreads) atomicAdd(&lh[fine_bin(cq[i])], 1u);
    __syncthreads();
    if (tid < 64) {
        int nb = wave_tau_from_lds(lh, mwant > 0 ? mwant : 1, tid);
        if (band > 0 && nb > 0) nb = max(nb - (tbin > 0 ? band : (band + 15) / 16), tbin > 0 ? 1 : 0);
        if (tid == 0) s_bin = nb > 0 ? nb : 0;
    }
    __syncthreads();
    const int sbin = s_bin;
    u32 mymin = 0xFFFFFFFFu;
    for (int i = tid; i < n; i += kFinalThreads) {
        const u64 kv = cq[i];
        if (fine_bin(kv) >= sbin) {
            const u32 sl = atomicAdd(&s_nsel, 1u);
            if (sl < (u32)a.sel_cap) sel[sl] = kv;
            const u32 ak = (u32)(kv >> 32);
            mymin = ak < mymin ? ak : mymin;
        }
    }
#pragma unroll
    for (int off = 32; off; off >>= 1) { const u32 o = (u32)__shfl_xor((int)mymin, off); mymin = o < mymin ? o : mymin; }
    if ((tid & 63) == 0) atomicMin(&s_minkey, mymin);
    __syncthreads();
    const int ns = (int)s_nsel;
    if (ns > a.sel_cap) {
        for (int i = tid; i < a.k; i += kFinalThreads) { a.out_ids[(long long)q * a.k + i] = -1; a.out_scores[(long long)q * a.k + i] = -FLT_MAX; }
        if (tid == 0) { a.flags[q] = n_raw > (u32)a.cap ? 2 : 1; a.cand_count_out[q] = n_raw; }
        return;
    }
    if (dbg) dbg[1] = wall_clock64();
    const float approx_floor = ns > 0 ? unorderkey(s_minkey) : -INFINITY;
    const int pr = tid >> 1, h = tid & 1;
    for (int i0 = 0; i0 < ns; i0 += kFinalThreads / 2) {
        const int i = i0 + pr;
        u32 row = (u32)sel[i < ns ? i : ns - 1];
        row = (long long)row < a.n_rows ? row : (u32)(a.n_rows - 1);
        const float nm = a.norm[row];
        const float acc = a.orig_dtype == VF_DTYPE_F16       ? rescore_pair<VF_DTYPE_F16>(a.rows_orig, row, a.d, qs, nm, h)
                          : a.orig_dtype == VF_DTYPE_FP8_E4M3 ? rescore_pair<VF_DTYPE_FP8_E4M3>(a.rows_orig, row, a.d, qs, nm, h)
                          : a.orig_dtype == VF_DTYPE_INT8     ? rescore_pair<VF_DTYPE_INT8>(a.rows_orig, row, a.d, qs, nm, h)
                                                              : rescore_pair<VF_DTYPE_F32>(a.rows_orig, row, a.d, qs, nm, h);
        __builtin_amdgcn_wave_barrier();
        if (h == 0 && i < ns) rk[i] = ((u64)orderkey(acc) << 32) | (u64)(0xFFFFFFFFu - row);
    }
    __syncthreads();
    if (dbg) dbg[2] = wall_clock64();
    const u64* ranked;
    if (ns <= 256) {
        rank_select_desc(rk, ns, top, ns < a.top_cap ? ns : a.top_cap, tid);
        ranked = top;
    } else {
        const int P = next_pow2(ns);
        for (int i = ns + tid; i < P; i += kFinalThreads) rk[i] = 0ull;
        __syncthreads();
        bitonic_sort_desc(rk, P, tid, kFinalThreads);
        ranked = rk;
    }
    __syncthreads();
    if (dbg) dbg[3] = wall_clock64();
    const int m = ns;
    for (int i = tid; i < a.k; i += kFinalThreads) {
        long long id = -1;
        float sc = -FLT_MAX;
        if (i < m) {
            const u64 kv = ranked[i];
            id = a.id_offset + (long long)(0xFFFFFFFFu - (u32)kv);
            sc = unorderkey((u32)(kv >> 32));
        }
        a.out_ids[(long long)q * a.k + i] = id;
        a.out_scores[(long long)q * a.k + i] = sc;
    }
    if (tid == 0) {
        int flag = 0;
        if (n_raw > (u32)a.cap) flag = 2;
        else if ((long long)m < a.n_rows) {
            if (tbin > 0 && (mwant < a.kprime || bin_of_x(bin_x(approx_floor)) < tbin)) flag = 1;
            if (a.k > m) flag = 1;
            else if (flag == 0) {
                const float ck_k = unorderkey((u32)(ranked[a.k - 1] >> 32));
                float bound = approx_floor;
                if (band > 0 && sbin > 0) bound = (forig + (float)(sbin - 1) / fscale - 0.5f * kHistBins) / (0.5f * kHistBins) + 0x1p-20f;
                if (!(ck_k > bound + (a.eps_q ? fmaxf(a.eps_q[q], a.eps) : a.eps))) flag = 1;
            }
        }
        a.flags[q] = flag;
        a.cand_count_out[q] = n_raw;
        if (dbg) dbg[4] = wall_clock64();
    }
}

hipError_t launch_final(FinalArgs a, int nq, hipStream_t s) {
    if (nq <= 0) return hipSuccess;
    a.top_cap = (a.kprime + 1) & ~1;
    int sc = 1024;
    while (sc < a.kprime + a.kprime / 4 && sc < 4096) sc <<= 1;
    if (a.band > 0) sc = 4096;
    a.sel_cap = sc > a.top_cap ? sc : a.top_cap;
    const size_t lds = ((size_t)a.top_cap + a.sel_cap) * 8 + ((size_t)a.d + 4 + kHistBins + 4) * 4;
    hipLaunchKernelGGL(k_final, dim3(nq), dim3(kFinalThreads), lds, s, a);
    return hipGetLastError();
}

hipError_t scan_configure() {
    static std::mutex mu;
    static bool done[64] = {};
    int dev = 0;
    hipError_t e = hipGetDevice(&dev);
    if (e != hipSuccess) return e;
    std::lock_guard<std::mutex> g(mu);
    if (dev >= 0 && dev < 64 && done[dev]) return hipSuccess;
#define VF_CFG(NTV, GV) \
    if ((e = configure_one<NTV, GV, kModeSample>()) != hipSuccess) return e; \
    if ((e = configure_one<NTV, GV, kModeMain>()) != hipSuccess) return e;
    VF_CFG(1, 1) VF_CFG(1, 2) VF_CFG(1, 3) VF_CFG(1, 4)
    VF_CFG(2, 1) VF_CFG(2, 2) VF_CFG(2, 3) VF_CFG(2, 4)
#undef VF_CFG
#define VF_X(NT, MODE, F8, S_, RB_, RING_, AR_) \
    if ((e = hipFuncSetAttribute((const void*)k_scan2r<NT, MODE, F8, S_, RB_, RING_, AR_>, hipFuncAttributeMaxDynamicSharedMemorySize, 160 * 1024)) != hipSuccess) return e;
    VF_SCAN2R_ALL(VF_X)
#undef VF_X
#define VF_X(P_, D_) \
    if ((e = hipFuncSetAttribute((const void*)k_scan_ksplit<kModeMain, P_, D_>, hipFuncAttributeMaxDynamicSharedMemorySize, 160 * 1024)) != hipSuccess) return e; \
    if ((e = hipFuncSetAttribute((const void*)k_scan_ksplit<kModeSample, P_, D_>, hipFuncAttributeMaxDynamicSharedMemorySize, 160 * 1024)) != hipSuccess) return e;
    VF_KSPLIT_SHAPES(VF_X)
#undef VF_X
#define VF_X(P_) \
    if ((e = hipFuncSetAttribute((const void*)k_scan_ksplit8<kModeMain, P_>, hipFuncAttributeMaxDynamicSharedMemorySize, 160 * 1024)) != hipSuccess) return e; \
    if ((e = hipFuncSetAttribute((const void*)k_scan_ksplit8<kModeSample, P_>, hipFuncAttributeMaxDynamicSharedMemorySize, 160 * 1024)) != hipSuccess) return e;
    VF_KSPLIT8_SHAPES(VF_X)
#undef VF_X
    if ((e = hipFuncSetAttribute((const void*)k_scan2<1, 0>, hipFuncAttributeMaxDynamicSharedMemorySize, 160 * 1024)) != hipSuccess) return e;
    if ((e = hipFuncSetAttribute((const void*)k_scan2<2, 0>, hipFuncAttributeMaxDynamicSharedMemorySize, 160 * 1024)) != hipSuccess) return e;
// ... 22 lines not shown
```

Baseline: 48450.

## Add per-workgroup global spill tier for scan2r candidate stage overflow

When the LDS candidate stage in k_scan2r fills, entries are now written to a per-workgroup global spill buffer instead of each doing a per-candidate global atomic on the query counter. At workgroup end the spill is batch-compacted with one atomic per query, like the LDS stage. The LDS stage area is also enlarged when the whole segment is ring-buffered. New spill/stat counters are exposed. This adds a spill buffer allocation, fences, an extra LDS descriptor, and a second pass over spilled entries.

```diff
diff --git a/include/veritasfi_hip.h b/include/veritasfi_hip.h
--- a/include/veritasfi_hip.h
+++ b/include/veritasfi_hip.h
@@ -36,7 +36,9 @@
     int64_t scans_overlap;
     int64_t scan_kernel;
     int64_t scan_image;
-    int64_t reserved[3];
+    int64_t stage_spills;
+    int64_t stage_direct;
+    int64_t reserved[1];
 } vf_search_stats;
 
 int vf_version(void);
diff --git a/veritasfi_amd/_ffi.py b/veritasfi_amd/_ffi.py
--- a/veritasfi_amd/_ffi.py
+++ b/veritasfi_amd/_ffi.py
@@ -49,7 +49,7 @@
     _fields_ = [
         ("path", c_i64), ("n_queries", c_i64), ("candidates", c_i64), ("max_candidates", c_i64),
         ("uncertified", c_i64), ("overflowed", c_i64), ("exact_reruns", c_i64), ("wide_launches", c_i64), ("wide_queries", c_i64),
-        ("aux_cus", c_i64), ("scans_overlap", c_i64), ("scan_kernel", c_i64), ("scan_image", c_i64), ("reserved", c_i64 * 3),
+        ("aux_cus", c_i64), ("scans_overlap", c_i64), ("scan_kernel", c_i64), ("scan_image", c_i64), ("stage_spills", c_i64), ("stage_direct", c_i64), ("reserved", c_i64 * 1),
     ]
 
     def as_dict(self):
diff --git a/veritasfi_amd/csrc/vf_api.hip b/veritasfi_amd/csrc/vf_api.hip
--- a/veritasfi_amd/csrc/vf_api.hip
+++ b/veritasfi_amd/csrc/vf_api.hip
@@ -95,6 +95,7 @@
     int scan_image = 0;
     DevBuf qn, qimg, s0, cnt, tau, hist, hist_coarse, cand, flags, counts;
     DevBuf dbg, wgbase, tilecnt, sib;
+    DevBuf spill, spill_stat;
     DevBuf qimg8, epsq;
     DevBuf qscale, bandq;
     int image_i8 = 0;
@@ -157,7 +158,7 @@
     std::mutex mu;
     Slot slots[kSlots];
     int64_t force_path = -1, sample_rows = -1, margin = -1, cap_opt = 0, waves_opt = 0, scan_g = 0,
-            refresh_every = 128, debug = 0, steal_opt = 0, wide_opt = 1, wide_sync = -1, wide_mfma = -1, wide8_waves = 8, wide8_stage = 0,
+            refresh_every = 128, stage_entries = 0, spill_entries = 0, debug = 0, steal_opt = 0, wide_opt = 1, wide_sync = -1, wide_mfma = -1, wide8_waves = 8, wide8_stage = 0,
             aux_cus = -1, sample_grid = -1, overlap_scans = -1, scan_impl = 2, sample_impl = -1, scan_image = 1, wide_rows = 1, image_mfma = -1;
     vf_search_stats stats{};
     bool profile = false;
@@ -179,7 +180,7 @@
     s.h_flags = nullptr; s.h_counts = nullptr; s.h_cap = 0;
     size_t cap = std::max<size_t>(nq_total, 256);
     VF_HIP(hipHostMalloc((void**)&s.h_flags, cap * sizeof(int), hipHostMallocMapped));
-    VF_HIP(hipHostMalloc((void**)&s.h_counts, cap * sizeof(u32), hipHostMallocMapped));
+    VF_HIP(hipHostMalloc((void**)&s.h_counts, (cap + 2) * sizeof(u32), hipHostMallocMapped));
     VF_HIP(hipHostGetDevicePointer((void**)&s.d_flags, s.h_flags, 0));
     VF_HIP(hipHostGetDevicePointer((void**)&s.d_counts, s.h_counts, 0));
     s.h_cap = cap;
@@ -361,7 +362,7 @@
     for (int i = 0; i < kSlots; ++i) {
         Slot& s = ix->slots[i];
         DevBuf* bufs[] = {&s.qn, &s.qimg, &s.s0, &s.cnt, &s.tau, &s.hist, &s.hist_coarse, &s.cand, &s.flags, &s.counts, &s.dense_s,
-                          &s.cn_tmp, &s.parts_ids, &s.parts_sc, &s.run_ids, &s.run_sc, &s.qsel, &s.dbg, &s.wgbase, &s.tilecnt, &s.sib};
+                          &s.cn_tmp, &s.parts_ids, &s.parts_sc, &s.run_ids, &s.run_sc, &s.qsel, &s.dbg, &s.wgbase, &s.tilecnt, &s.sib, &s.spill, &s.spill_stat};
         for (DevBuf* b : bufs) b->release();
         if (s.h_flags) (void)hipHostFree(s.h_flags);
         if (s.h_counts) (void)hipHostFree(s.h_counts);
@@ -637,6 +638,8 @@
     else if (s == "waves") { if (!in_range(0, 8 * 1024)) return fail(VF_EINVAL, "waves must be in [0, 8192]"); ix->waves_opt = value; }
     else if (s == "scan_g") { if (!in_range(0, 4)) return fail(VF_EINVAL, "scan_g must be in [0, 4]"); ix->scan_g = value; }
     else if (s == "refresh_every") { if (!in_range(1, 256)) return fail(VF_EINVAL, "refresh_every must be in [1, 256]"); ix->refresh_every = value; }
+    else if (s == "stage_entries") { if (value != 0 && !in_range(256, 3584)) return fail(VF_EINVAL, "stage_entries must be 0 (auto: what the kernel's LDS leaves) or in [256, 3584] (k_scan2r's candidate stage; more than auto is auto)"); ix->stage_entries = value; }
+    else if (s == "spill_entries") { if (!in_range(-1, 16384)) return fail(VF_EINVAL, "spill_entries must be 0 (auto: from the expected candidate count), -1 (no spill tier) or in [1, 16384] (per workgroup of k_scan2r; more than auto is auto)"); ix->spill_entries = value; }
     else if (s == "steal") { if (!in_range(0, 1)) return fail(VF_EINVAL, "steal must be 0 or 1"); ix->steal_opt = value; }
     else if (s == "wide") { if (!in_range(0, 4096)) return fail(VF_EINVAL, "wide must be 0 (off), 1 (auto) or a query count"); ix->wide_opt = value; }
     else if (s == "wide8_stage") { if (value != 0 && !in_range(64, 3584)) return fail(VF_EINVAL, "wide8_stage must be 0 (auto) or 64..3584 candidate-stage entries"); ix->wide8_stage = value; }
@@ -733,6 +736,7 @@
 
 struct FusedPlan {
     int kprime, cap, total_waves, grid, samp;
+    double expect;
     float eps;
     bool image;
     int tau_band, fine_band;
@@ -823,16 +827,18 @@
     p.grid = (int)wgs;
     p.total_waves = p.grid * (kScanThreads / 64);
     p.samp = ix->sample_rows > 0 ? (int)ix->sample_rows : ((ix->n <= 1500000 && 8ll * p.total_waves >= 16ll * p.kprime) ? 8 : 16);
-    if (ix->cap_opt <= 0) {
+    {
         const double sample_rows = (double)p.total_waves * p.samp;
-        const double expect = p.kprime * (1.0 + log(std::max(1.0, (double)ix->n / std::max(1.0, sample_rows))));
-        while (p.cap < (int)(1.6 * expect) && p.cap < 32768) p.cap <<= 1;
+        p.expect = p.kprime * (1.0 + log(std::max(1.0, (double)ix->n / std::max(1.0, sample_rows))));
+        if (ix->cap_opt <= 0)
+            while (p.cap < (int)(1.6 * p.expect) && p.cap < 32768) p.cap <<= 1;
     }
     p.eps = eps_plan;
     if (image) {
         image_bound(ix->d, ix->dtype, ix->rho_mean, &p.eps, &p.tau_band, &p.fine_band);
         p.kprime = k;
         p.cap = 32768;
+        p.expect = std::max(p.expect, 10000.0);
     }
     return p;
 }
@@ -952,6 +958,21 @@
     return VF_OK;
 }
 
+static int scan2r_tiers(vf_index* ix, Slot& s, const FusedPlan& p, ScanArgs& a2, int qt, int f8) {
+    const int stage_auto = scan2r_stage_cap(ix->dp, qt, f8);
+    a2.stage_cap = ix->stage_entries > 0 ? (int)std::min<int64_t>(ix->stage_entries, stage_auto) : stage_auto;
+    const int64_t hi = std::min<int64_t>(16384, ((int64_t)16 << 20) / 16 / std::max(1, p.grid));
+    const int64_t want = (int64_t)ceil(2.0 * p.expect * kMaxBatch / std::max(1, p.grid)) - stage_auto;
+    const int64_t spill_auto = std::max<int64_t>(std::min<int64_t>(256, hi), std::min<int64_t>(want, hi));
+    a2.spill_cap = ix->spill_entries < 0 ? 0 : (int)(ix->spill_entries > 0 ? std::min<int64_t>(ix->spill_entries, spill_auto) : spill_auto);
+    a2.spill = nullptr;
+    if (a2.spill_cap > 0) {
+        VF_TRY(s.spill.ensure((size_t)p.grid * a2.spill_cap * sizeof(uint4)));
+        a2.spill = s.spill.as<uint4>();
+    }
+    return VF_OK;
+}
+
 static int begin_impl(vf_index* ix, int slot_id, const float* d_queries, int nq, int k, int64_t* d_ids,
                       float* d_scores, hipStream_t user) {
     Slot& s = ix->slots[slot_id];
@@ -968,6 +989,7 @@
     VF_TRY(s.qn.ensure((size_t)std::max(nq, 1) * ix->d * sizeof(float)));
     VF_TRY(s.qimg.ensure(scan_lds_bytes(ix->dp, kMaxBatch)));
     VF_TRY(ensure_pinned(s, (size_t)nq));
+    if (s.h_counts) s.h_counts[s.h_cap] = s.h_counts[s.h_cap + 1] = 0u;
     s.pending = true; s.d_queries = d_queries; s.nq = nq; s.k = k; s.d_ids = d_ids; s.d_scores = d_scores;
     s.path = path; s.user_stream = user; s.wide_launches = 0; s.wide_queries = 0; s.scan_kernel = 0;
     if (nq == 0 || k == 0) { VF_HIP(hipEventRecord(s.ev_done, st)); return VF_OK; }
@@ -1010,6 +1032,7 @@
     VF_TRY(s.hist_coarse.ensure((size_t)kMaxBatch * 64 * sizeof(u32)));
     VF_TRY(s.cand.ensure((size_t)kMaxBatch * p.cap * sizeof(u64)));
     VF_TRY(s.tilecnt.ensure((size_t)p.grid * sizeof(u32)));
+    VF_TRY(s.spill_stat.ensure(2 * sizeof(u32)));
     s.timed = ix->profile;
     if (s.timed) VF_HIP(hipEventRecord(s.ev_t[2], st));
     if (s.wgbase_n != ix->n || s.wgbase_grid != p.grid) {
@@ -1041,6 +1064,7 @@
         a.cand = s.cand.as<u64>(); a.cap = p.cap; a.kprime = p.kprime; a.tau_band = p.tau_band;
         a.hist_coarse = s.hist_coarse.as<u32>(); a.stage_cap = ks ? ksplit_stage_cap(ix) : scan_stage_cap(ix->dp, qt);
         a.tile_cnt = ix->steal_opt ? s.tilecnt.as<u32>() : nullptr; a.scan_grid = p.grid;
+        a.spill_stat = s.spill_stat.as<u32>();
         a.dbg = nullptr;
         if (ix->debug & 128) { VF_TRY(s.dbg.ensure((size_t)p.total_waves * ((ix->debug & 512) ? 72 : 4) * sizeof(u64))); a.dbg = s.dbg.as<u64>(); if (ix->debug & 512) VF_HIP(hipMemsetAsync(s.dbg.p, 0, s.dbg.bytes, st)); }
         a.refresh_every = (int)std::min<int64_t>(256, std::max<int64_t>(4, std::max<int64_t>(1, ix->refresh_every) * nb / kMaxBatch));
@@ -1100,12 +1124,12 @@
             s.scan_kernel = 6;
         } else if (p.image) {
             ScanArgs a2 = a;
-            a2.stage_cap = scan2r_stage_cap(ix->dp, qt, img_f8);
+            VF_TRY(scan2r_tiers(ix, s, p, a2, qt, img_f8));
             VF_HIP(launch_scan2r(a2, qt, p.grid, img_f8, sst));
             s.scan_kernel = 5;
         } else if (capr >= 256) {
             ScanArgs a2 = a;
-            a2.stage_cap = capr;
+            VF_TRY(scan2r_tiers(ix, s, p, a2, qt, f8));
             VF_HIP(launch_scan2r(a2, qt, p.grid, f8, sst));
             s.scan_kernel = 5;
         } else if (cap2 >= 256) {
@@ -1141,6 +1165,7 @@
         if (s.image_i8) { f.eps_q = s.epsq.as<float>(); f.band_q = s.bandq.as<int>() + qt; }
         f.out_ids = (long long*)(d_ids + (size_t)b0 * k); f.out_scores = d_scores + (size_t)b0 * k;
         f.flags = s.d_flags + b0; f.cand_count_out = s.d_counts + b0;
+        f.spill_stat = a.spill_stat; f.spill_stat_out = s.d_counts + s.h_cap;
         f.dbg = nullptr;
         if (ix->debug & 256) { VF_TRY(s.dbg.ensure((size_t)std::max(p.total_waves * 4, 64 * 8) * sizeof(u64))); f.dbg = s.dbg.as<u64>(); }
         VF_HIP(launch_final(f, nb, st));
@@ -1168,6 +1193,7 @@
             if (hipEventElapsedTime(&ms, s.ev_t[2], s.ev_t[3]) == hipSuccess) ix->prof_pipe_ms += ms;
             s.timed = false;
         }
+        stt.stage_spills = s.h_counts[s.h_cap]; stt.stage_direct = s.h_counts[s.h_cap + 1];
         std::vector<int> redo;
         for (int q = 0; q < s.nq; ++q) {
             stt.candidates += s.h_counts[q];
diff --git a/veritasfi_amd/csrc/vf_internal.h b/veritasfi_amd/csrc/vf_internal.h
--- a/veritasfi_amd/csrc/vf_internal.h
+++ b/veritasfi_amd/csrc/vf_internal.h
@@ -108,6 +108,9 @@
     int sib_slack;
     unsigned long long* dbg;
     int debug;
+    uint4* spill;
+    int spill_cap;
+    u32* spill_stat;
 };
 
 struct FinalArgs {
@@ -126,6 +129,8 @@
     long long* out_ids; float* out_scores;
     int* flags;
     u32* cand_count_out;
+    const u32* spill_stat;
+    u32* spill_stat_out;
     unsigned long long* dbg;
 };
 
diff --git a/veritasfi_amd/csrc/vf_kernels.hip b/veritasfi_amd/csrc/vf_kernels.hip
--- a/veritasfi_amd/csrc/vf_kernels.hip
+++ b/veritasfi_amd/csrc/vf_kernels.hip
@@ -755,6 +755,7 @@
 }
 
 constexpr int kCtlBytes = 272;
+constexpr int kSpillDescBytes = 32;
 
 template <int NT>
 __device__ __forceinline__ constexpr int QN_of() { return NT * kQueryTile; }
@@ -798,7 +799,7 @@
     }
 }
 
-template <int NT, int MODE, bool PUBLISH = true, bool INV_LDS = false, bool OFF = false>
+template <int NT, int MODE, bool PUBLISH = true, bool INV_LDS = false, bool OFF = false, bool SPILL = false>
 __device__ __forceinline__ void tile_epilogue(const ScanArgs& a, const f16v (&acc)[NT], const EpiRegs<NT>& e,
                                               long long t0, long long hi, long long s0_slot, int lane, char* ctl) {
     const int r31 = lane & 31, h = lane >> 5;
@@ -927,8 +928,19 @@
             if (slot < (u32)a.stage_cap) {
                 stage_ent[slot] = make_uint4(row, key, (u32)q | (bin << 8), 1u);
             } else {
-                const u32 gs = atomicAdd(a.cnt + q * kCntStride, 1u);
-                if (gs < (u32)a.cap) a.cand[(long long)q * a.cap + gs] = ((u64)key << 32) | (u64)row;
+                bool spilled = false;
+                if constexpr (SPILL) {
+                    const uint4 sd = stage_ent[a.stage_cap];
+                    if (slot - (u32)a.stage_cap < (u32)__builtin_amdgcn_readfirstlane((int)sd.z)) {
+                        uint4* sp = (uint4*)(((u64)(u32)__builtin_amdgcn_readfirstlane((int)sd.y) << 32) | (u64)(u32)__builtin_amdgcn_readfirstlane((int)sd.x));
+                        sp[slot - (u32)a.stage_cap] = make_uint4(row, key, (u32)q | (bin << 8), 1u);
+                        spilled = true;
+                    }
+                }
+                if (!spilled) {
+                    const u32 gs = atomicAdd(a.cnt + q * kCntStride, 1u);
+                    if (gs < (u32)a.cap) a.cand[(long long)q * a.cap + gs] = ((u64)key << 32) | (u64)row;
+                }
                 atomicAdd(a.hist + (long long)q * kHistBins + bin, 1u);
                 atomicAdd(a.hist_coarse + q * 64 + (bin >> 5), 1u);
             }
@@ -1785,13 +1797,14 @@
 size_t scan2r_lds_bytes(int dp, int qn_tile, int stage_cap, int f8) {
     const Scan2rShape sh = scan2r_shape(dp, f8);
     const size_t seg_img = (size_t)(f8 ? 128 : 64) * qn_tile * 2;
-    return (size_t)(sh.S - sh.RB) * seg_img + (size_t)kScan2Waves * (sh.RING * kSegBytes + kScratchBytes) + kCtlBytes + (size_t)stage_cap * 16;
+    return (size_t)(sh.S - sh.RB) * seg_img + (size_t)kScan2Waves * (sh.RING * kSegBytes + kScratchBytes) + kCtlBytes + (size_t)stage_cap * 16 + kSpillDescBytes;
 }
 int scan2r_stage_cap(int dp, int qn_tile, int f8) {
     if (scan2r_shape(dp, f8).S == 0) return 0;
     const size_t fixed = scan2r_lds_bytes(dp, qn_tile, 0, f8);
     if (fixed + 256 * 16 > 160 * 1024) return 0;
-    const size_t area = std::min<size_t>(160 * 1024 - fixed, 32 * 1024);
+    const Scan2rShape sh = scan2r_shape(dp, f8);
+    const size_t area = std::min<size_t>(160 * 1024 - fixed, sh.S == sh.RB ? 56 * 1024 : 32 * 1024);
     return (int)(area / 16);
 }
 
@@ -1920,6 +1933,11 @@
         uint4* z = (uint4*)ctl;
         const int nz = kCtlBytes / 16 + (MODE == kModeMain ? a.stage_cap : 0);
         for (int i = tid; i < nz; i += THREADS) z[i] = make_uint4(0u, (i == 0) ? (u32)kScan2Waves : 0u, 0u, 0u);
+        if (MODE == kModeMain && tid == 0) {
+            const u64 sp = (u64)(a.spill + (long long)blockIdx.x * a.spill_cap), st = (u64)a.spill_stat;
+            z[nz] = make_uint4((u32)sp, (u32)(sp >> 32), a.spill ? (u32)a.spill_cap : 0u, 0u);
+            z[nz + 1] = make_uint4((u32)st, (u32)(st >> 32), 0u, 0u);
+        }
     }
     __syncthreads();
     if (MODE == kModeMain) {
@@ -2121,7 +2139,7 @@
 #pragma unroll
                 for (int nt = 0; nt < NT; ++nt) epi.tau_g[nt] = *(const int*)(sc + (nt * kQueryTile + r31) * 4);
             }
-            tile_epilogue<NT, MODE, true, true, F8 >= 2>(a, acc, epi, t0, t_hi, t_s0, lane, ctl);
+            tile_epilogue<NT, MODE, true, true, F8 >= 2, MODE == kModeMain>(a, acc, epi, t0, t_hi, t_s0, lane, ctl);
 #pragma unroll
             for (int nt = 0; nt < NT; ++nt)
 #pragma unroll
@@ -2136,6 +2154,7 @@
     if (dbg && dbg_rec > 4) dbg[69] = (unsigned long long)tiles_done;
     asm volatile("s_waitcnt vmcnt(0)" ::: "memory");
     if (MODE == kModeSample) return;
+    if (*(const volatile u32*)ctl > (u32)a.stage_cap) __builtin_amdgcn_fence(__ATOMIC_RELEASE, "agent");
     if (lane == 0) atomicAdd((u32*)(ctl + 8), 1u);
     if (dbg) dbg[1] = wall_clock64();
     __syncthreads();
@@ -2166,6 +2185,44 @@
             const u32 q = e.z & 0xFFu;
             const u32 gs = qbase[q] + (e.w - 2u);
             if (gs < (u32)a.cap) a.cand[(long long)q * a.cap + gs] = ((u64)e.y << 32) | (u64)e.x;
+        }
+        const uint4 sd = ent[a.stage_cap], sd1 = ent[a.stage_cap + 1];
+        const u32 over = staged > (u32)a.stage_cap ? staged - (u32)a.stage_cap : 0u;
+        const u32 nsp = over < sd.z ? over : sd.z;
+        if (nsp > 0u) {
+            const uint4* sp = (const uint4*)(((u64)sd.y << 32) | (u64)sd.x);
+            auto spill_entry = [&](u32 i) {
+                const u64* w = (const u64*)(sp + i);
+                const u64 lo_ = __hip_atomic_load(w, __ATOMIC_RELAXED, __HIP_MEMORY_SCOPE_AGENT), hi_ = __hip_atomic_load(w + 1, __ATOMIC_RELAXED, __HIP_MEMORY_SCOPE_AGENT);
+                return make_uint4((u32)lo_, (u32)(lo_ >> 32), (u32)hi_, (u32)(hi_ >> 32));
+            };
+            __syncthreads();
+            __builtin_amdgcn_fence(__ATOMIC_ACQUIRE, "agent");
+            if (tid < QN) qcnt[tid] = 0u;
+            __syncthreads();
+            for (u32 i = tid; i < nsp; i += THREADS) {
+                const uint4 e = spill_entry(i);
+                const u32 q = e.z & 0xFFu;
+                if (e.w == 1u && q < (u32)QN) atomicAdd(qcnt + q, 1u);
+            }
+            __syncthreads();
+            if (tid < QN) {
+                const u32 c = qcnt[tid];
+                qbase[tid] = c ? atomicAdd(a.cnt + tid * kCntStride, c) : 0u;
+            }
+            __syncthreads();
+            for (u32 i = tid; i < nsp; i += THREADS) {
+                const uint4 e = spill_entry(i);
+                const u32 q = e.z & 0xFFu;
+                if (e.w != 1u || q >= (u32)QN) continue;
+                const u32 gs = atomicAdd(qbase + q, 1u);
+                if (gs < (u32)a.cap) a.cand[(long long)q * a.cap + gs] = ((u64)e.y << 32) | (u64)e.x;
+            }
+        }
+        u32* stat = (u32*)(((u64)sd1.y << 32) | (u64)sd1.x);
+        if (tid == 0 && over > 0u && stat) {
+            if (nsp > 0u) atomicAdd(stat, nsp);
+            if (over > nsp) atomicAdd(stat + 1, over - nsp);
         }
     }
     if (dbg && dbg_rec > 4) dbg[71] = __builtin_amdgcn_s_memtime() - c_entry;
@@ -3434,6 +3491,7 @@
     }
     if (tid == 0) {
         a.cnt[q * kCntStride] = lcnt;
+        if (q == 0 && a.spill_stat) a.spill_stat[0] = a.spill_stat[1] = 0u;
         a.tau_bin[q] = (q < a.nq && !(a.debug & 1)) ? tb : kHistBins;
     }
     if (q == 0 && a.tile_cnt)
@@ -3610,6 +3668,10 @@
     const int q = blockIdx.x, tid = threadIdx.x;
     unsigned long long* dbg = (a.dbg && tid == 0) ? a.dbg + (long long)q * 8 : nullptr;
     if (dbg) dbg[0] = wall_clock64();
+    if (q == 0 && tid == 0 && a.spill_stat && a.spill_stat_out) {
+        a.spill_stat_out[0] += a.spill_stat[0];
+        a.spill_stat_out[1] += a.spill_stat[1];
+    }
     const u32 n_raw = a.cnt[q * kCntStride];
     const int n = n_raw < (u32)a.cap ? (int)n_raw : a.cap;
     const int mwant = n < a.kprime ? n : a.kprime;
```

After: 48900 (median of 5 runs). No clear change (+0.9%).
